# PreferredAI/cornac

Hardware: AMD Instinct MI355X
Metric: bpr_triplets_per_sec (higher is better)
Workload: dtype f32

## Files before the change

### cornac_amd/_lib.py

```python
import ctypes as C
import os
import subprocess

import numpy as np

_HERE = os.path.dirname(os.path.abspath(__file__))
PROFILE = os.environ.get("CORNAC_HIP_PROFILE", "") == "1"
LIB_PATH = os.path.join(_HERE, "lib", "libcornac_hip_profile.so" if PROFILE else "libcornac_hip.so")
CSRC = os.path.join(_HERE, "csrc")

MODE_DETERMINISTIC = 0
MODE_HOGWILD = 1
VEBPR_NO_OWNERSHIP = 0x100
HOG_FORM_MASK, HOG_FORM_SHIFT = 0xF0000, 16
FORM_AUTO, FORM_FUSED, FORM_STRATA, FORM_LDSBIN = (f << HOG_FORM_SHIFT for f in range(4))
HOG_PLAIN_STORES, HOG_VEC4_LAYOUT, HOG_NO_OWNERSHIP, HOG_DENSE_BIAS, HOG_SHARE_NEG = 1, 2, 4, 8, 16
HOG_BINNED, HOG_FUSED_OPT_OUT = 64, 128
HOG_ABLATE_MASK, HOG_ABLATE_SHIFT = 0xFF00, 8
NEG_UNIFORM = 0
NEG_POPULARITY = 1

SYMBOLS = [
    "cornac_hip_last_error", "cornac_hip_version", "cornac_hip_device_count", "cornac_hip_device_info",
    "cornac_hip_device_probe",
    "cornac_hip_bpr_create", "cornac_hip_bpr_destroy", "cornac_hip_bpr_set_factors", "cornac_hip_bpr_get_factors",
    "cornac_hip_bpr_bind_device", "cornac_hip_bpr_rebind_items", "cornac_hip_bpr_conveyor_setup", "cornac_hip_bpr_conveyor_layout", "cornac_hip_bpr_conveyor_enqueue", "cornac_hip_bpr_set_negative_population", "cornac_hip_bpr_device_ptrs", "cornac_hip_bpr_set_stream",
    "cornac_hip_bpr_seed_mt19937", "cornac_hip_bpr_seed_hogwild", "cornac_hip_bpr_fit_epochs",
    "cornac_hip_bpr_set_factors_f64", "cornac_hip_bpr_get_factors_f64", "cornac_hip_bpr_fit_epochs_f64",
    "cornac_hip_bpr_hogwild_enqueue", "cornac_hip_bpr_sync", "cornac_hip_bpr_debug_draw",
    "cornac_hip_bpr_last_timing", "cornac_hip_bpr_kernel_timing", "cornac_hip_mf_kernel_timing",
    "cornac_hip_bpr_debug_ownership", "cornac_hip_bpr_set_views", "cornac_hip_bpr_seed_view_stream",
    "cornac_hip_vebpr_fit_epochs", "cornac_hip_vebpr_fit_epochs_f64", "cornac_hip_vebpr_hogwild_form",
    "cornac_hip_mmmf_fit_epochs", "cornac_hip_mmmf_fit_epochs_f64", "cornac_hip_mmmf_hogwild_enqueue",
    "cornac_hip_bpr_strata_config", "cornac_hip_bpr_chunk_records", "cornac_hip_bpr_strata_stats", "cornac_hip_bpr_debug_strata",
    "cornac_hip_bpr_ldsbin_config", "cornac_hip_bpr_ldsbin_pass_config", "cornac_hip_bpr_ldsbin_stats",
    "cornac_hip_bpr_ldsbin_deal_config", "cornac_hip_bpr_debug_ldsbin_deal",
    "cornac_hip_bpr_sample_triplets", "cornac_hip_bpr_apply_triplets", "cornac_hip_bpr_gather_rows",
    "cornac_hip_bpr_staged_slots", "cornac_hip_bpr_emit_triplets", "cornac_hip_bpr_apply_staged",
    "cornac_hip_bpr_shard_mark", "cornac_hip_bpr_shard_slots", "cornac_hip_bpr_shard_uniq",
    "cornac_hip_bpr_scatter_diff_rows", "cornac_hip_bpr_switch_stream",
    "cornac_hip_bpr_scatter_add_rows", "cornac_hip_bpr_table_delta_begin", "cornac_hip_bpr_table_delta_finish",
    "cornac_hip_bpr_table_delta_step", "cornac_hip_table_delta", "cornac_hip_bpr_table_delta",
    "cornac_hip_bpr_resident_exchange_bins", "cornac_hip_bpr_epoch_resident_enqueue", "cornac_hip_bpr_resident_flush",
    "cornac_hip_stream_wait_counter", "cornac_hip_stream_set_flag", "cornac_hip_stream_ring_standin",
    "cornac_hip_vbpr_create", "cornac_hip_vbpr_destroy", "cornac_hip_vbpr_set_params", "cornac_hip_vbpr_get_params",
    "cornac_hip_vbpr_fit_batches", "cornac_hip_vbpr_item_tables",
    "cornac_hip_wmf_create", "cornac_hip_wmf_destroy", "cornac_hip_wmf_set_factors", "cornac_hip_wmf_get_factors",
    "cornac_hip_wmf_fit_batches", "cornac_hip_wmf_kernel_timing", "cornac_hip_wmf_last_timing",
    "cornac_hip_mf_create", "cornac_hip_mf_destroy", "cornac_hip_mf_set_factors", "cornac_hip_mf_get_factors",
    "cornac_hip_mf_fit", "cornac_hip_mf_bind_items", "cornac_hip_mf_bind_users", "cornac_hip_mf_set_stream", "cornac_hip_mf_epoch_enqueue",
    "cornac_hip_mf_sync", "cornac_hip_mf_fit_sgd", "cornac_hip_mf_last_timing",
    "cornac_hip_mf_hogwild_form", "cornac_hip_mf_hogwild_stats", "cornac_hip_mf_debug_split", "cornac_hip_mf_debug_ownership",
    "cornac_hip_mf_fit_minibatch", "cornac_hip_mf_fit_minibatch_dropout", "cornac_hip_mf_reset_optimizer",
    "cornac_hip_mf_pmf_set_factors", "cornac_hip_mf_pmf_get_factors", "cornac_hip_mf_pmf_fit", "cornac_hip_mf_pmf_form",
    "cornac_hip_mf_nmf_set_factors", "cornac_hip_mf_nmf_get_factors", "cornac_hip_mf_nmf_fit", "cornac_hip_mf_nmf_form",
    "cornac_hip_mf_hpf_set_tables", "cornac_hip_mf_hpf_get_tables", "cornac_hip_mf_hpf_fit", "cornac_hip_mf_hpf_elog",
    "cornac_hip_mf_hpf_form",
    "cornac_hip_scorer_create", "cornac_hip_scorer_destroy", "cornac_hip_scorer_set", "cornac_hip_score_user",
    "cornac_hip_scorer_set_f64", "cornac_hip_score_user_f64",
    "cornac_hip_score_block", "cornac_hip_rank_topk", "cornac_hip_rank_topk_device", "cornac_hip_score_pairs",
    "cornac_hip_scorer_set_exclusions", "cornac_hip_rank_topk_resident", "cornac_hip_scorer_host_buffer",
    "cornac_hip_rank_positions",
]


class HipError(RuntimeError):

    def __init__(self, code, msg):
        super().__init__("libcornac_hip error %d: %s" % (code, msg))
        self.code = code


def build(force=False, verbose=False):
    cmd = ["make", "-C", CSRC, "-j", "4"] + (["-B"] if force else []) + (["PROFILE=1"] if PROFILE else [])
    out = subprocess.run(cmd, stdout=subprocess.PIPE, stderr=subprocess.STDOUT, text=True)
    if verbose or out.returncode != 0:
        print(out.stdout)
    if out.returncode != 0:
        raise RuntimeError("building libcornac_hip.so failed")
    return LIB_PATH


_lib = None

_f32 = np.ctypeslib.ndpointer(np.float32, flags="C_CONTIGUOUS")
_i32 = np.ctypeslib.ndpointer(np.int32, flags="C_CONTIGUOUS")
_i64 = np.ctypeslib.ndpointer(np.int64, flags="C_CONTIGUOUS")
_vp = C.c_void_p


def _preload_torch_hip_runtime():
    import importlib.util
    import sys

    if "torch" in sys.modules:
        return
    try:
        spec = importlib.util.find_spec("torch")
        libdir = os.path.join(list(spec.submodule_search_locations)[0], "lib")
    except Exception:
        return
    for name in ("libhsa-runtime64.so", "libamdhip64.so"):
        path = os.path.join(libdir, name)
        if os.path.exists(path):
            try:
                C.CDLL(path, mode=C.RTLD_GLOBAL)
            except OSError:
                return


def lib():
    global _lib
    if _lib is None:
        if not os.path.exists(LIB_PATH):
            raise RuntimeError(
                "libcornac_hip.so not found at %s. Build it with `python -c 'import __graft_entry__ as g; g.build()'` "
                "or `make -C cornac_amd/csrc`. cornac_amd has no CPU fallback." % LIB_PATH)
        _preload_torch_hip_runtime()
        L = C.CDLL(LIB_PATH)
        L.cornac_hip_last_error.restype = C.c_char_p
        L.cornac_hip_version.restype = C.c_char_p
        L.cornac_hip_device_count.argtypes = [C.POINTER(C.c_int)]
        L.cornac_hip_device_info.argtypes = [C.c_int, C.c_char_p, C.c_int, C.POINTER(C.c_int), C.POINTER(C.c_int64)]
        L.cornac_hip_device_probe.argtypes = [C.c_int, C.c_int64, C.POINTER(C.c_double)]
        L.cornac_hip_bpr_create.argtypes = [C.POINTER(_vp), C.c_int, C.c_int64, C.c_int64, C.c_int64, C.c_int64,
                                            C.c_int, _i32, _i32, C.c_int64]
        L.cornac_hip_bpr_destroy.argtypes = [_vp]
        L.cornac_hip_bpr_set_factors.argtypes = [_vp, _vp, _vp, _vp]
        L.cornac_hip_bpr_get_factors.argtypes = [_vp, _vp, _vp, _vp]
        L.cornac_hip_bpr_bind_device.argtypes = [_vp, _vp, _vp, _vp]
        L.cornac_hip_bpr_rebind_items.argtypes = [_vp, _vp, _vp]
        L.cornac_hip_bpr_conveyor_setup.argtypes = [_vp, C.c_int, _vp, C.c_uint64, C.c_int, C.POINTER(C.c_int), C.POINTER(C.c_int),
                                                    C.POINTER(C.c_int)]
        L.cornac_hip_bpr_conveyor_layout.argtypes = [_vp, C.c_uint32, _vp, _vp]
        L.cornac_hip_bpr_conveyor_enqueue.argtypes = [_vp, C.c_uint32, C.c_uint32, C.c_int, C.POINTER(C.c_int32), C.POINTER(_vp),
                                                      C.c_float, C.c_float, C.c_int, C.c_int, C.c_int]
        L.cornac_hip_bpr_set_negative_population.argtypes = [_vp, _vp, C.c_int64]
        L.cornac_hip_bpr_device_ptrs.argtypes = [_vp, C.POINTER(_vp), C.POINTER(_vp), C.POINTER(_vp)]
        L.cornac_hip_bpr_set_stream.argtypes = [_vp, _vp]
        L.cornac_hip_bpr_switch_stream.argtypes = [_vp, _vp]
        L.cornac_hip_bpr_seed_mt19937.argtypes = [_vp, C.c_uint32, C.c_uint32, C.c_int]
        L.cornac_hip_bpr_seed_hogwild.argtypes = [_vp, C.c_uint64]
        L.cornac_hip_bpr_fit_epochs.argtypes = [_vp, C.c_int, C.c_float, C.c_float, C.c_int, C.c_int, C.c_int,
                                                C.c_int, C.POINTER(C.c_int64), C.POINTER(C.c_int64)]
        L.cornac_hip_bpr_set_factors_f64.argtypes = [_vp, _vp, _vp, _vp]
        L.cornac_hip_bpr_get_factors_f64.argtypes = [_vp, _vp, _vp, _vp]
        L.cornac_hip_bpr_fit_epochs_f64.argtypes = [_vp, C.c_int, C.c_double, C.c_double, C.c_int, C.c_int,
                                                    C.POINTER(C.c_int64), C.POINTER(C.c_int64)]
        L.cornac_hip_bpr_hogwild_enqueue.argtypes = [_vp, C.c_int64, C.c_float, C.c_float, C.c_int, C.c_int, C.c_int]
        L.cornac_hip_bpr_sync.argtypes = [_vp, C.POINTER(C.c_int64), C.POINTER(C.c_int64)]
        L.cornac_hip_bpr_debug_draw.argtypes = [_vp, C.c_int, C.c_uint64, C.c_int64, _i64]
        L.cornac_hip_bpr_last_timing.argtypes = [_vp, C.POINTER(C.c_double)]
        L.cornac_hip_bpr_set_views.argtypes = [_vp, _i32, _i32, C.c_int64]
        L.cornac_hip_bpr_seed_view_stream.argtypes = [_vp, C.c_uint32]
        L.cornac_hip_vebpr_hogwild_form.argtypes = [_vp, C.POINTER(C.c_int)]
        L.cornac_hip_vebpr_fit_epochs.argtypes = [_vp, C.c_int, C.c_float, C.c_float, C.c_float, C.c_int,
                                                  C.POINTER(C.c_int64), C.POINTER(C.c_int64)]
        L.cornac_hip_vebpr_fit_epochs_f64.argtypes = [_vp, C.c_int, C.c_double, C.c_double, C.c_double,
                                                      C.POINTER(C.c_int64), C.POINTER(C.c_int64)]
        L.cornac_hip_mmmf_fit_epochs.argtypes = [_vp, C.c_int, C.c_float, C.c_float, C.c_int, C.POINTER(C.c_int64),
                                                 C.POINTER(C.c_int64)]
        L.cornac_hip_mmmf_fit_epochs_f64.argtypes = [_vp, C.c_int, C.c_double, C.c_double, C.POINTER(C.c_int64),
                                                     C.POINTER(C.c_int64)]
        L.cornac_hip_mmmf_hogwild_enqueue.argtypes = [_vp, C.c_int64, C.c_float, C.c_float]
        L.cornac_hip_bpr_sample_triplets.argtypes = [_vp, C.c_int64, C.c_int, _vp, _vp, _vp]
        L.cornac_hip_bpr_apply_triplets.argtypes = [_vp, _vp, _vp, _vp, C.c_int64, _vp, _vp, C.c_int, C.c_float,
                                                    C.c_float, C.c_int]
        L.cornac_hip_bpr_gather_rows.argtypes = [_vp, _vp, _vp, C.c_int64, C.c_int, _vp]
        L.cornac_hip_bpr_staged_slots.argtypes = [_vp, C.c_int64, C.POINTER(C.c_int64)]
        L.cornac_hip_bpr_emit_triplets.argtypes = [_vp, C.c_int64, C.c_int, _vp, _vp, _vp, C.c_int64, C.POINTER(C.c_int64)]
        L.cornac_hip_bpr_apply_staged.argtypes = [_vp, _vp, _vp, _vp, C.c_int64, _vp, _vp, C.c_int, C.c_float, C.c_float,
                                                  C.c_int]
        L.cornac_hip_bpr_shard_mark.argtypes = [_vp, _vp, _vp, C.c_int64, C.c_int, C.c_int64, _vp]
        L.cornac_hip_bpr_shard_slots.argtypes = [_vp, _vp, _vp, C.c_int64, C.c_int, C.c_int64, _vp, _vp, _vp]
        L.cornac_hip_bpr_shard_uniq.argtypes = [_vp, _vp, _vp, C.c_int64, C.c_int64, _vp]
        L.cornac_hip_bpr_scatter_diff_rows.argtypes = [_vp, _vp, _vp, C.c_int64, C.c_int, _vp, _vp, _vp]
        L.cornac_hip_bpr_scatter_add_rows.argtypes = [_vp, _vp, _vp, C.c_int64, C.c_int, _vp]
        L.cornac_hip_bpr_table_delta_begin.argtypes = [_vp, _vp, _vp, C.c_int64, C.c_int, _vp, _vp]
        L.cornac_hip_bpr_table_delta_finish.argtypes = [_vp, _vp, _vp, _vp, _vp, C.c_int64, C.c_int]
        L.cornac_hip_bpr_table_delta_step.argtypes = [_vp, _vp, _vp, _vp, _vp, C.c_int64, C.c_int, _vp, _vp]
        L.cornac_hip_table_delta.argtypes = [C.c_int, C.c_int, _vp, _vp, _vp, _vp, _vp, C.c_int64, C.c_int, _vp, _vp]
        L.cornac_hip_bpr_table_delta.argtypes = [_vp, C.c_int, C.c_int, _vp, _vp, _vp, _vp, C.c_int64, C.c_int, _vp, _vp]
        L.cornac_hip_bpr_resident_exchange_bins.argtypes = [_vp, C.c_int, C.c_int, C.POINTER(C.c_int)]
        L.cornac_hip_bpr_epoch_resident_enqueue.argtypes = [_vp, C.c_float, C.c_float, C.c_int, C.c_int, C.c_int, C.c_int,
                                                            C.c_int, _vp, _vp, C.c_int64, _vp, C.c_int64, _vp, _vp, _vp,
                                                            C.POINTER(C.c_int)]
        L.cornac_hip_bpr_resident_flush.argtypes = [_vp, C.c_int, C.c_int, _vp, _vp, C.c_int64, _vp, C.c_int64, _vp, _vp]
        L.cornac_hip_stream_wait_counter.argtypes = [C.c_int, _vp, _vp, C.c_uint32, _vp, C.c_int]
        L.cornac_hip_stream_set_flag.argtypes = [C.c_int, _vp, _vp, C.c_uint32, _vp]
        L.cornac_hip_stream_ring_standin.argtypes = [C.c_int, _vp, _vp, C.c_int64, _vp, C.c_int64, C.c_int64, C.c_int]
        L.cornac_hip_bpr_debug_ownership.argtypes = [_vp, C.POINTER(C.c_int64), _vp, _vp, _vp]
        L.cornac_hip_bpr_strata_config.argtypes = [_vp, C.c_int, C.c_int, C.c_int]
        L.cornac_hip_bpr_chunk_records.argtypes = [_vp, C.c_int]
        L.cornac_hip_bpr_strata_stats.argtypes = [_vp, C.POINTER(C.c_int64)]
        L.cornac_hip_bpr_debug_strata.argtypes = [_vp, C.c_uint32, _vp, _vp, _vp, _vp, C.POINTER(C.c_uint32)]
        L.cornac_hip_bpr_ldsbin_config.argtypes = [_vp, C.c_int, C.c_int, C.c_int]
        L.cornac_hip_bpr_ldsbin_pass_config.argtypes = [_vp, C.c_int, C.c_int, C.c_int, C.c_int]
        L.cornac_hip_bpr_ldsbin_stats.argtypes = [_vp, C.POINTER(C.c_int64)]
        L.cornac_hip_bpr_ldsbin_deal_config.argtypes = [_vp, C.c_int, C.c_int]
        L.cornac_hip_bpr_debug_ldsbin_deal.argtypes = [_vp, C.c_uint64, C.c_uint32, _vp, _vp, _vp, _vp, _vp]
        L.cornac_hip_bpr_kernel_timing.argtypes = [_vp, C.c_int, C.POINTER(C.c_double), C.POINTER(C.c_int64)]
        L.cornac_hip_mf_kernel_timing.argtypes = [_vp, C.c_int, C.POINTER(C.c_double), C.POINTER(C.c_int64)]
        L.cornac_hip_vbpr_create.argtypes = [C.POINTER(_vp), C.c_int, C.c_int64, C.c_int64, C.c_int, C.c_int, C.c_int, _f32]
        L.cornac_hip_vbpr_destroy.argtypes = [_vp]
        L.cornac_hip_vbpr_set_params.argtypes = [_vp] + [_vp] * 6
        L.cornac_hip_vbpr_get_params.argtypes = [_vp] + [_vp] * 6
        L.cornac_hip_vbpr_fit_batches.argtypes = [_vp, _i32, _i32, _i32, C.c_int64, C.c_int, C.c_float, C.c_float,
                                                  C.c_float, C.c_float, C.POINTER(C.c_double)]
        L.cornac_hip_vbpr_item_tables.argtypes = [_vp, _f32, _f32]
        L.cornac_hip_mf_fit_minibatch.argtypes = [_vp, _i64, C.c_int64, C.c_int, C.c_int, C.c_float, C.c_float,
                                                  C.c_float, C.c_int, C.POINTER(C.c_double)]
        L.cornac_hip_mf_fit_minibatch_dropout.argtypes = [_vp, _i64, C.c_int64, C.c_int, C.c_int, C.c_float, C.c_float,
                                                          C.c_float, C.c_int, _vp, _vp, C.c_float, C.POINTER(C.c_double)]
        L.cornac_hip_mf_reset_optimizer.argtypes = [_vp]
        L.cornac_hip_mf_pmf_set_factors.argtypes = [_vp, _vp, _vp]
        L.cornac_hip_mf_pmf_get_factors.argtypes = [_vp, _vp, _vp]
        L.cornac_hip_mf_pmf_fit.argtypes = [_vp, C.c_int, C.c_float, C.c_float, C.c_float, C.c_int, _vp]
        L.cornac_hip_mf_pmf_form.argtypes = [_vp, C.POINTER(C.c_int), C.POINTER(C.c_int)]
        L.cornac_hip_mf_nmf_set_factors.argtypes = [_vp, _vp, _vp, _vp, _vp]
        L.cornac_hip_mf_nmf_get_factors.argtypes = [_vp, _vp, _vp, _vp, _vp]
        L.cornac_hip_mf_nmf_fit.argtypes = [_vp, C.c_int] + [C.c_float] * 6 + [C.c_int, C.c_int, _vp]
        L.cornac_hip_mf_nmf_form.argtypes = [_vp] + [C.POINTER(C.c_int)] * 3
        L.cornac_hip_mf_hpf_set_tables.argtypes = [_vp] * 5
        L.cornac_hip_mf_hpf_get_tables.argtypes = [_vp] * 7
        L.cornac_hip_mf_hpf_fit.argtypes = [_vp, C.c_int, C.c_int]
        L.cornac_hip_mf_hpf_elog.argtypes = [_vp, _vp, _vp]
        L.cornac_hip_mf_hpf_form.argtypes = [_vp] + [C.POINTER(C.c_int)] * 2
        L.cornac_hip_wmf_create.argtypes = [C.POINTER(_vp), C.c_int, C.c_int64, C.c_int64, C.c_int, _i64, _i32, _f32,
                                            C.c_int64]
        L.cornac_hip_wmf_destroy.argtypes = [_vp]
        L.cornac_hip_wmf_destroy.restype = None
        L.cornac_hip_wmf_set_factors.argtypes = [_vp, _f32, _f32]
        L.cornac_hip_wmf_get_factors.argtypes = [_vp, _f32, _f32]
        L.cornac_hip_wmf_fit_batches.argtypes = [_vp, _i32, _i64, C.c_int64, C.c_float, C.c_float, C.c_float,
                                                 C.c_float, C.c_float, _vp]
        L.cornac_hip_wmf_kernel_timing.argtypes = [_vp, C.c_int]
        L.cornac_hip_wmf_last_timing.argtypes = [_vp, C.POINTER(C.c_double)]
        L.cornac_hip_mf_create.argtypes = [C.POINTER(_vp), C.c_int, C.c_int64, C.c_int64, C.c_int, _i64, _i64, _f32,
                                           C.c_int64]
        L.cornac_hip_mf_destroy.argtypes = [_vp]
        L.cornac_hip_mf_set_factors.argtypes = [_vp, _vp, _vp, _vp, _vp]
        L.cornac_hip_mf_get_factors.argtypes = [_vp, _vp, _vp, _vp, _vp]
        L.cornac_hip_mf_bind_items.argtypes = [_vp, _vp, _vp]
        L.cornac_hip_mf_bind_users.argtypes = [_vp, _vp, _vp]
        L.cornac_hip_mf_set_stream.argtypes = [_vp, _vp]
        L.cornac_hip_mf_epoch_enqueue.argtypes = [_vp, C.c_int, C.c_int, C.c_float, C.c_float, C.c_float, C.c_int]
        L.cornac_hip_mf_sync.argtypes = [_vp, C.POINTER(C.c_double)]
        L.cornac_hip_mf_fit.argtypes = [_vp, C.c_int, C.c_float, C.c_float, C.c_float, C.c_int, C.c_int, C.c_int, _vp,
                                        C.POINTER(C.c_int)]
        L.cornac_hip_mf_fit_sgd.argtypes = [C.c_int, _i64, _i64, _f32, C.c_int64, _f32, _f32, _f32, _f32, C.c_int64,
                                            C.c_int64, C.c_int, C.c_float, C.c_float, C.c_float, C.c_int, C.c_int,
                                            C.c_int, C.c_int, _vp, C.POINTER(C.c_int)]
        L.cornac_hip_mf_last_timing.argtypes = [_vp, C.POINTER(C.c_double)]
        L.cornac_hip_mf_hogwild_form.argtypes = [_vp, C.c_int]
        L.cornac_hip_mf_hogwild_stats.argtypes = [_vp, C.POINTER(C.c_int64)]
        L.cornac_hip_mf_debug_split.argtypes = [_vp, C.POINTER(C.c_int64), C.POINTER(C.c_int64), _vp, _vp]
        L.cornac_hip_mf_debug_ownership.argtypes = [_vp, C.POINTER(C.c_int64), _vp, _vp, _vp]
        L.cornac_hip_scorer_create.argtypes = [C.POINTER(_vp), C.c_int, C.c_int64, C.c_int64, C.c_int]
        L.cornac_hip_scorer_destroy.argtypes = [_vp]
        L.cornac_hip_scorer_set.argtypes = [_vp, _f32, _f32, _vp, _vp]
        L.cornac_hip_score_user.argtypes = [_vp, C.c_int64, _f32]
        L.cornac_hip_scorer_set_f64.argtypes = [_vp, _vp, _vp, _vp, _vp]
        L.cornac_hip_score_user_f64.argtypes = [_vp, C.c_int64, _vp]
        L.cornac_hip_score_block.argtypes = [_vp, _i32, C.c_int64, _f32]
        L.cornac_hip_score_pairs.argtypes = [_vp, _i32, _i32, C.c_int64, C.c_int, C.c_float, C.c_float, _f32]
        L.cornac_hip_rank_topk.argtypes = [_vp, _i32, C.c_int64, C.c_int, _vp, _vp, _i32, _f32]
        L.cornac_hip_rank_positions.argtypes = [_vp, _i32, C.c_int64, _vp, _vp, _vp, _vp, _i32, _i32, _i32, _f32]
        L.cornac_hip_rank_topk_device.argtypes = [_vp, C.c_int64, C.c_int64, C.c_int, C.c_int, C.POINTER(C.c_double)]
        L.cornac_hip_scorer_set_exclusions.argtypes = [_vp, _vp, _vp]
        L.cornac_hip_scorer_host_buffer.argtypes = [_vp, C.c_size_t, C.POINTER(_vp)]
        L.cornac_hip_rank_topk_resident.argtypes = [_vp, _vp, C.c_int64, C.c_int64, C.c_int, _vp, _vp, _vp]
        _lib = L
    return _lib


def check(rc):
    if rc != 0:
        raise HipError(rc, lib().cornac_hip_last_error().decode("utf-8", "replace"))


def stream_wait_counter(device, stream, d_counter, target, d_error, timeout_ms=5000):
    check(lib().cornac_hip_stream_wait_counter(int(device), stream, d_counter, int(target), d_error, int(timeout_ms)))


def stream_ring_standin(device, stream, d_src, src_floats, d_dst, dst_floats, n_floats, n_workgroups=16):
    check(lib().cornac_hip_stream_ring_standin(int(device), stream, d_src, int(src_floats), d_dst, int(dst_floats),
                                               int(n_floats), int(n_workgroups)))


def stream_set_flag(device, stream, d_flag, value=1, d_unless=None):
    check(lib().cornac_hip_stream_set_flag(int(device), stream, d_flag, int(value), d_unless))


def device_count():
    n = C.c_int(0)
    check(lib().cornac_hip_device_count(C.byref(n)))
    return n.value


def device_probe(device=0, nbytes=6 << 30):
    o = (C.c_double * 3)()
    check(lib().cornac_hip_device_probe(device, int(nbytes), o))
    return {"d2d_copy_GBps": o[0], "stream_read_GBps": o[1], "row_gather_512B_GBps": o[2], "buffer_bytes": int(nbytes)}


def device_info(device=0):
    name = C.create_string_buffer(256)
    cus = C.c_int()
    mem = C.c_int64()
    check(lib().cornac_hip_device_info(device, name, 256, C.byref(cus), C.byref(mem)))
    return {"name": name.value.decode(), "compute_units": cus.value, "hbm_bytes": mem.value}


def _ptr(a):
    return None if a is None else a.ctypes.data


def _f32c(a):
    return None if a is None else np.ascontiguousarray(a, dtype=np.float32)


class BprTrainer:

    def __init__(self, indptr, indices, n_users, n_items, total_users, total_items, k, device=0):
        self.indptr = np.ascontiguousarray(indptr, np.int32)
        self.indices = np.ascontiguousarray(indices, np.int32)
        self.shape = (int(total_users), int(total_items), int(k))
        self.nnz = len(self.indices)
        self.n_items = int(n_items)
        self.device, self._stream = int(device), None
        self.h = _vp()
        check(lib().cornac_hip_bpr_create(C.byref(self.h), device, n_users, n_items, total_users, total_items, k,
                                          self.indptr, self.indices, self.nnz))

    def close(self):
        if getattr(self, "h", None) is not None and self.h and lib is not None:
            lib().cornac_hip_bpr_destroy(self.h)
            self.h = None

    __del__ = close

    def set_factors(self, U=None, V=None, B=None):
        U, V, B = _f32c(U), _f32c(V), _f32c(B)
        tu, ti, k = self.shape
        assert U is None or U.shape == (tu, k)
        assert V is None or V.shape == (ti, k)
        assert B is None or B.shape == (ti,)
        check(lib().cornac_hip_bpr_set_factors(self.h, _ptr(U), _ptr(V), _ptr(B)))

    def get_factors(self):
        tu, ti, k = self.shape
        U, V, B = np.empty((tu, k), np.float32), np.empty((ti, k), np.float32), np.empty(ti, np.float32)
        check(lib().cornac_hip_bpr_get_factors(self.h, U.ctypes.data, V.ctypes.data, B.ctypes.data))
        return U, V, B

    def set_factors_f64(self, U, V, B):
        tu, ti, k = self.shape
        U, V, B = (np.ascontiguousarray(a, np.float64) for a in (U, V, B))
        assert U.shape == (tu, k) and V.shape == (ti, k) and B.shape == (ti,)
        check(lib().cornac_hip_bpr_set_factors_f64(self.h, U.ctypes.data, V.ctypes.data, B.ctypes.data))

    def get_factors_f64(self):
        tu, ti, k = self.shape
        U, V, B = np.empty((tu, k), np.float64), np.empty((ti, k), np.float64), np.empty(ti, np.float64)
        check(lib().cornac_hip_bpr_get_factors_f64(self.h, U.ctypes.data, V.ctypes.data, B.ctypes.data))
        return U, V, B

    def fit_epochs_f64(self, n_epochs, lr, reg, use_bias=True, neg_population=NEG_UNIFORM):
        c, s = C.c_int64(), C.c_int64()
        check(lib().cornac_hip_bpr_fit_epochs_f64(self.h, n_epochs, float(lr), float(reg), int(use_bias), neg_population,
                                                  C.byref(c), C.byref(s)))
        return c.value, s.value

    def get_user_factors(self):
        tu, _, k = self.shape
        U = np.empty((tu, k), np.float32)
        check(lib().cornac_hip_bpr_get_factors(self.h, U.ctypes.data, None, None))
        return U

    def get_item_factors(self):
        _, ti, k = self.shape
        V, B = np.empty((ti, k), np.float32), np.empty(ti, np.float32)
        check(lib().cornac_hip_bpr_get_factors(self.h, None, V.ctypes.data, B.ctypes.data))
        return V, B

    def seed_mt19937(self, seed_pos, seed_neg, shared_stream=False):
        check(lib().cornac_hip_bpr_seed_mt19937(self.h, seed_pos, seed_neg, int(shared_stream)))

    def seed_hogwild(self, seed):
        check(lib().cornac_hip_bpr_seed_hogwild(self.h, int(seed) & 0xFFFFFFFFFFFFFFFF))

    def fit_epochs(self, n_epochs, lr, reg, use_bias=True, neg_population=NEG_UNIFORM, mode=MODE_HOGWILD, flags=0):
        c, s = C.c_int64(), C.c_int64()
        check(lib().cornac_hip_bpr_fit_epochs(self.h, n_epochs, lr, reg, int(use_bias), neg_population, mode, flags,
                                              C.byref(c), C.byref(s)))
        return c.value, s.value

    def hogwild_enqueue(self, n_samples, lr, reg, use_bias=True, neg_population=NEG_UNIFORM, flags=0):
        check(lib().cornac_hip_bpr_hogwild_enqueue(self.h, n_samples, lr, reg, int(use_bias), neg_population, flags))

    def sync(self):
        c, s = C.c_int64(), C.c_int64()
        check(lib().cornac_hip_bpr_sync(self.h, C.byref(c), C.byref(s)))
        return c.value, s.value

    def bind_device(self, dU=None, dV=None, dB=None):
        check(lib().cornac_hip_bpr_bind_device(self.h, dU, dV, dB))

    def set_negative_population(self, items):
        items = np.ascontiguousarray(items if items is not None else [], np.int32)
        check(lib().cornac_hip_bpr_set_negative_population(self.h, items.ctypes.data if len(items) else None, len(items)))

    def rebind_items(self, dV, dB):
        check(lib().cornac_hip_bpr_rebind_items(self.h, dV, dB))

    def conveyor_setup(self, n_blocks, rank_item=None, deal_seed=0, release_item_tables=True):
        order = None if rank_item is None else np.ascontiguousarray(rank_item, np.int32)
        nb, bpb, cap = C.c_int(), C.c_int(), C.c_int()
        check(lib().cornac_hip_bpr_conveyor_setup(self.h, int(n_blocks), None if order is None else order.ctypes.data,
                                                  int(deal_seed) & 0xFFFFFFFFFFFFFFFF, int(bool(release_item_tables)),
                                                  C.byref(nb), C.byref(bpb), C.byref(cap)))
        return nb.value, bpb.value, cap.value

    def conveyor_layout(self, layout_epoch, d_slot_item, d_item_slot):
        check(lib().cornac_hip_bpr_conveyor_layout(self.h, int(layout_epoch), d_slot_item, d_item_slot))

    def conveyor_enqueue(self, epoch, layout_epoch, first_blocks, d_rows, lr, reg, use_bias=True, neg_population=NEG_UNIFORM,
                         flags=0):
        n = len(first_blocks)
        fb = (C.c_int32 * n)(*[int(b) for b in first_blocks])
        rows = (_vp * n)(*[int(p) for p in d_rows])
        check(lib().cornac_hip_bpr_conveyor_enqueue(self.h, int(epoch), int(layout_epoch), n, fb, rows, lr, reg, int(use_bias),
                                                    neg_population, int(flags)))

    def device_ptrs(self):
        u, v, b = _vp(), _vp(), _vp()
        check(lib().cornac_hip_bpr_device_ptrs(self.h, C.byref(u), C.byref(v), C.byref(b)))
        return u.value, v.value, b.value

    def set_stream(self, stream_ptr):
        check(lib().cornac_hip_bpr_set_stream(self.h, stream_ptr))
        self._stream = stream_ptr

    def switch_stream(self, stream_ptr):
        check(lib().cornac_hip_bpr_switch_stream(self.h, stream_ptr))
        self._stream = stream_ptr

    def sample_triplets(self, n_draws, d_u, d_i, d_j, neg_population=NEG_UNIFORM):
        check(lib().cornac_hip_bpr_sample_triplets(self.h, int(n_draws), neg_population, d_u, d_i, d_j))

    def apply_triplets(self, d_u, d_slot_i, d_slot_j, n, d_rows, d_bias, bias_stride, lr, reg, use_bias=True):
        check(lib().cornac_hip_bpr_apply_triplets(self.h, d_u, d_slot_i, d_slot_j, int(n), d_rows, d_bias,
                                                  int(bias_stride), lr, reg, int(use_bias)))

    def staged_slots(self, n_draws):
        n = C.c_int64()
        check(lib().cornac_hip_bpr_staged_slots(self.h, int(n_draws), C.byref(n)))
        return n.value

    def emit_triplets(self, n_draws, d_u, d_i, d_j, slots_cap, neg_population=NEG_UNIFORM):
        n = C.c_int64()
        check(lib().cornac_hip_bpr_emit_triplets(self.h, int(n_draws), neg_population, d_u, d_i, d_j, int(slots_cap),
                                                 C.byref(n)))
        return n.value

    def apply_staged(self, d_u, d_slot_i, d_slot_j, n_slots, d_rows, d_bias, bias_stride, lr, reg, use_bias=True):
        check(lib().cornac_hip_bpr_apply_staged(self.h, d_u, d_slot_i, d_slot_j, int(n_slots), d_rows, d_bias,
                                                int(bias_stride), lr, reg, int(use_bias)))

    def shard_mark(self, d_i, d_j, n, world, rows_per_rank, d_mark):
        check(lib().cornac_hip_bpr_shard_mark(self.h, d_i, d_j, int(n), int(world), int(rows_per_rank), d_mark))

    def shard_slots(self, d_i, d_j, n, world, rows_per_rank, d_scan, d_slot_i, d_slot_j):
        check(lib().cornac_hip_bpr_shard_slots(self.h, d_i, d_j, int(n), int(world), int(rows_per_rank), d_scan, d_slot_i,
                                               d_slot_j))

    def shard_uniq(self, d_mark, d_scan, n_rows, rows_per_rank, d_uniq_local):
        check(lib().cornac_hip_bpr_shard_uniq(self.h, d_mark, d_scan, int(n_rows), int(rows_per_rank), d_uniq_local))

    def scatter_diff_rows(self, d_table, d_ids, n, width, d_now, d_before, d_scale=None):
        check(lib().cornac_hip_bpr_scatter_diff_rows(self.h, d_table, d_ids, int(n), int(width), d_now, d_before, d_scale))

    def _delta(self, op, rule, *args):
        check(lib().cornac_hip_bpr_table_delta(self.h, op, int(rule), *args))

    def table_delta_begin(self, d_flat, d_base, n_items, k, d_bucket, d_local, rule=0):
        if rule:
            return self._delta(0, rule, d_flat, d_base, None, None, int(n_items), int(k), d_bucket, d_local)
        check(lib().cornac_hip_bpr_table_delta_begin(self.h, d_flat, d_base, int(n_items), int(k), d_bucket, d_local))

    def table_delta_finish(self, d_flat, d_base, d_bucket, d_local, n_items, k, rule=0):
        if rule:
            return self._delta(1, rule, d_flat, d_base, d_bucket, d_local, int(n_items), int(k), None, None)
        check(lib().cornac_hip_bpr_table_delta_finish(self.h, d_flat, d_base, d_bucket, d_local, int(n_items), int(k)))

    def table_delta_step(self, d_flat, d_base, d_bucket_prev, d_local_prev, n_items, k, d_bucket, d_local, rule=0):
        if rule:
            return self._delta(2, rule, d_flat, d_base, d_bucket_prev, d_local_prev, int(n_items), int(k), d_bucket, d_local)
        check(lib().cornac_hip_bpr_table_delta_step(self.h, d_flat, d_base, d_bucket_prev, d_local_prev, int(n_items),
                                                    int(k), d_bucket, d_local))

    def resident_exchange_bins(self, neg_population=NEG_UNIFORM, flags=0):
        n = C.c_int()
        check(lib().cornac_hip_bpr_resident_exchange_bins(self.h, neg_population, flags, C.byref(n)))
        return n.value

    def epoch_resident_enqueue(self, lr, reg, use_bias, neg_population, flags, n_exchanges, rule, d_base, d_buckets,
                               bucket_stride, d_keeps, keep_stride, d_arrive, d_landed, d_applied):
        n = C.c_int()
        check(lib().cornac_hip_bpr_epoch_resident_enqueue(self.h, lr, reg, int(use_bias), neg_population, flags,
                                                          int(n_exchanges), int(rule), d_base, d_buckets, int(bucket_stride),
                                                          d_keeps, int(keep_stride), d_arrive, d_landed, d_applied, C.byref(n)))
        return n.value

    def resident_flush(self, n_exchanges, rule, d_base, d_buckets, bucket_stride, d_keeps, keep_stride, d_applied, d_landed=None):
        check(lib().cornac_hip_bpr_resident_flush(self.h, int(n_exchanges), int(rule), d_base, d_buckets, int(bucket_stride),
                                                  d_keeps, int(keep_stride), d_applied, d_landed))

    def gather_rows(self, d_table, d_ids, n, width, d_out):
        check(lib().cornac_hip_bpr_gather_rows(self.h, d_table, d_ids, int(n), int(width), d_out))

    def scatter_add_rows(self, d_table, d_ids, n, width, d_delta):
        check(lib().cornac_hip_bpr_scatter_add_rows(self.h, d_table, d_ids, int(n), int(width), d_delta))

    def debug_draw(self, stream, hi, n):
        out = np.empty(n, np.int64)
        check(lib().cornac_hip_bpr_debug_draw(self.h, stream, hi, n, out))
        return out

    def set_views(self, view_indptr, view_indices):
        self.v_indptr = np.ascontiguousarray(view_indptr, np.int32)
        self.v_indices = np.ascontiguousarray(view_indices, np.int32)
        if len(self.v_indices) == 0:
            self.v_indices = np.zeros(1, np.int32)
        check(lib().cornac_hip_bpr_set_views(self.h, self.v_indptr, self.v_indices, int(self.v_indptr[-1])))

    def seed_view_stream(self, seed_view):
        check(lib().cornac_hip_bpr_seed_view_stream(self.h, seed_view))

    def fit_epochs_vebpr(self, n_epochs, lr, reg, alpha, mode=MODE_HOGWILD, ownership=True):
        c, s = C.c_int64(), C.c_int64()
        check(lib().cornac_hip_vebpr_fit_epochs(self.h, n_epochs, lr, reg, alpha, mode | (0 if ownership else VEBPR_NO_OWNERSHIP),
                                                C.byref(c), C.byref(s)))
        return c.value, s.value

    def fit_epochs_vebpr_f64(self, n_epochs, lr, reg, alpha):
        c, s = C.c_int64(), C.c_int64()
        check(lib().cornac_hip_vebpr_fit_epochs_f64(self.h, n_epochs, float(lr), float(reg), float(alpha), C.byref(c),
                                                    C.byref(s)))
        return c.value, s.value

    def vebpr_hogwild_owned(self):
        o = C.c_int()
        check(lib().cornac_hip_vebpr_hogwild_form(self.h, C.byref(o)))
        return bool(o.value)

    def mmmf_fit_epochs(self, n_epochs, lr, reg, mode=MODE_HOGWILD):
        c, s = C.c_int64(), C.c_int64()
        check(lib().cornac_hip_mmmf_fit_epochs(self.h, n_epochs, lr, reg, mode, C.byref(c), C.byref(s)))
        return c.value, s.value

    def mmmf_fit_epochs_f64(self, n_epochs, lr, reg):
        c, s = C.c_int64(), C.c_int64()
        check(lib().cornac_hip_mmmf_fit_epochs_f64(self.h, n_epochs, float(lr), float(reg), C.byref(c), C.byref(s)))
        return c.value, s.value

    def mmmf_hogwild_enqueue(self, n_samples, lr, reg):
        check(lib().cornac_hip_mmmf_hogwild_enqueue(self.h, n_samples, lr, reg))

    def debug_ownership(self):
        w = C.c_int64()
        check(lib().cornac_hip_bpr_debug_ownership(self.h, C.byref(w), None, None, None))
        if w.value == 0:
            return None
        wp = np.empty(w.value + 1, np.int64)
        ou, oi = np.empty(self.nnz, np.int32), np.empty(self.nnz, np.int32)
        check(lib().cornac_hip_bpr_debug_ownership(self.h, C.byref(w), wp.ctypes.data, ou.ctypes.data,
                                                   oi.ctypes.data))
        return wp, ou, oi

    def ldsbin_config(self, hot_x1000=75, min_candidates=48, max_rounds=4):
        check(lib().cornac_hip_bpr_ldsbin_config(self.h, int(hot_x1000), int(min_candidates), int(max_rounds)))

    def ldsbin_deal_config(self, strata_groups=16, hot_cost_x16=32):
        check(lib().cornac_hip_bpr_ldsbin_deal_config(self.h, int(strata_groups), int(hot_cost_x16)))

    def debug_ldsbin_deal(self, seed, epoch):
        st = self.ldsbin_stats()
        bins, nh = st["bins"], st["hot_interactions"]
        bin_of = np.empty(self.n_items, np.int32)
        cold, off = np.empty(bins, np.uint32), np.empty(bins + 1, np.uint32)
        hu, hi = np.empty(max(nh, 1), np.int32), np.empty(max(nh, 1), np.int32)
        check(lib().cornac_hip_bpr_debug_ldsbin_deal(self.h, int(seed), int(epoch), bin_of.ctypes.data, cold.ctypes.data,
                                                     off.ctypes.data, hu.ctypes.data, hi.ctypes.data))
        return bin_of, cold, off, hu[:nh], hi[:nh]

    def ldsbin_pass_config(self, enable=True, waves=8, lds_kb=64, min_draws_x100=200):
        check(lib().cornac_hip_bpr_ldsbin_pass_config(self.h, int(bool(enable)), int(waves), int(lds_kb), int(min_draws_x100)))

    def ldsbin_stats(self):
        o = (C.c_int64 * 8)()
        check(lib().cornac_hip_bpr_ldsbin_stats(self.h, o))
        return {"bins": o[0], "rows_per_bin": o[1], "n_hot": o[2], "hot_interactions": o[3], "bitmap_words": o[4],
                "lds_bytes": o[5], "lock_timeouts": o[6], "block_threads": o[7]}

    def strata_config(self, hot_permille=120, hot_min_mult_x100=200, rehash_period=1):
        check(lib().cornac_hip_bpr_strata_config(self.h, int(hot_permille), int(hot_min_mult_x100), int(rehash_period)))

    def chunk_records(self, enable=True):
        check(lib().cornac_hip_bpr_chunk_records(self.h, int(bool(enable))))

    def strata_stats(self):
        o = (C.c_int64 * 4)()
        check(lib().cornac_hip_bpr_strata_stats(self.h, o))
        return {"n_hot": o[0], "misplaced_workgroups": o[1], "bucket_builds": o[2], "waves": o[3]}

    def debug_strata(self, epoch):
        wp = self.debug_ownership()[0]
        W = len(wp) - 1
        sptr = np.empty(8 * W + 1, np.int64)
        ru, ri = np.empty(self.nnz, np.int32), np.empty(self.nnz, np.int32)
        rank_item = np.empty(self.n_items, np.int32)
        key = C.c_uint32()
        check(lib().cornac_hip_bpr_debug_strata(self.h, int(epoch), sptr.ctypes.data, ru.ctypes.data, ri.ctypes.data,
                                                rank_item.ctypes.data, C.byref(key)))
        return sptr, ru, ri, rank_item, key.value

    def kernel_timing(self, enable=True):
        ms, n = C.c_double(), C.c_int64()
        check(lib().cornac_hip_bpr_kernel_timing(self.h, int(enable), C.byref(ms), C.byref(n)))
        return ms.value, n.value

    def last_timing(self):
        t = (C.c_double * 4)()
        check(lib().cornac_hip_bpr_last_timing(self.h, t))
        return {"sampler_ms": t[0], "schedule_ms": t[1], "sgd_ms": t[2], "total_ms": t[3]}


class MfTrainer:
    def __init__(self, rid, cid, val, n_users, n_items, k, device=0):
        self.rid = np.ascontiguousarray(rid, np.int64)
        self.cid = np.ascontiguousarray(cid, np.int64)
        self.val = np.ascontiguousarray(val, np.float32)
        self.shape = (int(n_users), int(n_items), int(k))
        self.h = _vp()
        check(lib().cornac_hip_mf_create(C.byref(self.h), device, n_users, n_items, k, self.rid, self.cid, self.val,
                                         len(self.val)))
        self.device, self._stream = int(device), None

    def close(self):
        if getattr(self, "h", None) is not None and self.h and lib is not None:
            lib().cornac_hip_mf_destroy(self.h)
            self.h = None

    __del__ = close

    def set_factors(self, U=None, V=None, Bu=None, Bi=None):
        U, V, Bu, Bi = _f32c(U), _f32c(V), _f32c(Bu), _f32c(Bi)
        check(lib().cornac_hip_mf_set_factors(self.h, _ptr(U), _ptr(V), _ptr(Bu), _ptr(Bi)))

    def get_factors(self):
        nu, ni, k = self.shape
        U, V = np.empty((nu, k), np.float32), np.empty((ni, k), np.float32)
        Bu, Bi = np.empty(nu, np.float32), np.empty(ni, np.float32)
        check(lib().cornac_hip_mf_get_factors(self.h, U.ctypes.data, V.ctypes.data, Bu.ctypes.data, Bi.ctypes.data))
        return U, V, Bu, Bi

    def fit(self, max_iter, lr, reg, mu, use_bias=True, early_stop=False, mode=MODE_HOGWILD):
        loss = np.zeros(max(max_iter, 1), np.float32)
        n = C.c_int()
        check(lib().cornac_hip_mf_fit(self.h, max_iter, lr, reg, mu, int(use_bias), int(early_stop), mode,
                                      loss.ctypes.data, C.byref(n)))
        return loss[:n.value], n.value

    def bind_items(self, d_V, d_Bi):
        check(lib().cornac_hip_mf_bind_items(self.h, d_V, d_Bi))

    def bind_users(self, d_U, d_Bu):
        check(lib().cornac_hip_mf_bind_users(self.h, d_U, d_Bu))

    def set_stream(self, hip_stream):
        check(lib().cornac_hip_mf_set_stream(self.h, hip_stream))
        self._stream = hip_stream

    def epoch_enqueue(self, part, n_parts, lr, reg, mu, use_bias=True):
        check(lib().cornac_hip_mf_epoch_enqueue(self.h, int(part), int(n_parts), lr, reg, mu, int(use_bias)))

    def sync(self):
        l = C.c_double()
        check(lib().cornac_hip_mf_sync(self.h, C.byref(l)))
        return l.value

    def table_delta_begin(self, d_flat, d_base, n_items, k, d_bucket, d_local, rule=0):
        check(lib().cornac_hip_table_delta(0 | (int(rule) << 4), self.device, self._stream, d_flat, d_base, None, None,
                                           int(n_items), int(k), d_bucket, d_local))

    def table_delta_finish(self, d_flat, d_base, d_bucket, d_local, n_items, k, rule=0):
        check(lib().cornac_hip_table_delta(1 | (int(rule) << 4), self.device, self._stream, d_flat, d_base, d_bucket, d_local,
                                           int(n_items), int(k), None, None))

    def table_delta_step(self, d_flat, d_base, d_bucket_prev, d_local_prev, n_items, k, d_bucket, d_local, rule=0):
        check(lib().cornac_hip_table_delta(2 | (int(rule) << 4), self.device, self._stream, d_flat, d_base, d_bucket_prev,
                                           d_local_prev, int(n_items), int(k), d_bucket, d_local))

    OPTIMIZERS = {"sgd": 0, "adam": 1, "rmsprop": 2, "adagrad": 3}

    def fit_minibatch(self, order, batch_size, optimizer, lr, reg, mu, use_bias=True, keep_u=None, keep_i=None,
                      keep_scale=1.0):
        order = np.ascontiguousarray(order, np.int64)
        loss = C.c_double()
        if keep_u is not None:
            keep_u, keep_i = np.ascontiguousarray(keep_u, np.uint8), np.ascontiguousarray(keep_i, np.uint8)
            if keep_u.shape != (len(order), self.shape[2]) or keep_i.shape != keep_u.shape:
                raise ValueError("keep masks must be [len(order), k] = %r, got %r / %r"
                                 % ((len(order), self.shape[2]), keep_u.shape, keep_i.shape))
            check(lib().cornac_hip_mf_fit_minibatch_dropout(self.h, order, len(order), int(batch_size),
                                                            self.OPTIMIZERS[optimizer], lr, reg, mu, int(use_bias),
                                                            keep_u.ctypes.data, keep_i.ctypes.data, float(keep_scale),
                                                            C.byref(loss)))
            return loss.value
        check(lib().cornac_hip_mf_fit_minibatch(self.h, order, len(order), int(batch_size), self.OPTIMIZERS[optimizer],
                                                lr, reg, mu, int(use_bias), C.byref(loss)))
        return loss.value

    def reset_optimizer(self):
        check(lib().cornac_hip_mf_reset_optimizer(self.h))

    PMF_VARIANTS = {"linear": 0, "non_linear": 1}

    def pmf_set_factors(self, U, V):
        nu, ni, k = self.shape
        U, V = np.ascontiguousarray(U, np.float64), np.ascontiguousarray(V, np.float64)
        if U.shape != (nu, k) or V.shape != (ni, k):
            raise ValueError("PMF tables must be %r and %r, got %r and %r" % ((nu, k), (ni, k), U.shape, V.shape))
        check(lib().cornac_hip_mf_pmf_set_factors(self.h, U.ctypes.data, V.ctypes.data))

    def pmf_get_factors(self):
        nu, ni, k = self.shape
        U, V = np.empty((nu, k), np.float64), np.empty((ni, k), np.float64)
        check(lib().cornac_hip_mf_pmf_get_factors(self.h, U.ctypes.data, V.ctypes.data))
        return U, V

    def pmf_fit(self, n_epochs, lr, reg, gamma, variant):
        loss = np.zeros(max(int(n_epochs), 1), np.float64)
        check(lib().cornac_hip_mf_pmf_fit(self.h, int(n_epochs), lr, reg, gamma, self.PMF_VARIANTS.get(variant, variant),
                                          loss.ctypes.data))
        return loss[:max(int(n_epochs), 0)]

    def pmf_form(self):
        form, group = C.c_int(), C.c_int()
        check(lib().cornac_hip_mf_pmf_form(self.h, C.byref(form), C.byref(group)))
        return form.value, group.value

    def nmf_set_factors(self, U, V, Bu=None, Bi=None):
        nu, ni, k = self.shape
        U, V, Bu, Bi = _f32c(U), _f32c(V), _f32c(Bu), _f32c(Bi)
        if U.shape != (nu, k) or V.shape != (ni, k):
            raise ValueError("NMF tables must be %r and %r, got %r and %r" % ((nu, k), (ni, k), U.shape, V.shape))
        if (Bu is not None and Bu.shape != (nu,)) or (Bi is not None and Bi.shape != (ni,)):
            raise ValueError("NMF biases must be (%d,) and (%d,)" % (nu, ni))
        check(lib().cornac_hip_mf_nmf_set_factors(self.h, _ptr(U), _ptr(V), _ptr(Bu), _ptr(Bi)))

    def nmf_get_factors(self):
        nu, ni, k = self.shape
        U, V = np.empty((nu, k), np.float32), np.empty((ni, k), np.float32)
        Bu, Bi = np.empty(nu, np.float32), np.empty(ni, np.float32)
        check(lib().cornac_hip_mf_nmf_get_factors(self.h, U.ctypes.data, V.ctypes.data, Bu.ctypes.data, Bi.ctypes.data))
        return U, V, Bu, Bi

    def nmf_fit(self, n_epochs, lr, lambda_u, lambda_v, lambda_bu, lambda_bi, mu, use_bias=False, mode=MODE_HOGWILD):
        loss = np.zeros(max(int(n_epochs), 1), np.float64)
        check(lib().cornac_hip_mf_nmf_fit(self.h, int(n_epochs), lr, lambda_u, lambda_v, lambda_bu, lambda_bi, mu,
                                          int(bool(use_bias)), int(mode), loss.ctypes.data))
        return loss[:max(int(n_epochs), 0)]

    def nmf_form(self):
        o = [C.c_int(), C.c_int(), C.c_int()]
        check(lib().cornac_hip_mf_nmf_form(self.h, *[C.byref(x) for x in o]))
        return tuple(x.value for x in o)

    HPF_MAX_K = 256

    def hpf_set_tables(self, G_s, G_r, L_s, L_r):
        nu, ni, k = self.shape
        if k > self.HPF_MAX_K:
            raise ValueError("HPF keeps a row's sums in registers: k = %d is above its limit of %d" % (k, self.HPF_MAX_K))
        tables = [np.ascontiguousarray(a, np.float64) for a in (G_s, G_r, L_s, L_r)]
        for a, name, shape in zip(tables, ("G_s", "G_r", "L_s", "L_r"), ((nu, k), (nu, k), (ni, k), (ni, k))):
            if a.shape != shape:
                raise ValueError("HPF table %s must be %r, got %r" % (name, shape, a.shape))
            if not (np.isfinite(a).all() and (a > 0).all()):
                raise ValueError("HPF table %s must be strictly positive and finite" % name)
        check(lib().cornac_hip_mf_hpf_set_tables(self.h, *[a.ctypes.data for a in tables]))

    def hpf_get_tables(self):
        nu, ni, k = self.shape
        out = [np.empty(s, np.float64) for s in ((nu, k), (nu, k), (ni, k), (ni, k), (nu,), (ni,))]
        check(lib().cornac_hip_mf_hpf_get_tables(self.h, *[a.ctypes.data for a in out]))
        return tuple(out)

    def hpf_fit(self, n_iters, hierarchical=True):
        check(lib().cornac_hip_mf_hpf_fit(self.h, int(n_iters), int(bool(hierarchical))))

    def hpf_elog(self):
        nu, ni, k = self.shape
        Lt, Lb = np.empty((nu, k), np.float64), np.empty((ni, k), np.float64)
        check(lib().cornac_hip_mf_hpf_elog(self.h, Lt.ctypes.data, Lb.ctypes.data))
        return Lt, Lb

    def hpf_form(self):
        o = [C.c_int(), C.c_int()]
        check(lib().cornac_hip_mf_hpf_form(self.h, *[C.byref(x) for x in o]))
        return tuple(x.value for x in o)

    def kernel_timing(self, enable=True):
        ms, n = C.c_double(), C.c_int64()
        check(lib().cornac_hip_mf_kernel_timing(self.h, int(enable), C.byref(ms), C.byref(n)))
        return ms.value, n.value

    def hogwild_form(self, form):
        check(lib().cornac_hip_mf_hogwild_form(self.h, int(form)))

    def hogwild_stats(self):
        o = (C.c_int64 * 4)()
        check(lib().cornac_hip_mf_hogwild_stats(self.h, o))
        return {"form_used": o[0], "tiles": o[1], "rows_per_bin": o[2], "gave_up": bool(o[3])}

    def debug_split(self):
        ns, nv = C.c_int64(), C.c_int64()
        check(lib().cornac_hip_mf_debug_split(self.h, C.byref(ns), C.byref(nv), None, None))
        items, ptr = np.empty(ns.value, np.int32), np.zeros(ns.value + 1, np.int32)
        if ns.value:
            check(lib().cornac_hip_mf_debug_split(self.h, C.byref(ns), C.byref(nv), items.ctypes.data, ptr.ctypes.data))
        return items, ptr

    def debug_ownership(self):
        w = C.c_int64()
        check(lib().cornac_hip_mf_debug_ownership(self.h, C.byref(w), None, None, None))
        if w.value == 0:
            return None
        wp = np.empty(w.value + 1, np.int64)
        ou, oi = np.empty(len(self.val), np.int32), np.empty(len(self.val), np.int32)
        check(lib().cornac_hip_mf_debug_ownership(self.h, C.byref(w), wp.ctypes.data, ou.ctypes.data, oi.ctypes.data))
        return wp, ou, oi

    def last_timing(self):
        t = (C.c_double * 4)()
        check(lib().cornac_hip_mf_last_timing(self.h, t))
        return {"schedule_ms": t[1], "sgd_ms": t[2], "total_ms": t[3]}


def mf_fit_sgd(rid, cid, val, U, V, Bu, Bi, lr, reg, mu, max_iter, use_bias, early_stop, mode, device=0):
    loss = np.zeros(max(max_iter, 1), np.float32)
    n = C.c_int()
    check(lib().cornac_hip_mf_fit_sgd(device, np.ascontiguousarray(rid, np.int64), np.ascontiguousarray(cid, np.int64),
                                      np.ascontiguousarray(val, np.float32), len(val), U, V, Bu, Bi, U.shape[0],
                                      V.shape[0], U.shape[1], lr, reg, mu, max_iter, int(use_bias), int(early_stop),
                                      mode, loss.ctypes.data, C.byref(n)))
    return loss[:n.value]


class Scorer:
    def __init__(self, U, V, item_base=None, user_base=None, device=0):
        U, V = _f32c(U), _f32c(V)
        self.n_users, self.k = U.shape
        self.n_items = V.shape[0]
        self.h = _vp()
        check(lib().cornac_hip_scorer_create(C.byref(self.h), device, self.n_users, self.n_items, self.k))
        self.set(U, V, item_base, user_base)

    def set(self, U, V, item_base=None, user_base=None):
        ib, ub = _f32c(item_base), _f32c(user_base)
        check(lib().cornac_hip_scorer_set(self.h, _f32c(U), _f32c(V), _ptr(ib), _ptr(ub)))

    def close(self):
        if getattr(self, "h", None) is not None and self.h and lib is not None:
            lib().cornac_hip_scorer_destroy(self.h)
            self.h = None

    __del__ = close

    def score_user(self, user):
        out = np.empty(self.n_items, np.float32)
        check(lib().cornac_hip_score_user(self.h, int(user), out))
        return out

    def set_f64(self, U, V, item_base=None, user_base=None):
        U, V = np.ascontiguousarray(U, np.float64), np.ascontiguousarray(V, np.float64)
        assert U.shape == (self.n_users, self.k) and V.shape == (self.n_items, self.k)
        ib = None if item_base is None else np.ascontiguousarray(item_base, np.float64)
        ub = None if user_base is None else np.ascontiguousarray(user_base, np.float64)
        check(lib().cornac_hip_scorer_set_f64(self.h, U.ctypes.data, V.ctypes.data, _ptr(ib), _ptr(ub)))

    def score_user_f64(self, user):
        out = np.empty(self.n_items, np.float64)
        check(lib().cornac_hip_score_user_f64(self.h, int(user), out.ctypes.data))
        return out

    def score_block(self, users):
        users = np.ascontiguousarray(users, np.int32)
        out = np.empty((len(users), self.n_items), np.float32)
        check(lib().cornac_hip_score_block(self.h, users, len(users), out))
        return out

    def score_pairs(self, users, items, clip=None):
        users = np.ascontiguousarray(users, np.int32)
        items = np.ascontiguousarray(items, np.int32)
        out = np.empty(len(users), np.float32)
        lo, hi = (0.0, 0.0) if clip is None else (float(clip[0]), float(clip[1]))
        check(lib().cornac_hip_score_pairs(self.h, users, items, len(users), int(clip is not None), lo, hi, out))
        return out

    def rank_topk(self, users, topk, exclude=None):
        users = np.ascontiguousarray(users, np.int32)
        items = np.empty((len(users), topk), np.int32)
        scores = np.empty((len(users), topk), np.float32)
        ip = ix = None
        if exclude is not None:
            ip = np.ascontiguousarray(exclude[0], np.int64)
            ix = np.ascontiguousarray(exclude[1], np.int32)
        check(lib().cornac_hip_rank_topk(self.h, users, len(users), topk, _ptr(ip), _ptr(ix), items, scores))
        return items, scores

    def rank_positions(self, users, targets, exclude=None):
        users = np.ascontiguousarray(users, np.int32)
        tp = np.ascontiguousarray(targets[0], np.int64)
        tx = np.ascontiguousarray(targets[1], np.int32)
        nt = int(tp[-1])
        greater, pos, ge = (np.empty(nt, np.int32) for _ in range(3))
        scores = np.empty(nt, np.float32)
        ip = ix = None
        if exclude is not None:
            ip = np.ascontiguousarray(exclude[0], np.int64)
            ix = np.ascontiguousarray(exclude[1], np.int32)
        check(lib().cornac_hip_rank_positions(self.h, users, len(users), _ptr(ip), _ptr(ix), _ptr(tp), _ptr(tx), greater,
                                              pos, ge, scores))
        return greater, pos, ge, scores

    def set_exclusions(self, indptr=None, indices=None):
        if indptr is None:
            check(lib().cornac_hip_scorer_set_exclusions(self.h, None, None))
            return
        ip = np.ascontiguousarray(indptr, np.int64)
        ix = np.ascontiguousarray(indices, np.int32)
        assert len(ip) == self.n_users + 1
        check(lib().cornac_hip_scorer_set_exclusions(self.h, ip.ctypes.data, _ptr(ix) if len(ix) else None))

    def rank_topk_resident(self, users, topk, fetch=True, timed=False, pinned=False):
        if isinstance(users, tuple):
            up, u0, n = None, int(users[0]), int(users[1])
        else:
            ua = np.ascontiguousarray(users, np.int32)
            up, u0, n = ua.ctypes.data, 0, len(ua)
        if fetch and pinned:
            want_scores = fetch != "items"
            nbytes = n * topk * 4 * (2 if want_scores else 1)
            buf = _vp()
            check(lib().cornac_hip_scorer_host_buffer(self.h, nbytes, C.byref(buf)))
            raw = (C.c_char * nbytes).from_address(buf.value)
            items = np.frombuffer(raw, np.int32, n * topk).reshape(n, topk)
            scores = np.frombuffer(raw, np.float32, n * topk, offset=n * topk * 4).reshape(n, topk) if want_scores else None
        else:
            items = np.empty((n, topk), np.int32) if fetch else None
            scores = np.empty((n, topk), np.float32) if fetch and fetch != "items" else None
        ms = C.c_double()
        check(lib().cornac_hip_rank_topk_resident(self.h, up, u0, n, topk, _ptr(items), _ptr(scores),
                                                  C.cast(C.byref(ms), _vp) if timed else None))
        return (items, scores, ms.value) if timed else (items, scores)

    def rank_topk_device_ms(self, u0, n, topk, repeats=1):
        ms = C.c_double()
        check(lib().cornac_hip_rank_topk_device(self.h, u0, n, topk, repeats, C.byref(ms)))
        return ms.value


class VbprTrainer:
    NAMES = ("Bi", "Gu", "Gi", "Tu", "E", "Bp")

    def __init__(self, features, n_users, n_items, k, k2, device=0):
        self.F = np.ascontiguousarray(features, np.float32)
        assert self.F.shape[0] == n_items
        self.dims = dict(n_users=int(n_users), n_items=int(n_items), k=int(k), k2=int(k2), n_feat=self.F.shape[1])
        self.h = _vp()
        check(lib().cornac_hip_vbpr_create(C.byref(self.h), device, n_users, n_items, k, k2, self.F.shape[1], self.F))

    def close(self):
        if getattr(self, "h", None) is not None and self.h and lib is not None:
            lib().cornac_hip_vbpr_destroy(self.h)
            self.h = None

    __del__ = close

    def _shapes(self):
        d = self.dims
        return {"Bi": (d["n_items"],), "Gu": (d["n_users"], d["k"]), "Gi": (d["n_items"], d["k"]),
                "Tu": (d["n_users"], d["k2"]), "E": (d["n_feat"], d["k2"]), "Bp": (d["n_feat"],)}

    def set_params(self, **params):
        arrs = []
        for n in self.NAMES:
            a = params.get(n)
            if a is not None:
                a = np.ascontiguousarray(np.asarray(a, np.float32).reshape(self._shapes()[n]))
            arrs.append(a)
        check(lib().cornac_hip_vbpr_set_params(self.h, *[_ptr(a) for a in arrs]))

    def get_params(self):
        out = {n: np.empty(s, np.float32) for n, s in self._shapes().items()}
        check(lib().cornac_hip_vbpr_get_params(self.h, *[out[n].ctypes.data for n in self.NAMES]))
        return out

    def fit_batches(self, u, i, j, batch_size, lr, lambda_w, lambda_b, lambda_e):
        u, i, j = (np.ascontiguousarray(x, np.int32) for x in (u, i, j))
        nll = C.c_double()
        check(lib().cornac_hip_vbpr_fit_batches(self.h, u, i, j, len(u), batch_size, lr, lambda_w, lambda_b, lambda_e,
                                                C.byref(nll)))
        return nll.value

    def item_tables(self):
        d = self.dims
        th, vb = np.empty((d["n_items"], d["k2"]), np.float32), np.empty(d["n_items"], np.float32)
        check(lib().cornac_hip_vbpr_item_tables(self.h, th, vb))
        return th, vb


class WmfTrainer:

    def __init__(self, csc, k, device=0):
        csc = csc.tocsc()
        self.n_users, self.n_items = (int(x) for x in csc.shape)
        self.k = int(k)
        self._indptr = np.ascontiguousarray(csc.indptr, np.int64)
        self._rows = np.ascontiguousarray(csc.indices, np.int32)
        self._vals = np.ascontiguousarray(csc.data, np.float32)
        self.h = _vp()
        check(lib().cornac_hip_wmf_create(C.byref(self.h), device, self.n_users, self.n_items, self.k, self._indptr,
                                          self._rows if len(self._rows) else np.zeros(1, np.int32),
                                          self._vals if len(self._vals) else np.zeros(1, np.float32), len(self._vals)))

    def close(self):
        if getattr(self, "h", None) is not None and self.h and lib is not None:
            lib().cornac_hip_wmf_destroy(self.h)
            self.h = None

    __del__ = close

    def set_factors(self, U, V):
        U = np.ascontiguousarray(np.asarray(U, np.float32).reshape(self.n_users, self.k))
        V = np.ascontiguousarray(np.asarray(V, np.float32).reshape(self.n_items, self.k))
        check(lib().cornac_hip_wmf_set_factors(self.h, U, V))

    def get_factors(self):
        U, V = np.empty((self.n_users, self.k), np.float32), np.empty((self.n_items, self.k), np.float32)
        check(lib().cornac_hip_wmf_get_factors(self.h, U, V))
        return U, V

    def fit_batches(self, batches, lambda_u, lambda_v, a, b, lr):
        batches = [np.asarray(x, np.int32).ravel() for x in batches]
        if not batches:
            return np.zeros(0)
        ptr = np.zeros(len(batches) + 1, np.int64)
        np.cumsum([len(x) for x in batches], out=ptr[1:])
        ids = np.ascontiguousarray(np.concatenate(batches), np.int32)
        loss = np.zeros(len(batches), np.float64)
        check(lib().cornac_hip_wmf_fit_batches(self.h, ids, ptr, len(batches), lambda_u, lambda_v, a, b, lr,
                                               loss.ctypes.data))
        return loss

    def kernel_timing(self, enabled=True):
        check(lib().cornac_hip_wmf_kernel_timing(self.h, int(enabled)))

    def last_device_ms(self):
        ms = C.c_double()
        check(lib().cornac_hip_wmf_last_timing(self.h, C.byref(ms)))
        return ms.value
```

### cornac_amd/csrc/score.hip

```cpp
#include <algorithm>
#include <cmath>
#include <cstdlib>

#include "common.h"

namespace chip {

constexpr int kBlk = 256;
typedef float f32x16 __attribute__((ext_vector_type(16)));
typedef float v4f32 __attribute__((ext_vector_type(4)));

__device__ __forceinline__ uint32_t order_key(float s) {
    const uint32_t b = __float_as_uint(s);
    const uint32_t k = (b & 0x80000000u) ? ~b : (b | 0x80000000u);
    return k ? k : 1u;
}
__device__ __forceinline__ float key_to_float(uint32_t k) {
    const uint32_t b = (k & 0x80000000u) ? (k & 0x7fffffffu) : ~k;
    return __uint_as_float(b);
}

__global__ __launch_bounds__(kBlk) void score_valu_kernel(const float *__restrict__ U, const float *__restrict__ V,
                                                          const float *__restrict__ item_base,
                                                          const float *__restrict__ user_base,
                                                          const int32_t *__restrict__ users, int64_t u0,
                                                          int64_t n_items, int k, int ld, float *__restrict__ out) {
    extern __shared__ float urow[];
    const int64_t b = blockIdx.y;
    const int64_t u = users ? (int64_t)users[b] : u0 + b;
    for (int f = threadIdx.x; f < k; f += kBlk) urow[f] = U[u * ld + f];
    __syncthreads();
    const int64_t i = (int64_t)blockIdx.x * kBlk + threadIdx.x;
    if (i >= n_items) return;
    const float *row = V + i * ld;
    float acc = 0.f;
    for (int f = 0; f < k; ++f) acc = fmaf(urow[f], row[f], acc);
    const float ub = user_base ? user_base[u] : 0.f;
    const float ib = item_base ? item_base[i] : 0.f;
    out[b * n_items + i] = (ib + ub) + acc;
}

__global__ __launch_bounds__(kBlk) void score_pairs_kernel(const float *__restrict__ U, const float *__restrict__ V,
                                                           const float *__restrict__ item_base,
                                                           const float *__restrict__ user_base,
                                                           const int32_t *__restrict__ users,
                                                           const int32_t *__restrict__ items, int64_t n, int k, int ld,
                                                           int do_clip, float lo, float hi, float *__restrict__ out) {
    const int64_t p = (int64_t)blockIdx.x * kBlk + threadIdx.x;
    if (p >= n) return;
    const int64_t u = users[p], i = items[p];
    const float *pu = U + u * ld, *pv = V + i * ld;
    float acc = 0.f;
    for (int f = 0; f < k; ++f) acc = fmaf(pu[f], pv[f], acc);
    float s = ((item_base ? item_base[i] : 0.f) + (user_base ? user_base[u] : 0.f)) + acc;
    if (do_clip) s = fminf(fmaxf(s, lo), hi);
    out[p] = s;
}

template <int KT, int MT>
__global__ __launch_bounds__(kBlk) void score_gemm_mfma_kernel(const float *__restrict__ U,
                                                               const float *__restrict__ V,
                                                               const float *__restrict__ item_base,
                                                               const float *__restrict__ user_base,
                                                               const int32_t *__restrict__ users, int64_t u0,
                                                               int64_t n_rows, int64_t n_items, int k,
                                                               int tiles_per_strip, float *__restrict__ out) {
    const int wave = threadIdx.x >> 6, lane = threadIdx.x & 63;
    const int col = lane & 31, half = lane >> 5;
    const int64_t row_tile0 = ((int64_t)blockIdx.y * (kBlk / 64) + wave) * MT;
    if (row_tile0 * 32 >= n_rows) return;
    float a[MT][KT];
    float ubias[MT];
    int64_t urow[MT];
#pragma unroll
    for (int m = 0; m < MT; ++m) {
        const int64_t r = (row_tile0 + m) * 32 + col;
        const bool ok = r < n_rows;
        const int64_t u = ok ? (users ? (int64_t)users[r] : u0 + r) : 0;
        urow[m] = u;
        const float *p = U + u * (2 * KT) + half;
#pragma unroll
        for (int t = 0; t < KT; ++t) a[m][t] = p[2 * t];
        ubias[m] = 0.f;
    }
    const int64_t n_item_tiles = (n_items + 31) / 32;
    const int64_t t_begin = (int64_t)blockIdx.x * tiles_per_strip;
    const int64_t t_end = min(n_item_tiles, t_begin + tiles_per_strip);
    for (int64_t it = t_begin; it < t_end; ++it) {
        const int64_t item = it * 32 + col;
        const bool iok = item < n_items;
        const float *q = V + (iok ? item : 0) * (2 * KT) + half;
        float bfrag[KT];
#pragma unroll
        for (int t = 0; t < KT; ++t) bfrag[t] = q[2 * t];
        const float ib = (iok && item_base) ? item_base[item] : 0.f;
#pragma unroll
        for (int m = 0; m < MT; ++m) {
            f32x16 acc = {0.f, 0.f, 0.f, 0.f, 0.f, 0.f, 0.f, 0.f, 0.f, 0.f, 0.f, 0.f, 0.f, 0.f, 0.f, 0.f};
#pragma unroll
            for (int t = 0; t < KT; ++t) acc = __builtin_amdgcn_mfma_f32_32x32x2f32(a[m][t], bfrag[t], acc, 0, 0, 0);
            if (iok) {
#pragma unroll
                for (int r = 0; r < 16; ++r) {
                    const int64_t row = (row_tile0 + m) * 32 + (r & 3) + 8 * (r >> 2) + 4 * half;
                    if (row < n_rows) {
                        float ub = 0.f;
                        if (user_base) ub = user_base[users ? (int64_t)users[row] : u0 + row];
                        out[row * n_items + item] = (ib + ub) + acc[r];
                    }
                }
            }
        }
    }
    (void)ubias;
    (void)urow;
}

template <typename T>
__device__ __forceinline__ uint32_t lds_offset(T *p) {
    return (uint32_t)(uintptr_t)(__attribute__((address_space(3))) T *)p;
}

template <int KT, int CAP, bool UB>
__global__ __launch_bounds__(kBlk, ((KT <= 32 || CAP <= 42) ? 2 : 1)) void rank_fused_kernel(const float *__restrict__ U, const float *__restrict__ V,
                                                          const float *__restrict__ item_base,
                                                          const float *__restrict__ user_base,
                                                          const int32_t *__restrict__ users, int64_t u0,
                                                          int64_t n_rows, int64_t n_items, int64_t work_per_wg,
                                                          int topk, const int64_t *__restrict__ excl_indptr,
                                                          const int32_t *__restrict__ excl_indices, int64_t excl_row0,
                                                          const uint32_t *__restrict__ excl_bits,
                                                          const int32_t *__restrict__ perm, float *tau_pub,
                                                          unsigned long long *__restrict__ part, int ablate) {
    constexpr int KP = 2 * KT;
    __shared__ unsigned long long keys[kBlk / 64][32][CAP];
    __shared__ int32_t ipos[3][32];
    __shared__ int cnt[kBlk / 64][32];
    __shared__ float tau[kBlk / 64][32];
    __shared__ float btile[2][32][KP + 1];
    __shared__ uint32_t meta_dump[1];
    __shared__ uint32_t wmask[3][kBlk / 64][32];
    __shared__ float ibase[3][32];
    const int wave = threadIdx.x >> 6, lane = threadIdx.x & 63;
    const int col = lane & 31, half = lane >> 5;
    const int64_t n_item_tiles = (n_items + 31) / 32;
    const int64_t n_row_blocks = (n_rows + 127) / 128;
    const int64_t work_total = n_row_blocks * n_item_tiles;
    int64_t pos = (int64_t)blockIdx.x * work_per_wg;
    const int64_t work_end = min(work_total, pos + work_per_wg);
    int64_t cur_rb = 0;
    float bcur[KT];
    constexpr int STG = (32 * KP / 4 + kBlk - 1) / kBlk;
    v4f32 stg[STG];
    uint32_t voff[STG];
#pragma unroll
    for (int q = 0; q < STG; ++q) {
        const int idx = threadIdx.x + q * kBlk;
        voff[q] = idx < 32 * KP / 4 ? (uint32_t)(((idx / (KP / 4)) * KP + 4 * (idx % (KP / 4))) * 4) : 0u;
    }
    uint32_t stg_a = 0;
    int32_t stg_id = 0;
    const uint32_t *pa = reinterpret_cast<const uint32_t *>(item_base);
    int64_t pa_stride = 0;
    const bool wave0 = __builtin_amdgcn_readfirstlane((int)(threadIdx.x >> 6)) == 0;
    const int32_t *pb = perm;
    auto stage_seek = [&](int64_t it) {
        if (threadIdx.x < 32) {
            pa = reinterpret_cast<const uint32_t *>(item_base) + it * 32 + threadIdx.x;
            pa_stride = 32;
        } else if (excl_bits && threadIdx.x < 32 + 32 * (kBlk / 64) && !(ablate & 32)) {
            const int w = (threadIdx.x - 32) >> 5, rl = (threadIdx.x - 32) & 31;
            pa = excl_bits + ((cur_rb * (kBlk / 64) + w) * 32 + rl) * n_item_tiles + it;
            pa_stride = 1;
        } else {
            pa = reinterpret_cast<const uint32_t *>(item_base);
            pa_stride = 0;
        }
        pb = perm + it * 32 + (threadIdx.x & 31);
    };
    auto stage_load = [&](int64_t it) {
        const char *vb = reinterpret_cast<const char *>(V) + it * (int64_t)(32 * KP * 4);
#pragma unroll
        for (int q = 0; q < STG; ++q) stg[q] = *reinterpret_cast<const v4f32 *>(vb + voff[q]);
        stg_a = *pa;
        pa += pa_stride;
        if (wave0) {
            stg_id = *pb;
            pb += 32;
        }
    };
    uint32_t meta_addr0 = lds_offset(&meta_dump[0]), meta_stride = 0;
    if (threadIdx.x < 32) {
        meta_addr0 = lds_offset(&ibase[0][threadIdx.x]);
        meta_stride = 32 * sizeof(float);
    } else if (excl_bits && threadIdx.x < 32 + 32 * (kBlk / 64)) {
        meta_addr0 = lds_offset(&wmask[0][(threadIdx.x - 32) >> 5][(threadIdx.x - 32) & 31]);
        meta_stride = (kBlk / 64) * 32 * sizeof(uint32_t);
    }
    auto stage_store = [&](int buf, int wbuf) {
#pragma unroll
        for (int q = 0; q < STG; ++q) {
            const int idx = threadIdx.x + q * kBlk;
            if ((q + 1) * kBlk <= 32 * KP / 4 || idx < 32 * KP / 4) {
                float *dst = &btile[buf][idx / (KP / 4)][4 * (idx % (KP / 4))];
                dst[0] = stg[q].x; dst[1] = stg[q].y; dst[2] = stg[q].z; dst[3] = stg[q].w;
            }
        }
        *reinterpret_cast<__attribute__((address_space(3))) uint32_t *>(meta_addr0 + (uint32_t)wbuf * meta_stride) = stg_a;
        if (wave0) ipos[wbuf][threadIdx.x & 31] = stg_id;
    };
    constexpr int FG = KT < 8 ? KT : 8;
    auto load_frags = [&](int buf, int g) {
#pragma unroll
        for (int t = g * FG; t < (g + 1) * FG; ++t) bcur[t] = btile[buf][col][2 * t + half];
    };
    const f32x16 zero16 = {0.f, 0.f, 0.f, 0.f, 0.f, 0.f, 0.f, 0.f, 0.f, 0.f, 0.f, 0.f, 0.f, 0.f, 0.f, 0.f};

    int64_t pos_hi = work_end;
    while (pos_hi > pos) {
        const int64_t rb = (pos_hi - 1) / n_item_tiles;
        cur_rb = rb;
        const int64_t seg_lo = max(pos, rb * n_item_tiles);
        const int64_t t_begin = seg_lo - rb * n_item_tiles;
        const int64_t t_end = pos_hi - rb * n_item_tiles;
        const int64_t seg = (int64_t)blockIdx.x - (rb * n_item_tiles) / work_per_wg;
        pos_hi = seg_lo;
        const int64_t row_tile = rb * (kBlk / 64) + wave;
        if (lane < 32) {
            cnt[wave][lane] = 0;
            const int64_t row = row_tile * 32 + lane;
            float t0 = -INFINITY;
            if (row >= n_rows) t0 = INFINITY;
            else if (t_begin > 0) t0 = __hip_atomic_load(tau_pub + row, __ATOMIC_RELAXED, __HIP_MEMORY_SCOPE_AGENT);
            tau[wave][lane] = t0;
        }
        float a[KT];
        {
            const int64_t r = row_tile * 32 + col;
            const bool ok = r < n_rows;
            const int64_t u = ok ? (users ? (int64_t)users[r] : u0 + r) : 0;
            const float *p = U + u * (2 * KT) + half;
#pragma unroll
            for (int t = 0; t < KT; ++t) a[t] = p[2 * t];
        }
        float ubias[16], thr[16];
        int cnt_r[16];
#pragma unroll
        for (int r = 0; r < 16; ++r) {
            const int rl = (r & 3) + 8 * (r >> 2) + 4 * half;
            const int64_t row = row_tile * 32 + rl;
            const bool row_ok = row < n_rows;
            ubias[r] = 0.f;
            if (user_base && row_ok) ubias[r] = user_base[users ? (int64_t)users[row] : u0 + row];
            thr[r] = row_ok ? -INFINITY : INFINITY;
            cnt_r[r] = 0;
        }
        if (t_begin > 0) {
            __builtin_amdgcn_fence(__ATOMIC_ACQ_REL, "wavefront");
            __builtin_amdgcn_wave_barrier();
#pragma unroll
            for (int r = 0; r < 16; ++r) thr[r] = tau[wave][(r & 3) + 8 * (r >> 2) + 4 * half];
        }
        auto compact = [&](unsigned need_l) __attribute__((always_inline)) {
            unsigned need = __builtin_amdgcn_readlane(need_l, 0) | __builtin_amdgcn_readlane(need_l, 32);
            if (col == 0) {
#pragma unroll
                for (int r = 0; r < 16; ++r) cnt[wave][(r & 3) + 8 * (r >> 2) + 4 * half] = cnt_r[r];
            }
            __builtin_amdgcn_fence(__ATOMIC_ACQ_REL, "wavefront");
            __builtin_amdgcn_wave_barrier();
            while (need) {
                const int rl = __builtin_ctz(need);
                need &= need - 1u;
                const int c = cnt[wave][rl];
                unsigned long long *krow = keys[wave][rl];
                unsigned long long mine = lane < c ? krow[lane] : 0ull;
                if (excl_indptr && !excl_bits) {
                    bool dropped = false;
                    if (mine != 0ull) {
                        const int32_t item = (int32_t)(uint32_t)mine;
                        const int64_t grow = excl_row0 + row_tile * 32 + rl;
                        int64_t lo = excl_indptr[grow], hi = excl_indptr[grow + 1];
                        const int64_t end = hi;
                        while (lo < hi) {
                            const int64_t mid = lo + ((hi - lo) >> 1);
                            if (excl_indices[mid] < item) lo = mid + 1; else hi = mid;
                        }
                        dropped = lo < end && excl_indices[lo] == item;
                    }
                    if (dropped) {
                        mine = 0ull;
                        krow[lane] = 0ull;
                    }
                    __builtin_amdgcn_fence(__ATOMIC_ACQ_REL, "wavefront");
                    __builtin_amdgcn_wave_barrier();
                }
                int rank = 0;
                for (int j0 = 0; j0 < c; j0 += 8) {
                    unsigned long long kj[8];
#pragma unroll
                    for (int q = 0; q < 8; ++q) kj[q] = krow[min(j0 + q, CAP - 1)];
#pragma unroll
                    for (int q = 0; q < 8; ++q) rank += (j0 + q < c && kj[q] > mine) ? 1 : 0;
                }
                const bool live = mine != 0ull;
                const int n_keep = min(__popcll(__ballot(live)), topk);
                const unsigned long long kth_mask = __ballot(live && rank == topk - 1);
                if (lane < CAP) krow[lane] = 0ull;
                if (live && rank < topk) krow[rank] = mine;
                if (kth_mask != 0ull) {
                    const int src = __builtin_ctzll(kth_mask);
                    const unsigned hi = __builtin_amdgcn_readlane((unsigned)(mine >> 32), src);
                    if (lane == 0 && row_tile * 32 + rl < n_rows) tau[wave][rl] = key_to_float(hi);
                }
                if (lane == 0) cnt[wave][rl] = n_keep;
            }
            __builtin_amdgcn_fence(__ATOMIC_ACQ_REL, "wavefront");
            __builtin_amdgcn_wave_barrier();
#pragma unroll
            for (int r = 0; r < 16; ++r) {
                const int rl = (r & 3) + 8 * (r >> 2) + 4 * half;
                thr[r] = tau[wave][rl];
                cnt_r[r] = cnt[wave][rl];
            }
        };
        f32x16 acc_a = zero16, acc_b = zero16;
        int wb = 0;
        float ib_a = 0.f, ib_b = 0.f;
        int32_t id_a = 0, id_b = 0;
        stage_seek(t_begin);
        stage_load(t_begin);
        stage_store(0, 0);
        __syncthreads();
        if (t_begin + 1 < t_end) stage_load(t_begin + 1);
        {
#pragma unroll
            for (int t = 0; t < KT; ++t) bcur[t] = btile[0][col][2 * t + half];
            ib_a = ibase[0][col];
            id_a = ipos[0][col];
#pragma unroll
            for (int t = 0; t < KT; ++t) acc_a = __builtin_amdgcn_mfma_f32_32x32x2f32(a[t], bcur[t], acc_a, 0, 0, 0);
        }
        if (t_begin + 1 < t_end) stage_store(1, 1);
        __syncthreads();
        auto step = [&](int64_t it, f32x16 &acc_cur, f32x16 &acc_nxt, float &ib_cur, float &ib_nxt, int32_t &id_cur,
                        int32_t &id_nxt) __attribute__((always_inline)) {
            const int buf_next = (int)((it + 1 - t_begin) & 1);
            load_frags(buf_next, 0);
            __builtin_amdgcn_sched_barrier(0);
            if (it + 2 < t_end && !(ablate & 2)) stage_load(it + 2);
            const int wb1 = wb == 2 ? 0 : wb + 1, wb2 = wb1 == 2 ? 0 : wb1 + 1;
            ib_nxt = ibase[wb1][col];
            id_nxt = ipos[wb1][col];
            const int32_t item = id_cur;
            unsigned long long hm[16];
            float sc[16];
#pragma unroll
            for (int g = 0; g < KT / FG; ++g) {
                if (g + 1 < KT / FG) load_frags(buf_next, g + 1);
                __builtin_amdgcn_sched_barrier(0);
#pragma unroll
                for (int t = g * FG; t < (g + 1) * FG; ++t) {
                    if (t == 0) acc_nxt = __builtin_amdgcn_mfma_f32_32x32x2f32(a[t], bcur[t], zero16, 0, 0, 0);
                    else acc_nxt = __builtin_amdgcn_mfma_f32_32x32x2f32(a[t], bcur[t], acc_nxt, 0, 0, 0);
                    if (t < 16) {
                        const int r = t;
                        sc[r] = UB ? (ib_cur + ubias[r]) + acc_cur[r] : ib_cur + acc_cur[r];
                        hm[r] = __ballot(sc[r] >= thr[r]);
                    }
                }
                __builtin_amdgcn_sched_barrier(0);
            }
            if (KT < 16) {
#pragma unroll
                for (int r = KT; r < 16; ++r) {
                    sc[r] = UB ? (ib_cur + ubias[r]) + acc_cur[r] : ib_cur + acc_cur[r];
                    hm[r] = __ballot(sc[r] >= thr[r]);
                }
            }
            unsigned long long any = 0ull;
#pragma unroll
            for (int r = 0; r < 16; ++r) any |= hm[r];
            if (ablate & 1) any = 0ull;
            auto drop_excluded = [&]() __attribute__((always_inline)) {
                const uint32_t wv = wmask[wb][wave][col];
                unsigned long long left = 0ull;
#pragma unroll
                for (int r = 0; r < 16; ++r) {
                    if (hm[r] != 0ull) {
                        const int rl = (r & 3) + 8 * (r >> 2);
                        const unsigned long long m = (unsigned long long)(uint32_t)__builtin_amdgcn_readlane(wv, rl) |
                                                     ((unsigned long long)(uint32_t)__builtin_amdgcn_readlane(wv, rl + 4) << 32);
                        hm[r] &= ~m;
                        left |= hm[r];
                    }
                }
                return left;
            };
            if (any != 0ull && excl_bits) any = drop_excluded();
            if (any != 0ull) {
                unsigned over_l = 0;
#pragma unroll
                for (int r = 0; r < 16; ++r) {
                    if (hm[r] != 0ull) {
                        const unsigned mine = half ? (unsigned)(hm[r] >> 32) : (unsigned)hm[r];
                        if (cnt_r[r] + __popc(mine) > CAP) over_l |= 1u << ((r & 3) + 8 * (r >> 2) + 4 * half);
                    }
                }
                if ((__builtin_amdgcn_readlane(over_l, 0) | __builtin_amdgcn_readlane(over_l, 32)) != 0u) {
                    compact(over_l);
#pragma unroll
                    for (int r = 0; r < 16; ++r) hm[r] = __ballot(sc[r] >= thr[r]);
                    if (excl_bits) (void)drop_excluded();
                }
#pragma unroll
                for (int r = 0; r < 16; ++r) {
                    const unsigned long long m = hm[r];
                    if (m != 0ull) {
                        const unsigned mine = half ? (unsigned)(m >> 32) : (unsigned)m;
                        if ((mine >> col) & 1u) {
                            const int rl = (r & 3) + 8 * (r >> 2) + 4 * half;
                            const int slot = cnt_r[r] + __popc(mine & ((1u << col) - 1u));
                            keys[wave][rl][slot] =
                                ((unsigned long long)order_key(sc[r]) << 32) | (unsigned long long)(uint32_t)item;
                        }
                        cnt_r[r] += __popc(mine);
                    }
                }
            }
            if (it + 2 < t_end && !(ablate & 8)) stage_store((int)((it + 2 - t_begin) & 1), wb2);
            if (!(ablate & 4)) __syncthreads();
            wb = wb1;
        };
        for (int64_t it = t_begin; it < t_end; it += 2) {
            step(it, acc_a, acc_b, ib_a, ib_b, id_a, id_b);
            if (it + 1 < t_end) step(it + 1, acc_b, acc_a, ib_b, ib_a, id_b, id_a);
        }
        compact(0xffffffffu);
        for (int rl = 0; rl < 32; ++rl) {
            const int64_t row = row_tile * 32 + rl;
            if (row >= n_rows) break;
            if (lane < topk) part[(seg * n_rows + row) * topk + lane] = keys[wave][rl][lane];
        }
        if (t_begin == 0 && t_end < n_item_tiles && lane < 32 && row_tile * 32 + lane < n_rows)
            __hip_atomic_store(tau_pub + row_tile * 32 + lane, tau[wave][lane], __ATOMIC_RELAXED, __HIP_MEMORY_SCOPE_AGENT);
        __builtin_amdgcn_fence(__ATOMIC_ACQ_REL, "wavefront");
        __builtin_amdgcn_wave_barrier();
    }
}

constexpr int kBitmapChunk = 1024;
constexpr int kBitmapRows = 1;
__global__ __launch_bounds__(kBlk) void excl_bitmap_kernel(const int64_t *__restrict__ indptr,
                                                          const int32_t *__restrict__ indices,
                                                          const int32_t *__restrict__ users, int64_t u0, int by_user,
                                                          const int32_t *__restrict__ inv_perm, int64_t n_rows,
                                                          int64_t n_rows_padded, int64_t n_item_tiles,
                                                          uint32_t *__restrict__ bits) {
    constexpr int NR = kBitmapRows;
    __shared__ uint32_t bm_all[kBlk / 64][NR][kBitmapChunk];
    const int wave = threadIdx.x >> 6, lane = threadIdx.x & 63;
    const int64_t row0 = ((int64_t)blockIdx.x * (kBlk / 64) + wave) * NR;
    if (row0 >= n_rows_padded) return;
    int64_t lo[NR], cnt[NR];
    int64_t cnt_max = 0;
#pragma unroll
    for (int q = 0; q < NR; ++q) {
        lo[q] = 0;
        cnt[q] = 0;
        const int64_t row = row0 + q;
        if (row < n_rows) {
            const int64_t key = by_user ? (users ? (int64_t)users[row] : u0 + row) : row;
            lo[q] = indptr[key];
            cnt[q] = indptr[key + 1] - lo[q];
        }
        cnt_max = max(cnt_max, cnt[q]);
    }
    for (int64_t c0 = 0; c0 < n_item_tiles; c0 += kBitmapChunk) {
        const int nt = (int)min((int64_t)kBitmapChunk, n_item_tiles - c0);
#pragma unroll
        for (int q = 0; q < NR; ++q)
            for (int i = lane; i < nt; i += 64) bm_all[wave][q][i] = 0u;
        __builtin_amdgcn_fence(__ATOMIC_ACQ_REL, "wavefront");
        __builtin_amdgcn_wave_barrier();
        for (int64_t p = lane; p < cnt_max; p += 64) {
            int32_t e[NR], pos[NR];
#pragma unroll
            for (int q = 0; q < NR; ++q) e[q] = p < cnt[q] ? indices[lo[q] + p] : 0;
#pragma unroll
            for (int q = 0; q < NR; ++q) pos[q] = inv_perm[e[q]];
#pragma unroll
            for (int q = 0; q < NR; ++q) {
                const int t = (pos[q] >> 5) - (int)c0;
                if (p < cnt[q] && t >= 0 && t < nt) atomicOr(&bm_all[wave][q][t], 1u << (pos[q] & 31));
            }
        }
        __builtin_amdgcn_fence(__ATOMIC_ACQ_REL, "wavefront");
        __builtin_amdgcn_wave_barrier();
#pragma unroll
        for (int q = 0; q < NR; ++q) {
            if (row0 + q < n_rows_padded)
                for (int i = lane; i < nt; i += 64)
                    __builtin_nontemporal_store(bm_all[wave][q][i], &bits[(row0 + q) * n_item_tiles + c0 + i]);
        }
        __builtin_amdgcn_fence(__ATOMIC_ACQ_REL, "wavefront");
        __builtin_amdgcn_wave_barrier();
    }
}

__global__ __launch_bounds__(64) void rank_merge_kernel(const unsigned long long *__restrict__ part, int n_strips,
                                                        int64_t n_rows, int topk, int pad,
                                                        int32_t *__restrict__ items_out,
                                                        float *__restrict__ scores_out) {
    extern __shared__ unsigned long long mlist[];
    const int64_t row = blockIdx.x;
    const int tid = threadIdx.x;
    const int n = n_strips * topk;
    for (int i = tid; i < pad; i += 64) {
        unsigned long long key = 0ull;
        if (i < n) key = part[((int64_t)(i / topk) * n_rows + row) * topk + (i % topk)];
        mlist[i] = key;
    }
    __syncthreads();
    for (int kk = 2; kk <= pad; kk <<= 1) {
        for (int j = kk >> 1; j > 0; j >>= 1) {
            for (int i = tid; i < pad; i += 64) {
                const int ixj = i ^ j;
                if (ixj > i) {
                    const unsigned long long x = mlist[i], y = mlist[ixj];
                    const bool desc = (i & kk) == 0;
                    if (desc ? (x < y) : (x > y)) {
                        mlist[i] = y;
                        mlist[ixj] = x;
                    }
                }
            }
            __syncthreads();
        }
    }
    for (int i = tid; i < topk; i += 64) {
        const unsigned long long key = mlist[i];
        items_out[row * topk + i] = key ? (int32_t)(uint32_t)key : -1;
        scores_out[row * topk + i] = key ? key_to_float((uint32_t)(key >> 32)) : -INFINITY;
    }
}

__global__ __launch_bounds__(kBlk) void mark_excluded_kernel(const int64_t *__restrict__ excl_indptr,
                                                             const int32_t *__restrict__ excl_indices, int64_t row0,
                                                             int64_t n_items, uint8_t *__restrict__ excl_mask) {
    const int64_t row = blockIdx.x;
    const int64_t lo = excl_indptr[row0 + row], hi = excl_indptr[row0 + row + 1];
    for (int64_t p = lo + threadIdx.x; p < hi; p += kBlk) {
        const int32_t it = excl_indices[p];
        if (it >= 0 && it < n_items) excl_mask[row * n_items + it] = 1;
    }
}

__device__ __forceinline__ unsigned long long composite_key(const float *__restrict__ scores,
                                                            const uint8_t *__restrict__ excl, int64_t i) {
    if (excl && excl[i]) return 0ull;
    return ((unsigned long long)order_key(scores[i]) << 32) | (unsigned long long)(uint32_t)i;
}

constexpr int TOPK_MAX = 2048;

__global__ __launch_bounds__(kBlk) void topk_select_kernel(const float *__restrict__ scores,
                                                           const uint8_t *__restrict__ excl_mask, int64_t n_items,
                                                           int topk, int topk_pad, int32_t *__restrict__ items_out,
                                                           float *__restrict__ scores_out) {
    __shared__ unsigned int hist[256];
    __shared__ unsigned long long sh_prefix;
    __shared__ unsigned int sh_remaining, sh_count;
    extern __shared__ unsigned long long list[];
    const int64_t row = blockIdx.x;
    const float *srow = scores + row * n_items;
    const uint8_t *erow = excl_mask ? excl_mask + row * n_items : nullptr;
    const int tid = threadIdx.x;
    if (tid == 0) {
        sh_prefix = 0ull;
        sh_remaining = (unsigned)topk;
        sh_count = 0;
    }
    __syncthreads();
    for (int pass = 0; pass < 8; ++pass) {
        const int shift = 56 - 8 * pass;
        hist[tid] = 0;
        __syncthreads();
        const unsigned long long prefix = sh_prefix;
        for (int64_t i = tid; i < n_items; i += kBlk) {
            const unsigned long long key = composite_key(srow, erow, i);
            const bool match = pass == 0 ? true : ((key >> (shift + 8)) == prefix);
            if (match) atomicAdd(&hist[(unsigned)(key >> shift) & 255u], 1u);
        }
        __syncthreads();
        if (tid == 0) {
            unsigned int rem = sh_remaining, acc = 0;
            int b = 255;
            for (; b > 0; --b) {
                if (acc + hist[b] >= rem) break;
                acc += hist[b];
            }
            sh_remaining = rem - acc;
            sh_prefix = (prefix << 8) | (unsigned long long)b;
        }
        __syncthreads();
    }
    const unsigned long long thresh = sh_prefix;
    for (int i = tid; i < topk_pad; i += kBlk) list[i] = 0ull;
    __syncthreads();
    for (int64_t i = tid; i < n_items; i += kBlk) {
        const unsigned long long key = composite_key(srow, erow, i);
        if (key >= thresh && key != 0ull) {
            const unsigned int pos = atomicAdd(&sh_count, 1u);
            if (pos < (unsigned)topk_pad) list[pos] = key;
        }
    }
    __syncthreads();
    for (int kk = 2; kk <= topk_pad; kk <<= 1) {
        for (int j = kk >> 1; j > 0; j >>= 1) {
            for (int i = tid; i < topk_pad; i += kBlk) {
                const int ixj = i ^ j;
                if (ixj > i) {
                    const unsigned long long x = list[i], y = list[ixj];
                    const bool desc = (i & kk) == 0;
                    if (desc ? (x < y) : (x > y)) {
                        list[i] = y;
                        list[ixj] = x;
                    }
                }
            }
            __syncthreads();
        }
    }
    for (int i = tid; i < topk; i += kBlk) {
        const unsigned long long key = list[i];
        items_out[row * topk + i] = key ? (int32_t)(uint32_t)key : -1;
        scores_out[row * topk + i] = key ? key_to_float((uint32_t)(key >> 32)) : -INFINITY;
    }
}

constexpr int kSortBlk = 1024;
constexpr int kSortChunk = 8192;
__global__ __launch_bounds__(kSortBlk) void full_sort_kernel(const float *__restrict__ scores,
                                                             const uint8_t *__restrict__ excl_mask, int64_t n_items,
                                                             int64_t n_pad, unsigned long long *__restrict__ scratch,
                                                             int topk, int32_t *__restrict__ items_out,
                                                             float *__restrict__ scores_out) {
    __shared__ unsigned long long lk[kSortChunk];
    const int64_t row = blockIdx.x;
    const float *srow = scores + row * n_items;
    const uint8_t *erow = excl_mask ? excl_mask + row * n_items : nullptr;
    unsigned long long *keys = scratch + row * n_pad;
    const int tid = threadIdx.x;
    const int64_t ch = n_pad < kSortChunk ? n_pad : kSortChunk;
    auto lds_stages = [&](int64_t c0, int64_t kk, int64_t j_hi) {
        for (int64_t j = j_hi; j > 0; j >>= 1) {
            for (int64_t p = tid; p < (ch >> 1); p += kSortBlk) {
                const int64_t i = ((p & ~(j - 1)) << 1) | (p & (j - 1)), ixj = i | j;
                const unsigned long long x = lk[i], y = lk[ixj];
                const bool desc = ((c0 + i) & kk) == 0;
                if (desc ? (x < y) : (x > y)) {
                    lk[i] = y;
                    lk[ixj] = x;
                }
            }
            __syncthreads();
        }
    };
    for (int64_t c0 = 0; c0 < n_pad; c0 += ch) {
        for (int64_t i = tid; i < ch; i += kSortBlk) {
            const int64_t g = c0 + i;
            lk[i] = g < n_items ? composite_key(srow, erow, g) : 0ull;
        }
        __syncthreads();
        for (int64_t kk = 2; kk <= ch; kk <<= 1) lds_stages(c0, kk, kk >> 1);
        for (int64_t i = tid; i < ch; i += kSortBlk) keys[c0 + i] = lk[i];
        __syncthreads();
    }
    for (int64_t kk = ch << 1; kk <= n_pad; kk <<= 1) {
        for (int64_t j = kk >> 1; j >= ch; j >>= 1) {
            for (int64_t p = tid; p < (n_pad >> 1); p += kSortBlk) {
                const int64_t i = ((p & ~(j - 1)) << 1) | (p & (j - 1)), ixj = i | j;
                const unsigned long long x = keys[i], y = keys[ixj];
                const bool desc = (i & kk) == 0;
                if (desc ? (x < y) : (x > y)) {
                    keys[i] = y;
                    keys[ixj] = x;
                }
            }
            __syncthreads();
        }
        for (int64_t c0 = 0; c0 < n_pad; c0 += ch) {
            for (int64_t i = tid; i < ch; i += kSortBlk) lk[i] = keys[c0 + i];
            __syncthreads();
            lds_stages(c0, kk, ch >> 1);
            for (int64_t i = tid; i < ch; i += kSortBlk) keys[c0 + i] = lk[i];
            __syncthreads();
        }
    }
    for (int64_t i = tid; i < topk; i += kSortBlk) {
        const unsigned long long key = keys[i];
        items_out[row * topk + i] = key ? (int32_t)(uint32_t)key : -1;
        scores_out[row * topk + i] = key ? key_to_float((uint32_t)(key >> 32)) : -INFINITY;
    }
}


constexpr int kPosT = 8;
__global__ __launch_bounds__(kBlk) void rank_positions_kernel(const float *__restrict__ scores,
                                                              const uint8_t *__restrict__ excl_mask, int64_t n_items,
                                                              const int64_t *__restrict__ tgt_indptr,
                                                              const int32_t *__restrict__ tgt_indices, int64_t row0,
                                                              int32_t *__restrict__ greater_out,
                                                              int32_t *__restrict__ pos_out,
                                                              int32_t *__restrict__ ge_out,
                                                              float *__restrict__ score_out) {
    const int64_t row = blockIdx.x;
    const float *srow = scores + row * n_items;
    const uint8_t *erow = excl_mask ? excl_mask + row * n_items : nullptr;
    const int64_t lo = tgt_indptr[row0 + row], hi = tgt_indptr[row0 + row + 1];
    __shared__ int cnt[kPosT * 3];
    const int64_t mis = (int64_t)((reinterpret_cast<uintptr_t>(srow) >> 2) & 3);
    const int64_t head = min(n_items, (4 - mis) & 3);
    const int64_t body_end = head + ((n_items - head) & ~int64_t(3));
    const bool vec_mask = !erow || ((reinterpret_cast<uintptr_t>(erow) + head) & 3) == 0;
    for (int64_t t0 = lo; t0 < hi; t0 += kPosT) {
        uint32_t ts[kPosT];
        bool ok[kPosT];
        int32_t titem[kPosT];
#pragma unroll
        for (int q = 0; q < kPosT; ++q) {
            const int64_t t = t0 + q;
            const int32_t item = t < hi ? tgt_indices[t] : -1;
            ok[q] = item >= 0 && item < n_items && !(erow && erow[item]);
            ts[q] = ok[q] ? order_key(srow[item]) : 0xFFFFFFFFu;
            titem[q] = item;
        }
        int g[kPosT], eq[kPosT], tie[kPosT];
#pragma unroll
        for (int q = 0; q < kPosT; ++q) g[q] = eq[q] = tie[q] = 0;
        auto visit = [&](const bool *live, const float *sc, int64_t i, int n) __attribute__((always_inline)) {
            uint32_t oc[4];
            unsigned long long any_eq = 0;
#pragma unroll
            for (int c = 0; c < n; ++c) {
                oc[c] = live[c] ? order_key(sc[c]) : 0u;
#pragma unroll
                for (int q = 0; q < kPosT; ++q) {
                    g[q] += oc[c] > ts[q];
                    any_eq |= __ballot(oc[c] == ts[q]);
                }
            }
            if (any_eq) {
#pragma unroll
                for (int c = 0; c < n; ++c) {
                    asm volatile("" : "+v"(oc[c]));
#pragma unroll
                    for (int q = 0; q < kPosT; ++q) {
                        const bool same = live[c] && oc[c] == ts[q];
                        eq[q] += same;
                        tie[q] += same && (uint32_t)(i + c) > (uint32_t)titem[q];
                    }
                }
            }
        };
        for (int64_t i = threadIdx.x; i < head; i += kBlk) {
            const bool lv = !(erow && erow[i]);
            const float sc = srow[i];
            visit(&lv, &sc, i, 1);
        }
        auto fetch = [&](int64_t i0, v4f32 &sv, uint32_t &em) __attribute__((always_inline)) {
            const bool in = i0 < body_end;
            sv = in ? *reinterpret_cast<const v4f32 *>(srow + i0) : v4f32{0.f, 0.f, 0.f, 0.f};
            em = 0u;
            if (erow && in) {
                if (vec_mask) em = *reinterpret_cast<const uint32_t *>(erow + i0);
                else em = (uint32_t)erow[i0] | ((uint32_t)erow[i0 + 1] << 8) | ((uint32_t)erow[i0 + 2] << 16) | ((uint32_t)erow[i0 + 3] << 24);
            }
        };
        const int64_t i_first = head + 4 * (int64_t)threadIdx.x, i_stop = body_end + 4 * (int64_t)(kBlk - 1);
        v4f32 sv_n = {0.f, 0.f, 0.f, 0.f};
        uint32_t em_n = 0u;
        if (i_first < i_stop) fetch(i_first, sv_n, em_n);
        for (int64_t i0 = i_first; i0 < i_stop; i0 += 4 * kBlk) {
            const v4f32 sv = sv_n;
            const uint32_t em = em_n;
            if (i0 + 4 * kBlk < i_stop) fetch(i0 + 4 * kBlk, sv_n, em_n);
            const bool in = i0 < body_end;
            const bool lv[4] = {in && !(em & 0xffu), in && !(em & 0xff00u), in && !(em & 0xff0000u), in && !(em & 0xff000000u)};
            const float sc[4] = {sv.x, sv.y, sv.z, sv.w};
            visit(lv, sc, i0, 4);
        }
        for (int64_t i = body_end + threadIdx.x; i < n_items; i += kBlk) {
            const bool lv = !(erow && erow[i]);
            const float sc = srow[i];
            visit(&lv, &sc, i, 1);
        }
#pragma unroll
        for (int q = 0; q < kPosT; ++q)
            for (int o = 32; o > 0; o >>= 1) {
                g[q] += __shfl_xor(g[q], o, 64);
                eq[q] += __shfl_xor(eq[q], o, 64);
                tie[q] += __shfl_xor(tie[q], o, 64);
            }
        if (threadIdx.x < kPosT * 3) cnt[threadIdx.x] = 0;
        __syncthreads();
        if ((threadIdx.x & 63) == 0) {
#pragma unroll
            for (int q = 0; q < kPosT; ++q) {
                atomicAdd(&cnt[q * 3 + 0], g[q]);
                atomicAdd(&cnt[q * 3 + 1], g[q] + tie[q]);
                atomicAdd(&cnt[q * 3 + 2], g[q] + eq[q]);
            }
        }
        __syncthreads();
#pragma unroll
        for (int q = 0; q < kPosT; ++q) {
            const int64_t t = t0 + q;
            if (threadIdx.x == q && t < hi) {
                greater_out[t] = ok[q] ? cnt[q * 3 + 0] : -1;
                pos_out[t] = ok[q] ? cnt[q * 3 + 1] : -1;
                ge_out[t] = ok[q] ? cnt[q * 3 + 2] : -1;
                score_out[t] = ok[q] ? srow[titem[q]] : -INFINITY;
            }
        }
        __syncthreads();
    }
}

}

using namespace chip;

struct cornac_hip_scorer {
    int device = 0;
    int64_t n_users = 0, n_items = 0;
    int k = 0;
    int ld = 0;
    hipStream_t stream = nullptr;
    DevBuf<float> U, V, item_base, user_base;
    DevBuf<float> Vr, ibr;
    DevBuf<int32_t> perm, inv_perm;
    DevBuf<uint32_t> excl_bits;
    void *pinned_out = nullptr;
    size_t pinned_bytes = 0;
    std::vector<void *> pinned_retired;
    DevBuf<int64_t> res_excl_indptr;
    DevBuf<int32_t> res_excl_indices;
    bool has_res_excl = false;
    DevBuf<float> tau_pub;
    bool has_user_base = false, is_set = false;
    DevBuf<float> scores;
    DevBuf<uint8_t> excl;
    DevBuf<int32_t> d_users, d_items_out, d_excl_indices;
    DevBuf<int64_t> d_excl_indptr;
    DevBuf<float> d_scores_out;
    DevBuf<int64_t> d_tgt_indptr;
    DevBuf<int32_t> d_tgt_indices, d_tgt_counts;
    DevBuf<float> d_tgt_scores;
    DevBuf<unsigned long long> sort_scratch, part;
    DevBuf<double> U64, V64, ib64, ub64, scores64;
    bool f64_set = false, f64_user_base = false;
};

static __global__ __launch_bounds__(256) void permute_rows_kernel(const float *__restrict__ V, const float *__restrict__ ib,
                                                                  const int32_t *__restrict__ perm, int64_t n, int ld,
                                                                  float *__restrict__ Vr, float *__restrict__ ibr) {
    const int gl = threadIdx.x & 15;
    for (int64_t p = ((int64_t)blockIdx.x * 256 + threadIdx.x) >> 4; p < n; p += ((int64_t)gridDim.x * 256) >> 4) {
        const int64_t src = perm[p];
        for (int f = gl * 4; f < ld; f += 64)
            *reinterpret_cast<v4f32 *>(Vr + p * ld + f) = *reinterpret_cast<const v4f32 *>(V + src * ld + f);
        if (gl == 0) ibr[p] = ib[src];
    }
}

static void build_rank_order(cornac_hip_scorer_t h, const float *U, const float *V, const float *item_base) {
    const int64_t ni = h->n_items, nu = h->n_users;
    const int k = h->k;
    const int64_t sample = std::min<int64_t>(nu, 16384), stride = std::max<int64_t>(1, nu / sample);
    const bool full_cov = (double)ni * k * k <= 4e9;
    std::vector<double> mean((size_t)k, 0.0), cov(full_cov ? (size_t)k * k : 0, 0.0);
    double ss = 0;
    int64_t cnt = 0;
    for (int64_t u = 0; u < nu; u += stride, ++cnt) {
        const float *ur = U + u * k;
        for (int f = 0; f < k; ++f) {
            mean[(size_t)f] += ur[f];
            ss += (double)ur[f] * ur[f];
        }
        if (full_cov)
            for (int f = 0; f < k; ++f)
                for (int g = f; g < k; ++g) cov[(size_t)f * k + g] += (double)ur[f] * ur[g];
    }
    const double inv = 1.0 / (double)std::max<int64_t>(cnt, 1);
    for (int f = 0; f < k; ++f) mean[(size_t)f] *= inv;
    if (full_cov)
        for (int f = 0; f < k; ++f)
            for (int g = f; g < k; ++g) {
                const double c = cov[(size_t)f * k + g] * inv - mean[(size_t)f] * mean[(size_t)g];
                cov[(size_t)f * k + g] = cov[(size_t)g * k + f] = c;
            }
    const double iso = std::max(0.0, ss * inv - [&] { double m2 = 0; for (int f = 0; f < k; ++f) m2 += mean[(size_t)f] * mean[(size_t)f]; return m2; }()) / (double)k;
    std::vector<float> pri((size_t)ni);
    std::vector<double> tmp((size_t)k);
    for (int64_t i = 0; i < ni; ++i) {
        const float *vr = V + i * k;
        double m = 0, var = 0;
        for (int f = 0; f < k; ++f) m += mean[(size_t)f] * vr[f];
        if (full_cov) {
            for (int f = 0; f < k; ++f) {
                double t = 0;
                for (int g = 0; g < k; ++g) t += cov[(size_t)f * k + g] * vr[g];
                var += t * vr[f];
            }
        } else {
            for (int f = 0; f < k; ++f) var += (double)vr[f] * vr[f];
            var *= iso;
        }
        pri[(size_t)i] = (float)((item_base ? (double)item_base[i] : 0.0) + m + 2.0 * std::sqrt(std::max(var, 0.0)));
    }
    std::vector<int32_t> order((size_t)ni);
    for (int64_t i = 0; i < ni; ++i) order[(size_t)i] = (int32_t)i;
    std::stable_sort(order.begin(), order.end(), [&](int32_t a, int32_t b) {
        const float pa = pri[(size_t)a], pb = pri[(size_t)b];
        return (pa > pb) || (pa != pa && pb == pb);
    });
    const int64_t ni_pad = (ni + 31) / 32 * 32;
    h->perm.ensure((size_t)ni_pad);
    h->Vr.ensure((size_t)ni_pad * h->ld);
    h->ibr.ensure((size_t)ni_pad);
    HIP_CHECK(hipMemsetAsync(h->perm.p, 0, (size_t)ni_pad * sizeof(int32_t), h->stream));
    HIP_CHECK(hipMemsetAsync(h->Vr.p, 0, (size_t)ni_pad * h->ld * sizeof(float), h->stream));
    HIP_CHECK(hipMemsetD32Async((hipDeviceptr_t)h->ibr.p, 0x7fc00000u , (size_t)ni_pad, h->stream));
    h->perm.upload(order.data(), (size_t)ni, h->stream);
    std::vector<int32_t> inv_order((size_t)ni);
    for (int64_t p = 0; p < ni; ++p) inv_order[(size_t)order[(size_t)p]] = (int32_t)p;
    h->inv_perm.ensure((size_t)ni);
    h->inv_perm.upload(inv_order.data(), (size_t)ni, h->stream);
    const unsigned grid = (unsigned)std::max<int64_t>(1, std::min<int64_t>((ni * 16 + 255) / 256, 8192));
    hipLaunchKernelGGL(permute_rows_kernel, dim3(grid), dim3(256), 0, h->stream, h->V.p, h->item_base.p, h->perm.p, ni, h->ld,
                       h->Vr.p, h->ibr.p);
    HIP_CHECK(hipGetLastError());
    HIP_CHECK(hipStreamSynchronize(h->stream));
}

static void validate_csr(const int64_t *indptr, const int32_t *indices, int64_t n, int64_t n_items, const char *what) {
    REQUIRE(indptr[0] == 0, "%s_indptr must start at 0", what);
    for (int64_t r = 0; r < n; ++r)
        REQUIRE(indptr[r + 1] >= indptr[r], "%s_indptr decreases at row %lld", what, (long long)r);
    const int64_t ne = indptr[n];
    int32_t lo = 0, hi = 0;
    for (int64_t p = 0; p < ne; ++p) {
        lo = std::min(lo, indices[p]);
        hi = std::max(hi, indices[p]);
    }
    REQUIRE(lo >= 0 && hi < n_items, "%s_indices out of range [0, %lld)", what, (long long)n_items);
}

static void sc_check(cornac_hip_scorer_t h, bool need_set = true) {
    REQUIRE(h != nullptr, "scorer handle is NULL");
    HIP_CHECK(hipSetDevice(h->device));
    if (need_set) REQUIRE(h->is_set, "cornac_hip_scorer_set has not been called");
}

static int64_t rows_per_batch(cornac_hip_scorer_t h) {
    const int64_t cap = (int64_t(2) << 30) / (h->n_items * (int64_t)sizeof(float));
    return std::max<int64_t>(32, std::min<int64_t>(cap / 32 * 32, 16384));
}

static void launch_scores(cornac_hip_scorer_t h, const int32_t *d_users, int64_t u0, int64_t n, bool use_mfma) {
    const float *ub = h->has_user_base ? h->user_base.p : nullptr;
    const int k = h->k;
    if (use_mfma && k <= 128) {
        const int64_t n_item_tiles = (h->n_items + 31) / 32;
        const DeviceInfo &di = device_info(h->device);
        auto go = [&](auto kernel, int MT) {
            const int64_t row_tiles = (n + 31) / 32;
            const int64_t wg_rows = (row_tiles + (int64_t)MT * 4 - 1) / ((int64_t)MT * 4);
            int64_t strips = std::max<int64_t>(1, ((int64_t)di.cus * 8 + wg_rows - 1) / wg_rows);
            strips = std::min(strips, n_item_tiles);
            const int tiles_per_strip = (int)((n_item_tiles + strips - 1) / strips);
            const int64_t gx = (n_item_tiles + tiles_per_strip - 1) / tiles_per_strip;
            hipLaunchKernelGGL(kernel, dim3((unsigned)gx, (unsigned)wg_rows), dim3(kBlk), 0, h->stream, h->U.p, h->V.p,
                               h->item_base.p, ub, d_users, u0, n, h->n_items, k, tiles_per_strip, h->scores.p);
        };
        if (h->ld == 16) go(score_gemm_mfma_kernel<8, 2>, 2);
        else if (h->ld == 32) go(score_gemm_mfma_kernel<16, 2>, 2);
        else if (h->ld == 64) go(score_gemm_mfma_kernel<32, 2>, 2);
        else go(score_gemm_mfma_kernel<64, 1>, 1);
    } else {
        dim3 grid((unsigned)((h->n_items + kBlk - 1) / kBlk), (unsigned)n);
        hipLaunchKernelGGL(score_valu_kernel, grid, dim3(kBlk), (size_t)k * sizeof(float), h->stream, h->U.p, h->V.p,
                           h->item_base.p, ub, d_users, u0, h->n_items, k, h->ld, h->scores.p);
    }
    HIP_CHECK(hipGetLastError());
}

static void launch_rank(cornac_hip_scorer_t h, int64_t n, int topk, bool have_excl, int32_t *items_out,
                        float *scores_out) {
    const uint8_t *excl = have_excl ? h->excl.p : nullptr;
    if (topk <= TOPK_MAX) {
        int pad = 1;
        while (pad < topk) pad <<= 1;
        hipLaunchKernelGGL(topk_select_kernel, dim3((unsigned)n), dim3(kBlk), (size_t)pad * 8, h->stream, h->scores.p,
                           excl, h->n_items, topk, pad, items_out, scores_out);
    } else {
        int64_t pad = 1;
        while (pad < h->n_items) pad <<= 1;
        h->sort_scratch.ensure((size_t)(n * pad));
        hipLaunchKernelGGL(full_sort_kernel, dim3((unsigned)n), dim3(kSortBlk), 0, h->stream, h->scores.p, excl,
                           h->n_items, pad, h->sort_scratch.p, topk, items_out, scores_out);
    }
    HIP_CHECK(hipGetLastError());
}

constexpr int kFusedMaxTopk = 32;

static bool can_fuse(cornac_hip_scorer_t h, int topk) { return topk <= kFusedMaxTopk && h->k <= 128; }

constexpr int64_t kMaxBitmapTiles = 8192;

static void launch_rank_fused_rows(cornac_hip_scorer_t h, const int32_t *d_users, int64_t u0, int64_t n, int topk,
                                   const int64_t *d_excl_indptr, const int32_t *d_excl_indices, int64_t excl_row0,
                                   int32_t *items_out, float *scores_out, bool excl_by_user) {
    const float *ub = h->has_user_base ? h->user_base.p : nullptr;
    const DeviceInfo &di = device_info(h->device);
    const int ablate = prof_env_int("CORNAC_HIP_RANK_ABLATE", 0);
    const int64_t n_item_tiles = (h->n_items + 31) / 32;
    const int64_t wg_rows = (n + 127) / 128;
    const int wgs_per_cu = (h->ld <= 64 || topk <= 10) ? 2 : 1;
    const int64_t work_total = wg_rows * n_item_tiles;
    int64_t work_per_wg = std::max<int64_t>((work_total + (int64_t)di.cus * wgs_per_cu - 1) / ((int64_t)di.cus * wgs_per_cu),
                                            std::min<int64_t>(16, n_item_tiles));
    const int64_t n_wgs = (work_total + work_per_wg - 1) / work_per_wg;
    const int64_t max_segs = (n_item_tiles + work_per_wg - 1) / work_per_wg + 1;
    h->part.ensure((size_t)(max_segs * n * topk));
    HIP_CHECK(hipMemsetAsync(h->part.p, 0, (size_t)(max_segs * n * topk) * sizeof(unsigned long long), h->stream));
    h->tau_pub.ensure((size_t)n);
    HIP_CHECK(hipMemsetD32Async((hipDeviceptr_t)h->tau_pub.p, 0xff800000u , (size_t)n, h->stream));
    const uint32_t *d_bits = nullptr;
    const bool no_bitmap = prof_env_set("CORNAC_HIP_RANK_NO_BITMAP");
    if (d_excl_indptr && n_item_tiles <= kMaxBitmapTiles && !no_bitmap) {
        const int64_t rows_padded = wg_rows * 128;
        h->excl_bits.ensure((size_t)(rows_padded * n_item_tiles));
        hipLaunchKernelGGL(excl_bitmap_kernel, dim3((unsigned)((rows_padded + kBitmapRows * (kBlk / 64) - 1) / (kBitmapRows * (kBlk / 64)))), dim3(kBlk), 0,
                           h->stream, d_excl_indptr + (excl_by_user ? 0 : excl_row0), d_excl_indices, d_users, u0,
                           excl_by_user ? 1 : 0, h->inv_perm.p, n, rows_padded, n_item_tiles, h->excl_bits.p);
        d_bits = h->excl_bits.p;
    } else if (d_excl_indptr) {
        REQUIRE(!excl_by_user, "resident exclusion lists need the bitmap path (catalogue too large)");
    }
    dim3 grid((unsigned)n_wgs), block(kBlk);
#define FUSED(KT_, CAP_) do {                                                                                    \
    if (prof_env_set("CORNAC_HIP_RANK_ABLATE")) {                                                                 \
        int occ = 0;                                                                                              \
        (void)hipOccupancyMaxActiveBlocksPerMultiprocessor(&occ, rank_fused_kernel<KT_, CAP_, true>, kBlk, 0);     \
        fprintf(stderr, "[rank_fused<%d,%d>] %u workgroups x %lld block-tiles, <= %lld segments/row, %d workgroups/CU\n", \
                KT_, CAP_, grid.x, (long long)work_per_wg, (long long)max_segs, occ);                              \
    }                                                                                                             \
    if (ub)                                                                                                       \
        hipLaunchKernelGGL((rank_fused_kernel<KT_, CAP_, true>), grid, block, 0, h->stream, h->U.p, h->Vr.p,       \
                           h->ibr.p, ub, d_users, u0, n, h->n_items, work_per_wg, topk, d_bits ? nullptr : d_excl_indptr, \
                           d_excl_indices, excl_row0, d_bits, h->perm.p, h->tau_pub.p, h->part.p, ablate);       \
    else                                                                                                          \
        hipLaunchKernelGGL((rank_fused_kernel<KT_, CAP_, false>), grid, block, 0, h->stream, h->U.p, h->Vr.p,      \
                           h->ibr.p, ub, d_users, u0, n, h->n_items, work_per_wg, topk, d_bits ? nullptr : d_excl_indptr, \
                           d_excl_indices, excl_row0, d_bits, h->perm.p, h->tau_pub.p, h->part.p, ablate); } while (0)
    if (topk <= 10 && h->ld == 128) {
        FUSED(64, 42);
    } else if (topk <= 24) {
        if (h->ld == 16) FUSED(8, 56);
        else if (h->ld == 32) FUSED(16, 56);
        else if (h->ld == 64) FUSED(32, 56);
        else FUSED(64, 56);
    } else {
        if (h->ld == 16) FUSED(8, 64);
        else if (h->ld == 32) FUSED(16, 64);
        else if (h->ld == 64) FUSED(32, 64);
        else FUSED(64, 64);
    }
#undef FUSED
    int pad = 1;
    while (pad < (int)max_segs * topk) pad <<= 1;
    hipLaunchKernelGGL(rank_merge_kernel, dim3((unsigned)n), dim3(64), (size_t)pad * 8, h->stream, h->part.p,
                       (int)max_segs, n, topk, pad, items_out, scores_out);
    HIP_CHECK(hipGetLastError());
}

constexpr int64_t kExclBitmapBudget = int64_t(512) << 20;
static void launch_rank_fused(cornac_hip_scorer_t h, const int32_t *d_users, int64_t u0, int64_t n, int topk,
                              const int64_t *d_excl_indptr, const int32_t *d_excl_indices, int64_t excl_row0,
                              int32_t *items_out, float *scores_out, bool excl_by_user = false) {
    const int64_t n_item_tiles = (h->n_items + 31) / 32;
    int64_t rows = n;
    if (d_excl_indptr && n_item_tiles <= kMaxBitmapTiles)
        rows = std::max<int64_t>(128, (kExclBitmapBudget / (n_item_tiles * 4)) / 128 * 128);
    for (int64_t r0 = 0; r0 < n; r0 += rows) {
        const int64_t m = std::min(rows, n - r0);
        launch_rank_fused_rows(h, d_users ? d_users + r0 : nullptr, u0 + r0, m, topk, d_excl_indptr, d_excl_indices,
                               excl_row0 + r0, items_out + r0 * topk, scores_out ? scores_out + r0 * topk : nullptr,
                               excl_by_user);
    }
}

extern "C" {

int cornac_hip_scorer_create(cornac_hip_scorer_t *out, int device, int64_t n_users, int64_t n_items, int k) {
    return guarded([&] {
        REQUIRE(out != nullptr, "out handle pointer is NULL");
        *out = nullptr;
        REQUIRE(n_users > 0 && n_items > 0 && k > 0, "n_users, n_items and k must be positive");
        REQUIRE(n_items < (int64_t(1) << 31), "n_items exceeds int32");
        use_device(device);
        std::unique_ptr<cornac_hip_scorer> h(new cornac_hip_scorer());
        h->device = device; h->n_users = n_users; h->n_items = n_items; h->k = k;
        h->ld = k <= 16 ? 16 : k <= 32 ? 32 : k <= 64 ? 64 : k <= 128 ? 128 : k;
        HIP_CHECK(hipStreamCreateWithFlags(&h->stream, hipStreamNonBlocking));
        h->U.alloc((size_t)n_users * h->ld);
        h->V.alloc((size_t)n_items * h->ld);
        HIP_CHECK(hipMemsetAsync(h->U.p, 0, h->U.n * sizeof(float), h->stream));
        HIP_CHECK(hipMemsetAsync(h->V.p, 0, h->V.n * sizeof(float), h->stream));
        HIP_CHECK(hipStreamSynchronize(h->stream));
        h->item_base.alloc((size_t)n_items);
        h->user_base.alloc((size_t)n_users);
        *out = h.release();
    });
}

int cornac_hip_scorer_destroy(cornac_hip_scorer_t h) {
    return guarded([&] {
        if (!h) return;
        (void)hipSetDevice(h->device);
        if (h->stream) {
            (void)hipStreamSynchronize(h->stream);
            (void)hipStreamDestroy(h->stream);
        }
        if (h->pinned_out) (void)hipHostFree(h->pinned_out);
        for (void *q : h->pinned_retired) (void)hipHostFree(q);
        delete h;
    });
}

int cornac_hip_scorer_set(cornac_hip_scorer_t h, const float *U, const float *V, const float *item_base,
                          const float *user_base) {
    return guarded([&] {
        sc_check(h, false);
        REQUIRE(U && V, "U and V are required");
        HIP_CHECK(hipMemcpy2DAsync(h->U.p, (size_t)h->ld * 4, U, (size_t)h->k * 4, (size_t)h->k * 4, (size_t)h->n_users,
                                   hipMemcpyHostToDevice, h->stream));
        HIP_CHECK(hipMemcpy2DAsync(h->V.p, (size_t)h->ld * 4, V, (size_t)h->k * 4, (size_t)h->k * 4, (size_t)h->n_items,
                                   hipMemcpyHostToDevice, h->stream));
        if (item_base) h->item_base.upload(item_base, (size_t)h->n_items, h->stream);
        else HIP_CHECK(hipMemsetAsync(h->item_base.p, 0, (size_t)h->n_items * 4, h->stream));
        h->has_user_base = user_base != nullptr;
        if (user_base) h->user_base.upload(user_base, (size_t)h->n_users, h->stream);
        build_rank_order(h, U, V, item_base);
        HIP_CHECK(hipStreamSynchronize(h->stream));
        h->is_set = true;
    });
}

int cornac_hip_score_user(cornac_hip_scorer_t h, int64_t user, float *out) {
    return guarded([&] {
        sc_check(h);
        REQUIRE(user >= 0 && user < h->n_users, "user %lld out of range", (long long)user);
        REQUIRE(out != nullptr, "out is NULL");
        h->scores.ensure((size_t)h->n_items);
        launch_scores(h, nullptr, user, 1, false);
        h->scores.download(out, (size_t)h->n_items, h->stream);
        HIP_CHECK(hipStreamSynchronize(h->stream));
    });
}

namespace chip {
__global__ __launch_bounds__(256) void score_user_f64_kernel(const double *__restrict__ u, const double *__restrict__ V,
                                                             const double *__restrict__ item_base, double user_base,
                                                             int64_t n_items, int k, double *__restrict__ out) {
    const int64_t i = (int64_t)blockIdx.x * 256 + threadIdx.x;
    if (i >= n_items) return;
    double acc = 0.0;
    const double *v = V + i * k;
    for (int f = 0; f < k; ++f) acc = acc + u[f] * v[f];
    out[i] = (item_base ? item_base[i] : 0.0) + user_base + acc;
}
}

int cornac_hip_scorer_set_f64(cornac_hip_scorer_t h, const double *U, const double *V, const double *item_base,
                              const double *user_base) {
    return guarded([&] {
        sc_check(h, false);
        REQUIRE(U && V, "U and V are required");
        h->U64.ensure((size_t)h->n_users * h->k);
        h->V64.ensure((size_t)h->n_items * h->k);
        h->U64.upload(U, (size_t)h->n_users * h->k, h->stream);
        h->V64.upload(V, (size_t)h->n_items * h->k, h->stream);
        h->ib64.ensure((size_t)h->n_items);
        if (item_base) h->ib64.upload(item_base, (size_t)h->n_items, h->stream);
        else HIP_CHECK(hipMemsetAsync(h->ib64.p, 0, (size_t)h->n_items * sizeof(double), h->stream));
        h->f64_user_base = user_base != nullptr;
        if (user_base) {
            h->ub64.ensure((size_t)h->n_users);
            h->ub64.upload(user_base, (size_t)h->n_users, h->stream);
        }
        h->scores64.ensure((size_t)h->n_items);
        HIP_CHECK(hipStreamSynchronize(h->stream));
        h->f64_set = true;
    });
}

int cornac_hip_score_user_f64(cornac_hip_scorer_t h, int64_t user, double *out) {
    return guarded([&] {
        sc_check(h, false);
        REQUIRE(h->f64_set, "no float64 tables (cornac_hip_scorer_set_f64)");
        REQUIRE(user >= 0 && user < h->n_users, "user %lld out of range", (long long)user);
        REQUIRE(out != nullptr, "out is NULL");
        double ub = 0.0;
        if (h->f64_user_base) HIP_CHECK(hipMemcpyAsync(&ub, h->ub64.p + user, sizeof ub, hipMemcpyDeviceToHost, h->stream));
        if (h->f64_user_base) HIP_CHECK(hipStreamSynchronize(h->stream));
        hipLaunchKernelGGL(score_user_f64_kernel, dim3((unsigned)((h->n_items + 255) / 256)), dim3(256), 0, h->stream,
                           h->U64.p + (size_t)user * h->k, h->V64.p, h->ib64.p, ub, h->n_items, h->k, h->scores64.p);
        HIP_CHECK(hipGetLastError());
        h->scores64.download(out, (size_t)h->n_items, h->stream);
        HIP_CHECK(hipStreamSynchronize(h->stream));
    });
}

int cornac_hip_score_block(cornac_hip_scorer_t h, const int32_t *users, int64_t n, float *out) {
    return guarded([&] {
        sc_check(h);
        REQUIRE(users && out && n > 0, "bad arguments");
        for (int64_t b = 0; b < n; ++b)
            REQUIRE(users[b] >= 0 && users[b] < h->n_users, "user %d out of range", users[b]);
        const int64_t cap = rows_per_batch(h);
        h->scores.ensure((size_t)(std::min(cap, n) * h->n_items));
        h->d_users.ensure((size_t)std::min(cap, n));
        for (int64_t b0 = 0; b0 < n; b0 += cap) {
            const int64_t nb = std::min(cap, n - b0);
            h->d_users.upload(users + b0, (size_t)nb, h->stream);
            launch_scores(h, h->d_users.p, 0, nb, true);
            h->scores.download(out + b0 * h->n_items, (size_t)(nb * h->n_items), h->stream);
            HIP_CHECK(hipStreamSynchronize(h->stream));
        }
    });
}

int cornac_hip_rank_topk(cornac_hip_scorer_t h, const int32_t *users, int64_t n, int topk, const int64_t *excl_indptr,
                         const int32_t *excl_indices, int32_t *items_out, float *scores_out) {
    return guarded([&] {
        sc_check(h);
        REQUIRE(users && items_out && scores_out && n > 0, "bad arguments");
        REQUIRE(topk >= 1 && topk <= h->n_items, "topk must be in [1, n_items]");
        for (int64_t b = 0; b < n; ++b)
            REQUIRE(users[b] >= 0 && users[b] < h->n_users, "user %d out of range", users[b]);
        const bool have_excl = excl_indptr != nullptr && excl_indices != nullptr;
        if (have_excl) {
            validate_csr(excl_indptr, excl_indices, n, h->n_items, "excl");
            h->d_excl_indptr.ensure((size_t)n + 1);
            h->d_excl_indptr.upload(excl_indptr, (size_t)n + 1, h->stream);
            const int64_t ne = excl_indptr[n];
            h->d_excl_indices.ensure((size_t)std::max<int64_t>(ne, 1));
            if (ne > 0) h->d_excl_indices.upload(excl_indices, (size_t)ne, h->stream);
        }
        if (can_fuse(h, topk)) {
            if (have_excl && (h->n_items + 31) / 32 > kMaxBitmapTiles)
                for (int64_t b = 0; b < n; ++b)
                    for (int64_t p = excl_indptr[b] + 1; p < excl_indptr[b + 1]; ++p)
                        REQUIRE(excl_indices[p] > excl_indices[p - 1], "exclusion row %lld is not strictly sorted",
                                (long long)b);
            h->d_users.ensure((size_t)n);
            h->d_items_out.ensure((size_t)(n * topk));
            h->d_scores_out.ensure((size_t)(n * topk));
            h->d_users.upload(users, (size_t)n, h->stream);
            launch_rank_fused(h, h->d_users.p, 0, n, topk, have_excl ? h->d_excl_indptr.p : nullptr,
                              have_excl ? h->d_excl_indices.p : nullptr, 0, h->d_items_out.p, h->d_scores_out.p);
            h->d_items_out.download(items_out, (size_t)(n * topk), h->stream);
            h->d_scores_out.download(scores_out, (size_t)(n * topk), h->stream);
            HIP_CHECK(hipStreamSynchronize(h->stream));
            return;
        }
        int64_t cap = rows_per_batch(h);
        if (topk > TOPK_MAX) cap = std::min<int64_t>(cap, 1024);
        const int64_t nb_max = std::min(cap, n);
        h->scores.ensure((size_t)(nb_max * h->n_items));
        h->d_users.ensure((size_t)nb_max);
        h->d_items_out.ensure((size_t)(nb_max * topk));
        h->d_scores_out.ensure((size_t)(nb_max * topk));
        if (have_excl) h->excl.ensure((size_t)(nb_max * h->n_items));
        for (int64_t b0 = 0; b0 < n; b0 += cap) {
            const int64_t nb = std::min(cap, n - b0);
            h->d_users.upload(users + b0, (size_t)nb, h->stream);
            launch_scores(h, h->d_users.p, 0, nb, true);
            if (have_excl) {
                HIP_CHECK(hipMemsetAsync(h->excl.p, 0, (size_t)(nb * h->n_items), h->stream));
                hipLaunchKernelGGL(mark_excluded_kernel, dim3((unsigned)nb), dim3(kBlk), 0, h->stream,
                                   h->d_excl_indptr.p, h->d_excl_indices.p, b0, h->n_items, h->excl.p);
            }
            launch_rank(h, nb, topk, have_excl, h->d_items_out.p, h->d_scores_out.p);
            h->d_items_out.download(items_out + b0 * topk, (size_t)(nb * topk), h->stream);
            h->d_scores_out.download(scores_out + b0 * topk, (size_t)(nb * topk), h->stream);
            HIP_CHECK(hipStreamSynchronize(h->stream));
        }
    });
}

int cornac_hip_rank_positions(cornac_hip_scorer_t h, const int32_t *users, int64_t n, const int64_t *excl_indptr,
                              const int32_t *excl_indices, const int64_t *tgt_indptr, const int32_t *tgt_indices,
                              int32_t *greater_out, int32_t *pos_out, int32_t *ge_out, float *tgt_scores_out) {
    return guarded([&] {
        sc_check(h);
        REQUIRE(users && tgt_indptr && n > 0, "bad arguments");
        REQUIRE(tgt_indptr[0] == 0, "tgt_indptr must start at 0");
        for (int64_t b = 0; b < n; ++b) {
            REQUIRE(users[b] >= 0 && users[b] < h->n_users, "user %d out of range", users[b]);
            REQUIRE(tgt_indptr[b + 1] >= tgt_indptr[b], "tgt_indptr must not decrease");
        }
        const int64_t nt = tgt_indptr[n];
        if (nt == 0) return;
        REQUIRE(tgt_indices && greater_out && pos_out && ge_out && tgt_scores_out, "bad arguments");
        const bool have_excl = excl_indptr != nullptr && excl_indices != nullptr;
        if (have_excl) {
            validate_csr(excl_indptr, excl_indices, n, h->n_items, "excl");
            h->d_excl_indptr.ensure((size_t)n + 1);
            h->d_excl_indptr.upload(excl_indptr, (size_t)n + 1, h->stream);
            const int64_t ne = excl_indptr[n];
            h->d_excl_indices.ensure((size_t)std::max<int64_t>(ne, 1));
            if (ne > 0) h->d_excl_indices.upload(excl_indices, (size_t)ne, h->stream);
        }
        h->d_tgt_indptr.ensure((size_t)n + 1);
        h->d_tgt_indptr.upload(tgt_indptr, (size_t)n + 1, h->stream);
        h->d_tgt_indices.ensure((size_t)nt);
        h->d_tgt_indices.upload(tgt_indices, (size_t)nt, h->stream);
        h->d_tgt_counts.ensure((size_t)(3 * nt));
        h->d_tgt_scores.ensure((size_t)nt);
        const int64_t cap = rows_per_batch(h);
        const int64_t nb_max = std::min(cap, n);
        h->scores.ensure((size_t)(nb_max * h->n_items));
        h->d_users.ensure((size_t)nb_max);
        if (have_excl) h->excl.ensure((size_t)(nb_max * h->n_items));
        for (int64_t b0 = 0; b0 < n; b0 += cap) {
            const int64_t nb = std::min(cap, n - b0);
            h->d_users.upload(users + b0, (size_t)nb, h->stream);
            launch_scores(h, h->d_users.p, 0, nb, true);
            if (have_excl) {
                HIP_CHECK(hipMemsetAsync(h->excl.p, 0, (size_t)(nb * h->n_items), h->stream));
                hipLaunchKernelGGL(mark_excluded_kernel, dim3((unsigned)nb), dim3(kBlk), 0, h->stream,
                                   h->d_excl_indptr.p, h->d_excl_indices.p, b0, h->n_items, h->excl.p);
            }
            hipLaunchKernelGGL(rank_positions_kernel, dim3((unsigned)nb), dim3(kBlk), 0, h->stream, h->scores.p,
                               have_excl ? h->excl.p : nullptr, h->n_items, h->d_tgt_indptr.p, h->d_tgt_indices.p, b0,
                               h->d_tgt_counts.p, h->d_tgt_counts.p + nt, h->d_tgt_counts.p + 2 * nt,
                               h->d_tgt_scores.p);
            HIP_CHECK(hipGetLastError());
            HIP_CHECK(hipStreamSynchronize(h->stream));
        }
        HIP_CHECK(hipMemcpyAsync(greater_out, h->d_tgt_counts.p, (size_t)nt * 4, hipMemcpyDeviceToHost, h->stream));
        HIP_CHECK(hipMemcpyAsync(pos_out, h->d_tgt_counts.p + nt, (size_t)nt * 4, hipMemcpyDeviceToHost, h->stream));
        HIP_CHECK(hipMemcpyAsync(ge_out, h->d_tgt_counts.p + 2 * nt, (size_t)nt * 4, hipMemcpyDeviceToHost, h->stream));
        h->d_tgt_scores.download(tgt_scores_out, (size_t)nt, h->stream);
        HIP_CHECK(hipStreamSynchronize(h->stream));
    });
}

int cornac_hip_score_pairs(cornac_hip_scorer_t h, const int32_t *users, const int32_t *items, int64_t n, int clip,
                           float lo, float hi, float *out) {
    return guarded([&] {
        sc_check(h);
        REQUIRE(users && items && out && n > 0, "bad arguments");
        for (int64_t p = 0; p < n; ++p)
            REQUIRE(users[p] >= 0 && users[p] < h->n_users && items[p] >= 0 && items[p] < h->n_items,
                    "pair %lld is out of range", (long long)p);
        DevBuf<int32_t> du, di;
        DevBuf<float> dout;
        du.alloc((size_t)n);
        di.alloc((size_t)n);
        dout.alloc((size_t)n);
        du.upload(users, (size_t)n, h->stream);
        di.upload(items, (size_t)n, h->stream);
        hipLaunchKernelGGL(score_pairs_kernel, dim3((unsigned)((n + kBlk - 1) / kBlk)), dim3(kBlk), 0, h->stream,
                           h->U.p, h->V.p, h->item_base.p, h->has_user_base ? h->user_base.p : nullptr, du.p, di.p, n,
                           h->k, h->ld, clip, lo, hi, dout.p);
        HIP_CHECK(hipGetLastError());
        dout.download(out, (size_t)n, h->stream);
        HIP_CHECK(hipStreamSynchronize(h->stream));
    });
}

int cornac_hip_scorer_set_exclusions(cornac_hip_scorer_t h, const int64_t *indptr, const int32_t *indices) {
    return guarded([&] {
        sc_check(h, false);
        if (!indptr) {
            h->has_res_excl = false;
            return;
        }
        REQUIRE(indices != nullptr || indptr[h->n_users] == 0, "indices is NULL");
        validate_csr(indptr, indices, h->n_users, h->n_items, "excl");
        const int64_t ne = indptr[h->n_users];
        h->res_excl_indptr.ensure((size_t)h->n_users + 1);
        h->res_excl_indices.ensure((size_t)std::max<int64_t>(ne, 1));
        h->res_excl_indptr.upload(indptr, (size_t)h->n_users + 1, h->stream);
        if (ne > 0) h->res_excl_indices.upload(indices, (size_t)ne, h->stream);
        HIP_CHECK(hipStreamSynchronize(h->stream));
        h->has_res_excl = true;
    });
}

int cornac_hip_rank_topk_resident(cornac_hip_scorer_t h, const int32_t *users, int64_t u0, int64_t n, int topk,
                                  int32_t *items_out, float *scores_out, double *device_ms) {
    return guarded([&] {
        sc_check(h);
        REQUIRE(h->has_res_excl, "cornac_hip_scorer_set_exclusions has not been called");
        REQUIRE(n > 0 && topk >= 1 && topk <= h->n_items, "bad arguments");
        REQUIRE(can_fuse(h, topk) && (h->n_items + 31) / 32 <= kMaxBitmapTiles,
                "resident exclusion lists serve the fused top-k path (topk <= 32, k <= 128, <= 262144 items)");
        if (users) {
            for (int64_t b = 0; b < n; ++b) REQUIRE(users[b] >= 0 && users[b] < h->n_users, "user %d out of range", users[b]);
            h->d_users.ensure((size_t)n);
            h->d_users.upload(users, (size_t)n, h->stream);
        } else {
            REQUIRE(u0 >= 0 && u0 + n <= h->n_users, "user range out of bounds");
        }
        h->d_items_out.ensure((size_t)(n * topk));
        h->d_scores_out.ensure((size_t)(n * topk));
        hipEvent_t e0 = nullptr, e1 = nullptr;
        if (device_ms) {
            HIP_CHECK(hipEventCreate(&e0));
            HIP_CHECK(hipEventCreate(&e1));
            HIP_CHECK(hipEventRecord(e0, h->stream));
        }
        launch_rank_fused(h, users ? h->d_users.p : nullptr, u0, n, topk, h->res_excl_indptr.p, h->res_excl_indices.p, 0,
                          h->d_items_out.p, h->d_scores_out.p, true);
        if (device_ms) HIP_CHECK(hipEventRecord(e1, h->stream));
        if (items_out) h->d_items_out.download(items_out, (size_t)(n * topk), h->stream);
        if (scores_out) h->d_scores_out.download(scores_out, (size_t)(n * topk), h->stream);
        HIP_CHECK(hipStreamSynchronize(h->stream));
        if (device_ms) {
            float t = 0.f;
            HIP_CHECK(hipEventElapsedTime(&t, e0, e1));
            (void)hipEventDestroy(e0);
            (void)hipEventDestroy(e1);
            *device_ms = (double)t;
        }
    });
}

int cornac_hip_scorer_host_buffer(cornac_hip_scorer_t h, size_t bytes, void **out) {
    return guarded([&] {
        sc_check(h);
        REQUIRE(out != nullptr, "out is NULL");
        if (bytes > h->pinned_bytes) {
            if (h->pinned_out) h->pinned_retired.push_back(h->pinned_out);
            h->pinned_out = nullptr;
            const size_t want = std::max(bytes, 2 * h->pinned_bytes);
            h->pinned_bytes = 0;
            HIP_CHECK(hipHostMalloc(&h->pinned_out, want, hipHostMallocDefault));
            h->pinned_bytes = want;
        }
        *out = h->pinned_out;
    });
}

int cornac_hip_rank_topk_device(cornac_hip_scorer_t h, int64_t u0, int64_t n, int topk, int repeats, double *ms) {
    return guarded([&] {
        sc_check(h);
        REQUIRE(u0 >= 0 && n > 0 && u0 + n <= h->n_users, "user range out of bounds");
        REQUIRE(topk >= 1 && topk <= h->n_items, "topk out of range");
        REQUIRE(repeats >= 1 && ms, "bad arguments");
        const bool fused = can_fuse(h, topk);
        const int64_t cap = fused ? n : rows_per_batch(h);
        const int64_t nb_max = std::min(cap, n);
        if (!fused) h->scores.ensure((size_t)(nb_max * h->n_items));
        if (!fused && topk > TOPK_MAX) {
            int64_t pad = 1;
            while (pad < h->n_items) pad <<= 1;
            h->sort_scratch.ensure((size_t)(nb_max * pad));
        }
        h->d_items_out.ensure((size_t)(nb_max * topk));
        h->d_scores_out.ensure((size_t)(nb_max * topk));
        hipEvent_t e0, e1;
        HIP_CHECK(hipEventCreate(&e0));
        HIP_CHECK(hipEventCreate(&e1));
        HIP_CHECK(hipEventRecord(e0, h->stream));
        for (int r = 0; r < repeats; ++r) {
            for (int64_t b0 = 0; b0 < n; b0 += cap) {
                const int64_t nb = std::min(cap, n - b0);
                if (fused) {
                    launch_rank_fused(h, nullptr, u0 + b0, nb, topk, nullptr, nullptr, 0, h->d_items_out.p,
                                      h->d_scores_out.p);
                } else {
                    launch_scores(h, nullptr, u0 + b0, nb, true);
                    launch_rank(h, nb, topk, false, h->d_items_out.p, h->d_scores_out.p);
                }
            }
        }
        HIP_CHECK(hipEventRecord(e1, h->stream));
        HIP_CHECK(hipEventSynchronize(e1));
        float t = 0.f;
        HIP_CHECK(hipEventElapsedTime(&t, e0, e1));
        (void)hipEventDestroy(e0);
        (void)hipEventDestroy(e1);
        *ms = (double)t;
    });
}
}
```

### include/cornac_hip.h

```cpp
#ifndef CORNAC_HIP_H_
#define CORNAC_HIP_H_

#include <stdint.h>

#ifdef __cplusplus
extern "C" {
#endif

#define CORNAC_HIP_OK 0
#define CORNAC_HIP_ERR_INVALID 1
#define CORNAC_HIP_ERR_HIP 2
#define CORNAC_HIP_ERR_NO_DEVICE 3
#define CORNAC_HIP_ERR_UNSUPPORTED 4

#define CORNAC_HIP_MODE_DETERMINISTIC 0
#define CORNAC_HIP_MODE_HOGWILD 1

#define CORNAC_HIP_NEG_UNIFORM 0
#define CORNAC_HIP_NEG_POPULARITY 1

const char *cornac_hip_last_error(void);
const char *cornac_hip_version(void);
int cornac_hip_device_count(int *count);
int cornac_hip_device_info(int device, char *name, int name_len, int *compute_units, int64_t *hbm_bytes);
int cornac_hip_device_probe(int device, int64_t bytes, double *out3);

typedef struct cornac_hip_bpr *cornac_hip_bpr_t;

int cornac_hip_bpr_create(cornac_hip_bpr_t *out, int device, int64_t n_users, int64_t n_items,
                          int64_t total_users, int64_t total_items, int k, const int32_t *indptr,
                          const int32_t *indices, int64_t nnz);
int cornac_hip_bpr_destroy(cornac_hip_bpr_t h);

int cornac_hip_bpr_set_factors(cornac_hip_bpr_t h, const float *U, const float *V, const float *B);
int cornac_hip_bpr_get_factors(cornac_hip_bpr_t h, float *U, float *V, float *B);

int cornac_hip_bpr_set_factors_f64(cornac_hip_bpr_t h, const double *U, const double *V, const double *B);
int cornac_hip_bpr_get_factors_f64(cornac_hip_bpr_t h, double *U, double *V, double *B);
int cornac_hip_bpr_fit_epochs_f64(cornac_hip_bpr_t h, int n_epochs, double lr, double reg, int use_bias, int neg_population,
                                  int64_t *correct, int64_t *skipped);

int cornac_hip_bpr_bind_device(cornac_hip_bpr_t h, float *dU, float *dV, float *dB);
int cornac_hip_bpr_device_ptrs(cornac_hip_bpr_t h, float **dU, float **dV, float **dB);
int cornac_hip_bpr_rebind_items(cornac_hip_bpr_t h, float *dV, float *dB);
int cornac_hip_bpr_set_stream(cornac_hip_bpr_t h, void *hip_stream);
int cornac_hip_bpr_switch_stream(cornac_hip_bpr_t h, void *hip_stream);

int cornac_hip_bpr_seed_mt19937(cornac_hip_bpr_t h, uint32_t mt_seed_pos, uint32_t mt_seed_neg, int shared_stream);
int cornac_hip_bpr_seed_hogwild(cornac_hip_bpr_t h, uint64_t seed);

int cornac_hip_bpr_set_negative_population(cornac_hip_bpr_t h, const int32_t *items, int64_t n);

#define CORNAC_HIP_HOG_PLAIN_STORES 1
#define CORNAC_HIP_HOG_VEC4_LAYOUT 2
#define CORNAC_HIP_HOG_NO_OWNERSHIP 4
#define CORNAC_HIP_HOG_DENSE_BIAS 8
#define CORNAC_HIP_HOG_SHARE_NEG 16
#define CORNAC_HIP_HOG_BINNED 64
#define CORNAC_HIP_HOG_FUSED_OPT_OUT 128
#define CORNAC_HIP_HOG_ABLATE_MASK 0xff00
#define CORNAC_HIP_HOG_ABLATE_SHIFT 8
#define CORNAC_HIP_HOG_FORM_MASK 0xf0000
#define CORNAC_HIP_HOG_FORM_SHIFT 16
#define CORNAC_HIP_FORM_AUTO (0 << CORNAC_HIP_HOG_FORM_SHIFT)
#define CORNAC_HIP_FORM_FUSED (1 << CORNAC_HIP_HOG_FORM_SHIFT)
#define CORNAC_HIP_FORM_STRATA (2 << CORNAC_HIP_HOG_FORM_SHIFT)
#define CORNAC_HIP_FORM_LDSBIN (3 << CORNAC_HIP_HOG_FORM_SHIFT)

int cornac_hip_bpr_fit_epochs(cornac_hip_bpr_t h, int n_epochs, float lr, float reg, int use_bias, int neg_population,
                              int mode, int hogwild_flags, int64_t *correct, int64_t *skipped);
int cornac_hip_bpr_hogwild_enqueue(cornac_hip_bpr_t h, int64_t n_samples, float lr, float reg, int use_bias,
                                   int neg_population, int hogwild_flags);
int cornac_hip_bpr_sync(cornac_hip_bpr_t h, int64_t *correct, int64_t *skipped);

int cornac_hip_bpr_debug_draw(cornac_hip_bpr_t h, int stream, uint64_t hi, int64_t n, int64_t *out);
int cornac_hip_bpr_debug_ownership(cornac_hip_bpr_t h, int64_t *n_waves, int64_t *wave_ptr, int32_t *own_u,
                                   int32_t *own_i);
int cornac_hip_bpr_strata_config(cornac_hip_bpr_t h, int hot_permille, int hot_min_mult_x100, int rehash_period);
int cornac_hip_bpr_chunk_records(cornac_hip_bpr_t h, int enable);
int cornac_hip_bpr_strata_stats(cornac_hip_bpr_t h, int64_t *out4);
int cornac_hip_bpr_debug_strata(cornac_hip_bpr_t h, uint32_t epoch, int64_t *sptr, int32_t *rec_u, int32_t *rec_i,
                                int32_t *rank_item, uint32_t *key);
int cornac_hip_bpr_ldsbin_config(cornac_hip_bpr_t h, int hot_x1000, int min_candidates, int max_rounds);
int cornac_hip_bpr_ldsbin_pass_config(cornac_hip_bpr_t h, int enable, int waves, int lds_kb, int min_draws_x100);
int cornac_hip_bpr_ldsbin_stats(cornac_hip_bpr_t h, int64_t *out8);
int cornac_hip_bpr_ldsbin_deal_config(cornac_hip_bpr_t h, int strata_groups, int hot_cost_x16);
int cornac_hip_bpr_debug_ldsbin_deal(cornac_hip_bpr_t h, uint64_t seed, uint32_t epoch, int32_t *bin_of_item,
                                     uint32_t *cold_mass, uint32_t *hot_off, int32_t *hot_u, int32_t *hot_i);
int cornac_hip_bpr_kernel_timing(cornac_hip_bpr_t h, int enable, double *total_ms, int64_t *launches);
int cornac_hip_bpr_last_timing(cornac_hip_bpr_t h, double *ms4);

int cornac_hip_bpr_sample_triplets(cornac_hip_bpr_t h, int64_t n_draws, int neg_population, int32_t *d_u,
                                   int32_t *d_i, int32_t *d_j);
int cornac_hip_bpr_apply_triplets(cornac_hip_bpr_t h, const int32_t *d_u, const int32_t *d_slot_i,
                                  const int32_t *d_slot_j, int64_t n, float *d_rows, float *d_bias, int bias_stride,
                                  float lr, float reg, int use_bias);
int cornac_hip_bpr_staged_slots(cornac_hip_bpr_t h, int64_t n_draws, int64_t *n_slots);
int cornac_hip_bpr_emit_triplets(cornac_hip_bpr_t h, int64_t n_draws, int neg_population, int32_t *d_u, int32_t *d_i,
                                 int32_t *d_j, int64_t slots_cap, int64_t *n_slots);
int cornac_hip_bpr_apply_staged(cornac_hip_bpr_t h, const int32_t *d_u, const int32_t *d_slot_i, const int32_t *d_slot_j,
                                int64_t n_slots, float *d_rows, float *d_bias, int bias_stride, float lr, float reg,
                                int use_bias);
int cornac_hip_bpr_shard_mark(cornac_hip_bpr_t h, const int32_t *d_i, const int32_t *d_j, int64_t n, int world,
                              int64_t rows_per_rank, int32_t *d_mark);
int cornac_hip_bpr_shard_slots(cornac_hip_bpr_t h, const int32_t *d_i, const int32_t *d_j, int64_t n, int world,
                               int64_t rows_per_rank, const int32_t *d_scan, int32_t *d_slot_i, int32_t *d_slot_j);
int cornac_hip_bpr_shard_uniq(cornac_hip_bpr_t h, const int32_t *d_mark, const int32_t *d_scan, int64_t n_rows,
                              int64_t rows_per_rank, int32_t *d_uniq_local);
int cornac_hip_bpr_scatter_diff_rows(cornac_hip_bpr_t h, float *d_table, const int32_t *d_ids, int64_t n, int width,
                                     const float *d_now, const float *d_before, const float *d_scale);
int cornac_hip_bpr_gather_rows(cornac_hip_bpr_t h, const float *d_table, const int32_t *d_ids, int64_t n, int width,
                               float *d_out);
int cornac_hip_bpr_scatter_add_rows(cornac_hip_bpr_t h, float *d_table, const int32_t *d_ids, int64_t n, int width,
                                    const float *d_delta);
int cornac_hip_bpr_table_delta_begin(cornac_hip_bpr_t h, const float *d_flat, const float *d_base, int64_t n_items,
                                     int k, float *d_bucket, float *d_local);
int cornac_hip_bpr_table_delta_finish(cornac_hip_bpr_t h, float *d_flat, float *d_base, const float *d_bucket,
                                      const float *d_local, int64_t n_items, int k);
int cornac_hip_bpr_table_delta_step(cornac_hip_bpr_t h, float *d_flat, float *d_base, const float *d_bucket_prev,
                                    const float *d_local_prev, int64_t n_items, int k, float *d_bucket, float *d_local);
int cornac_hip_bpr_table_delta(cornac_hip_bpr_t h, int op, int rule, float *d_flat, float *d_base, const float *d_bucket_prev,
                               const float *d_local_prev, int64_t n_items, int k, float *d_bucket, float *d_local);
int cornac_hip_table_delta(int op, int device, void *hip_stream, float *d_flat, float *d_base, const float *d_bucket_prev,
                           const float *d_local_prev, int64_t n_items, int k, float *d_bucket, float *d_local);
int cornac_hip_bpr_resident_exchange_bins(cornac_hip_bpr_t h, int neg_population, int hogwild_flags, int *n_bins);
int cornac_hip_bpr_epoch_resident_enqueue(cornac_hip_bpr_t h, float lr, float reg, int use_bias, int neg_population,
                                          int hogwild_flags, int n_exchanges, int rule, float *d_base, float *d_buckets,
                                          int64_t bucket_stride, float *d_keeps, int64_t keep_stride, uint32_t *d_arrive,
                                          const uint32_t *d_landed, uint32_t *d_applied, int *n_arrivals);
int cornac_hip_bpr_resident_flush(cornac_hip_bpr_t h, int n_exchanges, int rule, float *d_base, const float *d_buckets,
                                  int64_t bucket_stride, const float *d_keeps, int64_t keep_stride,
                                  const uint32_t *d_applied, const uint32_t *d_landed);
int cornac_hip_bpr_conveyor_setup(cornac_hip_bpr_t h, int n_blocks, const int32_t *rank_item, uint64_t deal_seed,
                                  int release_item_tables, int *n_bins, int *bins_per_block, int *cap);
int cornac_hip_bpr_conveyor_layout(cornac_hip_bpr_t h, uint32_t layout_epoch, int32_t *d_slot_item, int32_t *d_item_slot);
int cornac_hip_bpr_conveyor_enqueue(cornac_hip_bpr_t h, uint32_t epoch, uint32_t layout_epoch, int n_ranges,
                                    const int32_t *first_block, float *const *d_rows, float lr, float reg, int use_bias,
                                    int neg_population, int hogwild_flags);
int cornac_hip_stream_wait_counter(int device, void *hip_stream, const uint32_t *d_counter, uint32_t target,
                                   uint32_t *d_error, int timeout_ms);
int cornac_hip_stream_set_flag(int device, void *hip_stream, uint32_t *d_flag, uint32_t value, const uint32_t *d_unless);
int cornac_hip_stream_ring_standin(int device, void *hip_stream, const float *d_src, int64_t src_floats, float *d_dst,
                                   int64_t dst_floats, int64_t n_floats, int n_workgroups);

int cornac_hip_bpr_set_views(cornac_hip_bpr_t h, const int32_t *view_indptr, const int32_t *view_indices,
                             int64_t nnz_view);
int cornac_hip_bpr_seed_view_stream(cornac_hip_bpr_t h, uint32_t mt_seed_view);
int cornac_hip_vebpr_fit_epochs(cornac_hip_bpr_t h, int n_epochs, float lr, float reg, float alpha, int mode,
                                int64_t *correct, int64_t *skipped);
int cornac_hip_vebpr_fit_epochs_f64(cornac_hip_bpr_t h, int n_epochs, double lr, double reg, double alpha, int64_t *correct,
                                    int64_t *skipped);
#define CORNAC_HIP_VEBPR_NO_OWNERSHIP 0x100
int cornac_hip_vebpr_hogwild_form(cornac_hip_bpr_t h, int *owned);

int cornac_hip_mmmf_fit_epochs(cornac_hip_bpr_t h, int n_epochs, float lr, float reg, int mode, int64_t *correct,
                               int64_t *skipped);
int cornac_hip_mmmf_fit_epochs_f64(cornac_hip_bpr_t h, int n_epochs, double lr, double reg, int64_t *correct,
                                   int64_t *skipped);
int cornac_hip_mmmf_hogwild_enqueue(cornac_hip_bpr_t h, int64_t n_samples, float lr, float reg);

typedef struct cornac_hip_mf *cornac_hip_mf_t;

int cornac_hip_mf_create(cornac_hip_mf_t *out, int device, int64_t n_users, int64_t n_items, int k,
                         const int64_t *rid, const int64_t *cid, const float *val, int64_t nnz);
int cornac_hip_mf_destroy(cornac_hip_mf_t h);
int cornac_hip_mf_set_factors(cornac_hip_mf_t h, const float *U, const float *V, const float *Bu, const float *Bi);
int cornac_hip_mf_get_factors(cornac_hip_mf_t h, float *U, float *V, float *Bu, float *Bi);
int cornac_hip_mf_fit(cornac_hip_mf_t h, int max_iter, float lr, float reg, float mu, int use_bias, int early_stop,
                      int mode, float *loss_per_epoch, int *epochs_run);
int cornac_hip_mf_hogwild_form(cornac_hip_mf_t h, int form);
int cornac_hip_mf_hogwild_stats(cornac_hip_mf_t h, int64_t *out4);
int cornac_hip_mf_debug_split(cornac_hip_mf_t h, int64_t *n_split, int64_t *n_virtual, int32_t *split_item, int32_t *split_ptr);
int cornac_hip_mf_debug_ownership(cornac_hip_mf_t h, int64_t *n_waves, int64_t *wave_ptr, int32_t *own_u, int32_t *own_i);
int cornac_hip_mf_fit_sgd(int device, const int64_t *rid, const int64_t *cid, const float *val, int64_t nnz, float *U,
                          float *V, float *Bu, float *Bi, int64_t n_users, int64_t n_items, int k, float lr, float reg,
                          float mu, int max_iter, int use_bias, int early_stop, int mode, float *loss_per_epoch,
                          int *epochs_run);
int cornac_hip_mf_bind_items(cornac_hip_mf_t h, float *dV, float *dBi);
int cornac_hip_mf_bind_users(cornac_hip_mf_t h, float *dU, float *dBu);
int cornac_hip_mf_set_stream(cornac_hip_mf_t h, void *hip_stream);
int cornac_hip_mf_epoch_enqueue(cornac_hip_mf_t h, int part, int n_parts, float lr, float reg, float mu, int use_bias);
int cornac_hip_mf_sync(cornac_hip_mf_t h, double *sq_err_sum);
int cornac_hip_mf_kernel_timing(cornac_hip_mf_t h, int enable, double *total_ms, int64_t *launches);
int cornac_hip_mf_last_timing(cornac_hip_mf_t h, double *ms4);

#define CORNAC_HIP_PMF_LINEAR 0
#define CORNAC_HIP_PMF_NON_LINEAR 1
int cornac_hip_mf_pmf_set_factors(cornac_hip_mf_t h, const double *U, const double *V);
int cornac_hip_mf_pmf_get_factors(cornac_hip_mf_t h, double *U, double *V);
int cornac_hip_mf_pmf_fit(cornac_hip_mf_t h, int n_epochs, float lr, float reg, float gamma, int variant, double *loss_per_epoch);
int cornac_hip_mf_pmf_form(cornac_hip_mf_t h, int *form, int *group);

int cornac_hip_mf_nmf_set_factors(cornac_hip_mf_t h, const float *U, const float *V, const float *Bu, const float *Bi);
int cornac_hip_mf_nmf_get_factors(cornac_hip_mf_t h, float *U, float *V, float *Bu, float *Bi);
int cornac_hip_mf_nmf_fit(cornac_hip_mf_t h, int n_epochs, float lr, float lambda_u, float lambda_v, float lambda_bu,
                          float lambda_bi, float mu, int use_bias, int mode, double *loss_per_epoch);
int cornac_hip_mf_nmf_form(cornac_hip_mf_t h, int *sum_form, int *bias_form, int *rows_split);

int cornac_hip_mf_hpf_set_tables(cornac_hip_mf_t h, const double *G_s, const double *G_r, const double *L_s, const double *L_r);
int cornac_hip_mf_hpf_get_tables(cornac_hip_mf_t h, double *G_s, double *G_r, double *L_s, double *L_r, double *K_r, double *T_r);
int cornac_hip_mf_hpf_fit(cornac_hip_mf_t h, int n_iters, int hierarchical);
int cornac_hip_mf_hpf_elog(cornac_hip_mf_t h, double *Lt, double *Lb);
int cornac_hip_mf_hpf_form(cornac_hip_mf_t h, int *group, int *rows_split);

#define CORNAC_HIP_OPT_SGD 0
#define CORNAC_HIP_OPT_ADAM 1
#define CORNAC_HIP_OPT_RMSPROP 2
#define CORNAC_HIP_OPT_ADAGRAD 3
int cornac_hip_mf_fit_minibatch(cornac_hip_mf_t h, const int64_t *order, int64_t n_total, int batch_size,
                                int optimizer, float lr, float reg, float mu, int use_bias, double *loss_sum);
int cornac_hip_mf_fit_minibatch_dropout(cornac_hip_mf_t h, const int64_t *order, int64_t n_total, int batch_size,
                                        int optimizer, float lr, float reg, float mu, int use_bias, const uint8_t *keep_u,
                                        const uint8_t *keep_i, float keep_scale, double *loss_sum);
int cornac_hip_mf_reset_optimizer(cornac_hip_mf_t h);

typedef struct cornac_hip_vbpr *cornac_hip_vbpr_t;

int cornac_hip_vbpr_create(cornac_hip_vbpr_t *out, int device, int64_t n_users, int64_t n_items, int k, int k2,
                           int n_feat, const float *features);
int cornac_hip_vbpr_destroy(cornac_hip_vbpr_t h);
int cornac_hip_vbpr_set_params(cornac_hip_vbpr_t h, const float *Bi, const float *Gu, const float *Gi, const float *Tu,
                               const float *E, const float *Bp);
int cornac_hip_vbpr_get_params(cornac_hip_vbpr_t h, float *Bi, float *Gu, float *Gi, float *Tu, float *E, float *Bp);
int cornac_hip_vbpr_fit_batches(cornac_hip_vbpr_t h, const int32_t *u, const int32_t *i, const int32_t *j,
                                int64_t n_total, int batch_size, float lr, float lambda_w, float lambda_b,
                                float lambda_e, double *sum_nll);
int cornac_hip_vbpr_item_tables(cornac_hip_vbpr_t h, float *theta_item, float *visual_bias);

typedef struct cornac_hip_wmf *cornac_hip_wmf_t;

int cornac_hip_wmf_create(cornac_hip_wmf_t *out, int device, int64_t n_users, int64_t n_items, int k,
                          const int64_t *csc_indptr, const int32_t *csc_rows, const float *csc_vals, int64_t nnz);
void cornac_hip_wmf_destroy(cornac_hip_wmf_t h);
int cornac_hip_wmf_set_factors(cornac_hip_wmf_t h, const float *U, const float *V);
int cornac_hip_wmf_get_factors(cornac_hip_wmf_t h, float *U, float *V);
int cornac_hip_wmf_fit_batches(cornac_hip_wmf_t h, const int32_t *item_ids, const int64_t *batch_ptr,
                               int64_t n_batches, float lambda_u, float lambda_v, float a, float b,
                               float learning_rate, double *loss_out);
int cornac_hip_wmf_kernel_timing(cornac_hip_wmf_t h, int enabled);
int cornac_hip_wmf_last_timing(cornac_hip_wmf_t h, double *device_ms);

typedef struct cornac_hip_scorer *cornac_hip_scorer_t;

int cornac_hip_scorer_set_exclusions(cornac_hip_scorer_t h, const int64_t *indptr, const int32_t *indices);
int cornac_hip_scorer_host_buffer(cornac_hip_scorer_t h, size_t bytes, void **out);
int cornac_hip_rank_topk_resident(cornac_hip_scorer_t h, const int32_t *users, int64_t u0, int64_t n, int topk,
                                  int32_t *items_out, float *scores_out, double *device_ms);

int cornac_hip_scorer_create(cornac_hip_scorer_t *out, int device, int64_t n_users, int64_t n_items, int k);
int cornac_hip_scorer_destroy(cornac_hip_scorer_t h);
int cornac_hip_scorer_set(cornac_hip_scorer_t h, const float *U, const float *V, const float *item_base,
                          const float *user_base);
int cornac_hip_score_user(cornac_hip_scorer_t h, int64_t user, float *out);
int cornac_hip_scorer_set_f64(cornac_hip_scorer_t h, const double *U, const double *V, const double *item_base,
                              const double *user_base);
int cornac_hip_score_user_f64(cornac_hip_scorer_t h, int64_t user, double *out);
int cornac_hip_score_block(cornac_hip_scorer_t h, const int32_t *users, int64_t n, float *out);
int cornac_hip_score_pairs(cornac_hip_scorer_t h, const int32_t *users, const int32_t *items, int64_t n, int clip,
                           float lo, float hi, float *out);
int cornac_hip_rank_topk(cornac_hip_scorer_t h, const int32_t *users, int64_t n, int topk, const int64_t *excl_indptr,
                         const int32_t *excl_indices, int32_t *items_out, float *scores_out);
int cornac_hip_rank_positions(cornac_hip_scorer_t h, const int32_t *users, int64_t n, const int64_t *excl_indptr,
                              const int32_t *excl_indices, const int64_t *tgt_indptr, const int32_t *tgt_indices,
                              int32_t *greater_out, int32_t *pos_out, int32_t *ge_out, float *tgt_scores_out);
int cornac_hip_rank_topk_device(cornac_hip_scorer_t h, int64_t u0, int64_t n, int topk, int repeats, double *ms);

#ifdef __cplusplus
}
#endif
#endif
```

Baseline: 3.431 billion.

## Add bf16 split-precision MFMA filter to fused top-k ranking with fp32 fallback

Adds a filtered variant of the fused rank kernel that scores items with bf16 hi/lo split MFMAs against a pre-split item tile layout. It keeps candidates within a per-user error band of the k-th score, and reruns in fp32 when the candidate buffer overflows. The aim is to cut the cost of fp32 MFMA and item-tile bandwidth in scoring. The change touches only the scorer's ranking path, so the BPR training throughput metric should not be affected.

New measurement: 3.351 billion. 2.3% lower.

```diff
diff --git a/cornac_amd/_lib.py b/cornac_amd/_lib.py
--- a/cornac_amd/_lib.py
+++ b/cornac_amd/_lib.py
@@ -60,6 +60,7 @@
     "cornac_hip_scorer_set_f64", "cornac_hip_score_user_f64",
     "cornac_hip_score_block", "cornac_hip_rank_topk", "cornac_hip_rank_topk_device", "cornac_hip_score_pairs",
     "cornac_hip_scorer_set_exclusions", "cornac_hip_rank_topk_resident", "cornac_hip_scorer_host_buffer",
+    "cornac_hip_scorer_rank_filter", "cornac_hip_scorer_rank_stats", "cornac_hip_scorer_rank_filter_debug",
     "cornac_hip_rank_positions",
 ]
 
@@ -270,6 +271,9 @@
         L.cornac_hip_scorer_set_exclusions.argtypes = [_vp, _vp, _vp]
         L.cornac_hip_scorer_host_buffer.argtypes = [_vp, C.c_size_t, C.POINTER(_vp)]
         L.cornac_hip_rank_topk_resident.argtypes = [_vp, _vp, C.c_int64, C.c_int64, C.c_int, _vp, _vp, _vp]
+        L.cornac_hip_scorer_rank_filter.argtypes = [_vp, C.c_int]
+        L.cornac_hip_scorer_rank_stats.argtypes = [_vp, _vp, C.c_int]
+        L.cornac_hip_scorer_rank_filter_debug.argtypes = [_vp, _i32, C.c_int64, _f32, _f32]
         _lib = L
     return _lib
 
@@ -973,6 +977,24 @@
         check(lib().cornac_hip_rank_topk_device(self.h, u0, n, topk, repeats, C.byref(ms)))
         return ms.value
 
+    RANK_STATS = ("filter", "fp32_switched_off", "fp32_unqualified", "fp32_no_band", "fp32_no_bitmap",
+                  "overflow_reruns", "max_kept", "qualified")
+
+    def rank_filter(self, enable):
+        check(lib().cornac_hip_scorer_rank_filter(self.h, 1 if enable else 0))
+
+    def rank_stats(self):
+        out = np.zeros(len(self.RANK_STATS), np.int64)
+        check(lib().cornac_hip_scorer_rank_stats(self.h, out.ctypes.data, len(out)))
+        return dict(zip(self.RANK_STATS, (int(v) for v in out)))
+
+    def rank_filter_debug(self, users):
+        users = np.ascontiguousarray(users, np.int32)
+        approx = np.empty((len(users), self.n_items), np.float32)
+        eps = np.empty(len(users), np.float32)
+        check(lib().cornac_hip_scorer_rank_filter_debug(self.h, users, len(users), approx, eps))
+        return approx, eps
+
 
 class VbprTrainer:
     NAMES = ("Bi", "Gu", "Gi", "Tu", "E", "Bp")
diff --git a/cornac_amd/csrc/rank_filter.inc b/cornac_amd/csrc/rank_filter.inc
--- /dev/null
+++ b/cornac_amd/csrc/rank_filter.inc
@@ -0,0 +1,80 @@
+typedef __bf16 bf16x8 __attribute__((ext_vector_type(8)));
+
+constexpr float kFiltMinMag = 0x1p-50f, kFiltMaxMag = 0x1p40f;
+
+__host__ __device__ __forceinline__ uint32_t bf16_rne_bits(float x) {
+    const uint32_t b = __builtin_bit_cast(uint32_t, x);
+    return (b + 0x7fffu + ((b >> 16) & 1u)) >> 16;
+}
+__host__ __device__ __forceinline__ void bf16_split(float x, uint32_t &hi, uint32_t &lo) {
+    hi = bf16_rne_bits(x);
+    lo = bf16_rne_bits(x - __builtin_bit_cast(float, hi << 16));
+}
+__device__ __forceinline__ void bf16_split8(const v4f32 x0, const v4f32 x1, uint4 &h, uint4 &l) {
+    uint32_t hh[8], ll[8];
+    const float x[8] = {x0.x, x0.y, x0.z, x0.w, x1.x, x1.y, x1.z, x1.w};
+#pragma unroll
+    for (int j = 0; j < 8; ++j) bf16_split(x[j], hh[j], ll[j]);
+    h = make_uint4(hh[0] | (hh[1] << 16), hh[2] | (hh[3] << 16), hh[4] | (hh[5] << 16), hh[6] | (hh[7] << 16));
+    l = make_uint4(ll[0] | (ll[1] << 16), ll[2] | (ll[3] << 16), ll[4] | (ll[5] << 16), ll[6] | (ll[7] << 16));
+}
+
+template <int NS>
+__device__ __forceinline__ void filt_load_a(const float *__restrict__ p, uint4 *ah, uint4 *al) {
+#pragma unroll
+    for (int s = 0; s < NS; ++s)
+        bf16_split8(*reinterpret_cast<const v4f32 *>(p + 16 * s), *reinterpret_cast<const v4f32 *>(p + 16 * s + 4), ah[s], al[s]);
+}
+
+template <int NS>
+__device__ __forceinline__ f32x16 filt_mfma(int m, const uint4 *ah, const uint4 *al, const uint4 *bh, const uint4 *bl,
+                                            f32x16 acc) {
+    const int s = m / 3, w = m % 3;
+    const uint4 a = w == 2 ? al[s] : ah[s];
+    const uint4 b = w == 1 ? bl[s] : bh[s];
+    return __builtin_amdgcn_mfma_f32_32x32x16_bf16(__builtin_bit_cast(bf16x8, a), __builtin_bit_cast(bf16x8, b), acc, 0, 0, 0);
+}
+
+__global__ __launch_bounds__(256) void filt_split_tiles_kernel(const float *__restrict__ Vr, int64_t n_tiles, int kp,
+                                                               uint4 *__restrict__ Vq) {
+    const int qr = kp / 8, nch = 64 * qr;
+    const int64_t c = (int64_t)blockIdx.x * 256 + threadIdx.x;
+    if (c >= n_tiles * nch) return;
+    const int64_t tile = c / nch;
+    const int r = (int)(c % nch), blk = r / (32 * qr), row = (r / qr) & 31, cc = r % qr;
+    const float *src = Vr + ((tile * 32 + row) * kp + cc * 8);
+    uint4 h, l;
+    bf16_split8(*reinterpret_cast<const v4f32 *>(src), *reinterpret_cast<const v4f32 *>(src + 4), h, l);
+    Vq[c] = blk ? l : h;
+}
+
+template <int NS>
+__global__ __launch_bounds__(64) void filt_debug_kernel(const float *__restrict__ U, const uint4 *__restrict__ Vq,
+                                                        const float *__restrict__ ibr, const float *__restrict__ user_base,
+                                                        const int32_t *__restrict__ users, const int32_t *__restrict__ perm,
+                                                        int64_t n_rows, int64_t n_items, float *__restrict__ out) {
+    constexpr int KP = 16 * NS, QR = KP / 8;
+    const int lane = threadIdx.x, col = lane & 31, half = lane >> 5;
+    const int64_t it = blockIdx.x, row_tile = blockIdx.y;
+    uint4 ah[NS], al[NS], bh[NS], bl[NS];
+    const int64_t r = row_tile * 32 + col;
+    filt_load_a<NS>(U + (r < n_rows ? (int64_t)users[r] : 0) * KP + 8 * half, ah, al);
+    const uint4 *tile = Vq + it * (64 * QR);
+#pragma unroll
+    for (int s = 0; s < NS; ++s) {
+        bh[s] = tile[col * QR + 2 * s + half];
+        bl[s] = tile[32 * QR + col * QR + 2 * s + half];
+    }
+    f32x16 acc = {0.f, 0.f, 0.f, 0.f, 0.f, 0.f, 0.f, 0.f, 0.f, 0.f, 0.f, 0.f, 0.f, 0.f, 0.f, 0.f};
+#pragma unroll
+    for (int m = 0; m < 3 * NS; ++m) acc = filt_mfma<NS>(m, ah, al, bh, bl, acc);
+    const int64_t p = it * 32 + col;
+    if (p >= n_items) return;
+    const float ib = ibr[p];
+    const int64_t item = perm[p];
+#pragma unroll
+    for (int q = 0; q < 16; ++q) {
+        const int64_t row = row_tile * 32 + (q & 3) + 8 * (q >> 2) + 4 * half;
+        if (row < n_rows) out[row * n_items + item] = user_base ? (ib + user_base[users[row]]) + acc[q] : ib + acc[q];
+    }
+}
diff --git a/cornac_amd/csrc/score.hip b/cornac_amd/csrc/score.hip
--- a/cornac_amd/csrc/score.hip
+++ b/cornac_amd/csrc/score.hip
@@ -121,7 +121,9 @@
     return (uint32_t)(uintptr_t)(__attribute__((address_space(3))) T *)p;
 }
 
-template <int KT, int CAP, bool UB>
+#include "rank_filter.inc"
+
+template <int KT, int CAP, bool UB, bool FILT = false>
 __global__ __launch_bounds__(kBlk, ((KT <= 32 || CAP <= 42) ? 2 : 1)) void rank_fused_kernel(const float *__restrict__ U, const float *__restrict__ V,
                                                           const float *__restrict__ item_base,
                                                           const float *__restrict__ user_base,
@@ -131,14 +133,23 @@
                                                           const int32_t *__restrict__ excl_indices, int64_t excl_row0,
                                                           const uint32_t *__restrict__ excl_bits,
                                                           const int32_t *__restrict__ perm, float *tau_pub,
-                                                          unsigned long long *__restrict__ part, int ablate) {
+                                                          unsigned long long *__restrict__ part, int ablate,
+                                                          const uint4 *__restrict__ Vq, const float *__restrict__ eps_u,
+                                                          int *ovf_flag, int *kept_max_out) {
     constexpr int KP = 2 * KT;
     __shared__ unsigned long long keys[kBlk / 64][32][CAP];
     __shared__ int32_t ipos[3][32];
     __shared__ int cnt[kBlk / 64][32];
     __shared__ float tau[kBlk / 64][32];
-    __shared__ float btile[2][32][KP + 1];
+    __shared__ float btile[FILT ? 1 : 2][FILT ? 1 : 32][KP + 1];
     __shared__ uint32_t meta_dump[1];
+    constexpr int NS = KP / 16;
+    constexpr int QR = KP / 8;
+    constexpr int RS = QR + 1;
+    constexpr int NCH = 64 * QR;
+    constexpr int SLOTS = FILT ? CAP - 32 : 0;
+    __shared__ uint4 bq[FILT ? 2 : 1][FILT ? 64 * RS : 1];
+    __shared__ float eps2s[FILT ? kBlk / 64 : 1][32];
     __shared__ uint32_t wmask[3][kBlk / 64][32];
     __shared__ float ibase[3][32];
     const int wave = threadIdx.x >> 6, lane = threadIdx.x & 63;
@@ -150,13 +161,14 @@
     const int64_t work_end = min(work_total, pos + work_per_wg);
     int64_t cur_rb = 0;
     float bcur[KT];
-    constexpr int STG = (32 * KP / 4 + kBlk - 1) / kBlk;
+    constexpr int STG = FILT ? (NCH + kBlk - 1) / kBlk : (32 * KP / 4 + kBlk - 1) / kBlk;
     v4f32 stg[STG];
     uint32_t voff[STG];
 #pragma unroll
     for (int q = 0; q < STG; ++q) {
         const int idx = threadIdx.x + q * kBlk;
-        voff[q] = idx < 32 * KP / 4 ? (uint32_t)(((idx / (KP / 4)) * KP + 4 * (idx % (KP / 4))) * 4) : 0u;
+        if constexpr (FILT) voff[q] = idx < NCH ? (uint32_t)idx * 16u : 0u;
+        else voff[q] = idx < 32 * KP / 4 ? (uint32_t)(((idx / (KP / 4)) * KP + 4 * (idx % (KP / 4))) * 4) : 0u;
     }
     uint32_t stg_a = 0;
     int32_t stg_id = 0;
@@ -179,7 +191,8 @@
         pb = perm + it * 32 + (threadIdx.x & 31);
     };
     auto stage_load = [&](int64_t it) {
-        const char *vb = reinterpret_cast<const char *>(V) + it * (int64_t)(32 * KP * 4);
+        const char *vb = FILT ? reinterpret_cast<const char *>(Vq) + it * (int64_t)(NCH * 16)
+                              : reinterpret_cast<const char *>(V) + it * (int64_t)(32 * KP * 4);
 #pragma unroll
         for (int q = 0; q < STG; ++q) stg[q] = *reinterpret_cast<const v4f32 *>(vb + voff[q]);
         stg_a = *pa;
@@ -201,7 +214,10 @@
 #pragma unroll
         for (int q = 0; q < STG; ++q) {
             const int idx = threadIdx.x + q * kBlk;
-            if ((q + 1) * kBlk <= 32 * KP / 4 || idx < 32 * KP / 4) {
+            if constexpr (FILT) {
+                if ((q + 1) * kBlk <= NCH || idx < NCH)
+                    bq[buf][(idx / (32 * QR)) * 32 * RS + ((idx / QR) & 31) * RS + (idx % QR)] = __builtin_bit_cast(uint4, stg[q]);
+            } else if ((q + 1) * kBlk <= 32 * KP / 4 || idx < 32 * KP / 4) {
                 float *dst = &btile[buf][idx / (KP / 4)][4 * (idx % (KP / 4))];
                 dst[0] = stg[q].x; dst[1] = stg[q].y; dst[2] = stg[q].z; dst[3] = stg[q].w;
             }
@@ -214,6 +230,15 @@
 #pragma unroll
         for (int t = g * FG; t < (g + 1) * FG; ++t) bcur[t] = btile[buf][col][2 * t + half];
     };
+    uint4 bh[FILT ? NS : 1], bl[FILT ? NS : 1];
+    auto load_frags_q = [&](int buf) {
+#pragma unroll
+        for (int s = 0; s < NS; ++s) {
+            bh[s] = bq[buf][col * RS + 2 * s + half];
+            bl[s] = bq[buf][32 * RS + col * RS + 2 * s + half];
+        }
+    };
+    int kept_max = 0;
     const f32x16 zero16 = {0.f, 0.f, 0.f, 0.f, 0.f, 0.f, 0.f, 0.f, 0.f, 0.f, 0.f, 0.f, 0.f, 0.f, 0.f, 0.f};
 
     int64_t pos_hi = work_end;
@@ -233,9 +258,15 @@
             if (row >= n_rows) t0 = INFINITY;
             else if (t_begin > 0) t0 = __hip_atomic_load(tau_pub + row, __ATOMIC_RELAXED, __HIP_MEMORY_SCOPE_AGENT);
             tau[wave][lane] = t0;
-        }
-        float a[KT];
-        {
+            if constexpr (FILT) eps2s[wave][lane] = row < n_rows ? 2.f * eps_u[users ? (int64_t)users[row] : u0 + row] : 0.f;
+        }
+        float a[FILT ? 1 : KT];
+        uint4 ah[FILT ? NS : 1], al[FILT ? NS : 1];
+        if constexpr (FILT) {
+            const int64_t r = row_tile * 32 + col;
+            const int64_t u = r < n_rows ? (users ? (int64_t)users[r] : u0 + r) : 0;
+            filt_load_a<NS>(U + u * KP + 8 * half, ah, al);
+        } else {
             const int64_t r = row_tile * 32 + col;
             const bool ok = r < n_rows;
             const int64_t u = ok ? (users ? (int64_t)users[r] : u0 + r) : 0;
@@ -259,7 +290,10 @@
             __builtin_amdgcn_fence(__ATOMIC_ACQ_REL, "wavefront");
             __builtin_amdgcn_wave_barrier();
 #pragma unroll
-            for (int r = 0; r < 16; ++r) thr[r] = tau[wave][(r & 3) + 8 * (r >> 2) + 4 * half];
+            for (int r = 0; r < 16; ++r) {
+                const int rl = (r & 3) + 8 * (r >> 2) + 4 * half;
+                thr[r] = FILT ? tau[wave][rl] - eps2s[wave][rl] : tau[wave][rl];
+            }
         }
         auto compact = [&](unsigned need_l) __attribute__((always_inline)) {
             unsigned need = __builtin_amdgcn_readlane(need_l, 0) | __builtin_amdgcn_readlane(need_l, 32);
@@ -304,14 +338,31 @@
                     for (int q = 0; q < 8; ++q) rank += (j0 + q < c && kj[q] > mine) ? 1 : 0;
                 }
                 const bool live = mine != 0ull;
-                const int n_keep = min(__popcll(__ballot(live)), topk);
                 const unsigned long long kth_mask = __ballot(live && rank == topk - 1);
-                if (lane < CAP) krow[lane] = 0ull;
-                if (live && rank < topk) krow[rank] = mine;
-                if (kth_mask != 0ull) {
-                    const int src = __builtin_ctzll(kth_mask);
-                    const unsigned hi = __builtin_amdgcn_readlane((unsigned)(mine >> 32), src);
-                    if (lane == 0 && row_tile * 32 + rl < n_rows) tau[wave][rl] = key_to_float(hi);
+                int n_keep;
+                if constexpr (FILT) {
+                    bool keep = live;
+                    if (kth_mask != 0ull) {
+                        const int src = __builtin_ctzll(kth_mask);
+                        const float kth = key_to_float(__builtin_amdgcn_readlane((unsigned)(mine >> 32), src));
+                        keep = live && key_to_float((uint32_t)(mine >> 32)) >= kth - eps2s[wave][rl];
+                        if (lane == 0 && row_tile * 32 + rl < n_rows) tau[wave][rl] = kth;
+                    }
+                    const int n_band = __popcll(__ballot(keep));
+                    kept_max = max(kept_max, n_band);
+                    n_keep = min(n_band, SLOTS);
+                    if (n_band > SLOTS && lane == 0) __hip_atomic_store(ovf_flag, 1, __ATOMIC_RELAXED, __HIP_MEMORY_SCOPE_SYSTEM);
+                    if (lane < CAP) krow[lane] = 0ull;
+                    if (live && rank < n_keep) krow[rank] = mine;
+                } else {
+                    n_keep = min(__popcll(__ballot(live)), topk);
+                    if (lane < CAP) krow[lane] = 0ull;
+                    if (live && rank < topk) krow[rank] = mine;
+                    if (kth_mask != 0ull) {
+                        const int src = __builtin_ctzll(kth_mask);
+                        const unsigned hi = __builtin_amdgcn_readlane((unsigned)(mine >> 32), src);
+                        if (lane == 0 && row_tile * 32 + rl < n_rows) tau[wave][rl] = key_to_float(hi);
+                    }
                 }
                 if (lane == 0) cnt[wave][rl] = n_keep;
             }
@@ -320,7 +371,7 @@
 #pragma unroll
             for (int r = 0; r < 16; ++r) {
                 const int rl = (r & 3) + 8 * (r >> 2) + 4 * half;
-                thr[r] = tau[wave][rl];
+                thr[r] = FILT ? tau[wave][rl] - eps2s[wave][rl] : tau[wave][rl];
                 cnt_r[r] = cnt[wave][rl];
             }
         };
@@ -333,7 +384,13 @@
         stage_store(0, 0);
         __syncthreads();
         if (t_begin + 1 < t_end) stage_load(t_begin + 1);
-        {
+        if constexpr (FILT) {
+            load_frags_q(0);
+            ib_a = ibase[0][col];
+            id_a = ipos[0][col];
+#pragma unroll
+            for (int m = 0; m < 3 * NS; ++m) acc_a = filt_mfma<NS>(m, ah, al, bh, bl, acc_a);
+        } else {
 #pragma unroll
             for (int t = 0; t < KT; ++t) bcur[t] = btile[0][col][2 * t + half];
             ib_a = ibase[0][col];
@@ -346,7 +403,8 @@
         auto step = [&](int64_t it, f32x16 &acc_cur, f32x16 &acc_nxt, float &ib_cur, float &ib_nxt, int32_t &id_cur,
                         int32_t &id_nxt) __attribute__((always_inline)) {
             const int buf_next = (int)((it + 1 - t_begin) & 1);
-            load_frags(buf_next, 0);
+            if constexpr (FILT) load_frags_q(buf_next);
+            else load_frags(buf_next, 0);
             __builtin_amdgcn_sched_barrier(0);
             if (it + 2 < t_end && !(ablate & 2)) stage_load(it + 2);
             const int wb1 = wb == 2 ? 0 : wb + 1, wb2 = wb1 == 2 ? 0 : wb1 + 1;
@@ -355,27 +413,40 @@
             const int32_t item = id_cur;
             unsigned long long hm[16];
             float sc[16];
-#pragma unroll
-            for (int g = 0; g < KT / FG; ++g) {
-                if (g + 1 < KT / FG) load_frags(buf_next, g + 1);
-                __builtin_amdgcn_sched_barrier(0);
-#pragma unroll
-                for (int t = g * FG; t < (g + 1) * FG; ++t) {
-                    if (t == 0) acc_nxt = __builtin_amdgcn_mfma_f32_32x32x2f32(a[t], bcur[t], zero16, 0, 0, 0);
-                    else acc_nxt = __builtin_amdgcn_mfma_f32_32x32x2f32(a[t], bcur[t], acc_nxt, 0, 0, 0);
-                    if (t < 16) {
-                        const int r = t;
+            if constexpr (FILT) {
+                constexpr int NM = 3 * NS;
+#pragma unroll
+                for (int m = 0; m < NM; ++m) {
+#pragma unroll
+                    for (int r = m * 16 / NM; r < (m + 1) * 16 / NM; ++r) {
                         sc[r] = UB ? (ib_cur + ubias[r]) + acc_cur[r] : ib_cur + acc_cur[r];
                         hm[r] = __ballot(sc[r] >= thr[r]);
                     }
+                    acc_nxt = filt_mfma<NS>(m, ah, al, bh, bl, m == 0 ? zero16 : acc_nxt);
                 }
-                __builtin_amdgcn_sched_barrier(0);
-            }
-            if (KT < 16) {
-#pragma unroll
-                for (int r = KT; r < 16; ++r) {
-                    sc[r] = UB ? (ib_cur + ubias[r]) + acc_cur[r] : ib_cur + acc_cur[r];
-                    hm[r] = __ballot(sc[r] >= thr[r]);
+            } else {
+#pragma unroll
+                for (int g = 0; g < KT / FG; ++g) {
+                    if (g + 1 < KT / FG) load_frags(buf_next, g + 1);
+                    __builtin_amdgcn_sched_barrier(0);
+#pragma unroll
+                    for (int t = g * FG; t < (g + 1) * FG; ++t) {
+                        if (t == 0) acc_nxt = __builtin_amdgcn_mfma_f32_32x32x2f32(a[t], bcur[t], zero16, 0, 0, 0);
+                        else acc_nxt = __builtin_amdgcn_mfma_f32_32x32x2f32(a[t], bcur[t], acc_nxt, 0, 0, 0);
+                        if (t < 16) {
+                            const int r = t;
+                            sc[r] = UB ? (ib_cur + ubias[r]) + acc_cur[r] : ib_cur + acc_cur[r];
+                            hm[r] = __ballot(sc[r] >= thr[r]);
+                        }
+                    }
+                    __builtin_amdgcn_sched_barrier(0);
+                }
+                if (KT < 16) {
+#pragma unroll
+                    for (int r = KT; r < 16; ++r) {
+                        sc[r] = UB ? (ib_cur + ubias[r]) + acc_cur[r] : ib_cur + acc_cur[r];
+                        hm[r] = __ballot(sc[r] >= thr[r]);
+                    }
                 }
             }
             unsigned long long any = 0ull;
@@ -440,12 +511,17 @@
         for (int rl = 0; rl < 32; ++rl) {
             const int64_t row = row_tile * 32 + rl;
             if (row >= n_rows) break;
-            if (lane < topk) part[(seg * n_rows + row) * topk + lane] = keys[wave][rl][lane];
+            if constexpr (FILT) {
+                if (lane < SLOTS) part[(seg * n_rows + row) * SLOTS + lane] = keys[wave][rl][lane];
+            } else if (lane < topk) part[(seg * n_rows + row) * topk + lane] = keys[wave][rl][lane];
         }
         if (t_begin == 0 && t_end < n_item_tiles && lane < 32 && row_tile * 32 + lane < n_rows)
             __hip_atomic_store(tau_pub + row_tile * 32 + lane, tau[wave][lane], __ATOMIC_RELAXED, __HIP_MEMORY_SCOPE_AGENT);
         __builtin_amdgcn_fence(__ATOMIC_ACQ_REL, "wavefront");
         __builtin_amdgcn_wave_barrier();
+    }
+    if constexpr (FILT) {
+        if (lane == 0 && kept_max > 0) atomicMax(kept_max_out, kept_max);
     }
 }
 
@@ -508,19 +584,40 @@
     }
 }
 
+template <bool RESCORE>
 __global__ __launch_bounds__(64) void rank_merge_kernel(const unsigned long long *__restrict__ part, int n_strips,
-                                                        int64_t n_rows, int topk, int pad,
+                                                        int64_t n_rows, int stride, int topk, int pad,
                                                         int32_t *__restrict__ items_out,
-                                                        float *__restrict__ scores_out) {
+                                                        float *__restrict__ scores_out, const float *__restrict__ U,
+                                                        const float *__restrict__ V, const float *__restrict__ item_base,
+                                                        const float *__restrict__ user_base,
+                                                        const int32_t *__restrict__ users, int64_t u0, int k, int ld) {
     extern __shared__ unsigned long long mlist[];
     const int64_t row = blockIdx.x;
     const int tid = threadIdx.x;
-    const int n = n_strips * topk;
-    for (int i = tid; i < pad; i += 64) {
+    const int n = n_strips * stride;
+    auto load_key = [&](int i) {
         unsigned long long key = 0ull;
-        if (i < n) key = part[((int64_t)(i / topk) * n_rows + row) * topk + (i % topk)];
-        mlist[i] = key;
-    }
+        if (i < n) key = part[((int64_t)(i / stride) * n_rows + row) * stride + (i % stride)];
+        if constexpr (RESCORE) {
+            if (key != 0ull) {
+                const int64_t u = users ? (int64_t)users[row] : u0 + row, item = (int64_t)(uint32_t)key;
+                const float *pu = U + u * ld, *pv = V + item * ld;
+                float acc = 0.f;
+                for (int f = 0; f < ld; f += 4) {
+                    const v4f32 a = *reinterpret_cast<const v4f32 *>(pu + f), b = *reinterpret_cast<const v4f32 *>(pv + f);
+                    acc = fmaf(a.x, b.x, acc);
+                    acc = fmaf(a.y, b.y, acc);
+                    acc = fmaf(a.z, b.z, acc);
+                    acc = fmaf(a.w, b.w, acc);
+                }
+                const float sc = user_base ? (item_base[item] + user_base[u]) + acc : item_base[item] + acc;
+                key = ((unsigned long long)order_key(sc) << 32) | (unsigned long long)(uint32_t)item;
+            }
+        }
+        return key;
+    };
+    for (int i = tid; i < pad; i += 64) mlist[i] = load_key(i);
     __syncthreads();
     for (int kk = 2; kk <= pad; kk <<= 1) {
         for (int j = kk >> 1; j > 0; j >>= 1) {
@@ -849,6 +946,14 @@
     DevBuf<int32_t> res_excl_indices;
     bool has_res_excl = false;
     DevBuf<float> tau_pub;
+    DevBuf<uint4> Vq;
+    DevBuf<float> eps_u;
+    DevBuf<int> kept_max;
+    int *ovf_host = nullptr;
+    bool filt_ok = false;
+    bool filt_enabled = true;
+    bool filt_suspended = false;
+    int64_t st_filter = 0, st_off = 0, st_unqualified = 0, st_band = 0, st_no_bitmap = 0, st_overflow = 0;
     bool has_user_base = false, is_set = false;
     DevBuf<float> scores;
     DevBuf<uint8_t> excl;
@@ -943,6 +1048,74 @@
                        h->Vr.p, h->ibr.p);
     HIP_CHECK(hipGetLastError());
     HIP_CHECK(hipStreamSynchronize(h->stream));
+}
+
+static double filt_c(int kp) {
+    return 1.01 * (3.03 * 0x1p-16 + 1.03 * 3.0 * kp * 0x1p-22 + 1.01 * kp * 0x1p-24 + 0x1p-22);
+}
+static float filt_eps(int kp, double unorm, double vmax, double ub_abs, double ib_max) {
+    const double e = filt_c(kp) * unorm * vmax + 0x1p-22 * (ub_abs + ib_max) + 0x1p-100;
+    return std::nextafter((float)e, INFINITY);
+}
+
+static void build_rank_filter(cornac_hip_scorer_t h, const float *U, const float *V, const float *item_base,
+                              const float *user_base) {
+    h->filt_ok = false;
+    if (h->k > 128) return;
+    const int64_t ni = h->n_items, nu = h->n_users;
+    const int k = h->k;
+    auto in_range = [](float x) {
+        const float a = std::fabs(x);
+        return a == 0.f || (a >= kFiltMinMag && a <= kFiltMaxMag);
+    };
+    double vmax2 = 0, ibmax = 0;
+    for (int64_t i = 0; i < ni; ++i) {
+        double n2 = 0;
+        for (int f = 0; f < k; ++f) {
+            const float x = V[i * k + f];
+            if (!in_range(x)) return;
+            n2 += (double)x * x;
+        }
+        vmax2 = std::max(vmax2, n2);
+        if (item_base) {
+            if (!(std::fabs(item_base[i]) <= kFiltMaxMag)) return;
+            ibmax = std::max(ibmax, (double)std::fabs(item_base[i]));
+        }
+    }
+    const double vmax = std::sqrt(vmax2) * (1.0 + 0x1p-40);
+    std::vector<float> eps((size_t)nu);
+    for (int64_t u = 0; u < nu; ++u) {
+        double n2 = 0;
+        for (int f = 0; f < k; ++f) {
+            const float x = U[u * k + f];
+            if (!in_range(x)) return;
+            n2 += (double)x * x;
+        }
+        double ub = 0;
+        if (user_base) {
+            if (!(std::fabs(user_base[u]) <= kFiltMaxMag)) return;
+            ub = std::fabs(user_base[u]);
+        }
+        eps[(size_t)u] = filt_eps(h->ld, std::sqrt(n2) * (1.0 + 0x1p-40), vmax, ub, ibmax);
+    }
+    const int64_t n_tiles = (ni + 31) / 32;
+    const int64_t chunks = n_tiles * 64 * (h->ld / 8);
+    h->Vq.ensure((size_t)chunks);
+    hipLaunchKernelGGL(filt_split_tiles_kernel, dim3((unsigned)((chunks + 255) / 256)), dim3(256), 0, h->stream, h->Vr.p,
+                       n_tiles, h->ld, h->Vq.p);
+    HIP_CHECK(hipGetLastError());
+    h->eps_u.ensure((size_t)nu);
+    h->eps_u.upload(eps.data(), (size_t)nu, h->stream);
+    if (!h->kept_max.p) {
+        h->kept_max.ensure(1);
+        HIP_CHECK(hipMemsetAsync(h->kept_max.p, 0, sizeof(int), h->stream));
+    }
+    if (!h->ovf_host) {
+        HIP_CHECK(hipHostMalloc(reinterpret_cast<void **>(&h->ovf_host), sizeof(int), hipHostMallocMapped));
+        *h->ovf_host = 0;
+    }
+    HIP_CHECK(hipStreamSynchronize(h->stream));
+    h->filt_ok = true;
 }
 
 static void validate_csr(const int64_t *indptr, const int32_t *indices, int64_t n, int64_t n_items, const char *what) {
@@ -1029,14 +1202,37 @@
     const int ablate = prof_env_int("CORNAC_HIP_RANK_ABLATE", 0);
     const int64_t n_item_tiles = (h->n_items + 31) / 32;
     const int64_t wg_rows = (n + 127) / 128;
-    const int wgs_per_cu = (h->ld <= 64 || topk <= 10) ? 2 : 1;
+    const bool bitmap_ok = !d_excl_indptr || (n_item_tiles <= kMaxBitmapTiles && !prof_env_set("CORNAC_HIP_RANK_NO_BITMAP"));
+    bool filt = false;
+    if (!h->filt_enabled || h->filt_suspended) ++h->st_off;
+    else if (!h->filt_ok) ++h->st_unqualified;
+    else if (topk > 24) ++h->st_band;
+    else if (!bitmap_ok) ++h->st_no_bitmap;
+    else {
+        filt = true;
+        ++h->st_filter;
+    }
+    const int filt_cap = topk <= 16 ? 56 : 64;
     const int64_t work_total = wg_rows * n_item_tiles;
-    int64_t work_per_wg = std::max<int64_t>((work_total + (int64_t)di.cus * wgs_per_cu - 1) / ((int64_t)di.cus * wgs_per_cu),
-                                            std::min<int64_t>(16, n_item_tiles));
-    const int64_t n_wgs = (work_total + work_per_wg - 1) / work_per_wg;
-    const int64_t max_segs = (n_item_tiles + work_per_wg - 1) / work_per_wg + 1;
-    h->part.ensure((size_t)(max_segs * n * topk));
-    HIP_CHECK(hipMemsetAsync(h->part.p, 0, (size_t)(max_segs * n * topk) * sizeof(unsigned long long), h->stream));
+    int stride = 0;
+    int64_t work_per_wg = 0, n_wgs = 0, max_segs = 0;
+    auto decompose = [&] {
+        stride = filt ? filt_cap - 32 : topk;
+        const int wgs_per_cu = filt ? (h->ld <= 64 ? 2 : 1) : (h->ld <= 64 || topk <= 10) ? 2 : 1;
+        work_per_wg = std::max<int64_t>((work_total + (int64_t)di.cus * wgs_per_cu - 1) / ((int64_t)di.cus * wgs_per_cu),
+                                        std::min<int64_t>(16, n_item_tiles));
+        n_wgs = (work_total + work_per_wg - 1) / work_per_wg;
+        max_segs = (n_item_tiles + work_per_wg - 1) / work_per_wg + 1;
+    };
+    decompose();
+    if (filt && max_segs * stride > 8192) {
+        filt = false;
+        --h->st_filter;
+        ++h->st_band;
+        decompose();
+    }
+    h->part.ensure((size_t)(max_segs * n * stride));
+    HIP_CHECK(hipMemsetAsync(h->part.p, 0, (size_t)(max_segs * n * stride) * sizeof(unsigned long long), h->stream));
     h->tau_pub.ensure((size_t)n);
     HIP_CHECK(hipMemsetD32Async((hipDeviceptr_t)h->tau_pub.p, 0xff800000u , (size_t)n, h->stream));
     const uint32_t *d_bits = nullptr;
@@ -1062,12 +1258,35 @@
     if (ub)                                                                                                       \
         hipLaunchKernelGGL((rank_fused_kernel<KT_, CAP_, true>), grid, block, 0, h->stream, h->U.p, h->Vr.p,       \
                            h->ibr.p, ub, d_users, u0, n, h->n_items, work_per_wg, topk, d_bits ? nullptr : d_excl_indptr, \
-                           d_excl_indices, excl_row0, d_bits, h->perm.p, h->tau_pub.p, h->part.p, ablate);       \
+                           d_excl_indices, excl_row0, d_bits, h->perm.p, h->tau_pub.p, h->part.p, ablate, nullptr, nullptr, nullptr, nullptr); \
     else                                                                                                          \
         hipLaunchKernelGGL((rank_fused_kernel<KT_, CAP_, false>), grid, block, 0, h->stream, h->U.p, h->Vr.p,      \
                            h->ibr.p, ub, d_users, u0, n, h->n_items, work_per_wg, topk, d_bits ? nullptr : d_excl_indptr, \
-                           d_excl_indices, excl_row0, d_bits, h->perm.p, h->tau_pub.p, h->part.p, ablate); } while (0)
-    if (topk <= 10 && h->ld == 128) {
+                           d_excl_indices, excl_row0, d_bits, h->perm.p, h->tau_pub.p, h->part.p, ablate, nullptr, nullptr, nullptr, nullptr); } while (0)
+#define FUSED_FILT(KT_, CAP_) do {                                                                               \
+    int *ovf_dev = nullptr;                                                                                       \
+    HIP_CHECK(hipHostGetDevicePointer(reinterpret_cast<void **>(&ovf_dev), h->ovf_host, 0));                      \
+    if (ub)                                                                                                       \
+        hipLaunchKernelGGL((rank_fused_kernel<KT_, CAP_, true, true>), grid, block, 0, h->stream, h->U.p, h->Vr.p, \
+                           h->ibr.p, ub, d_users, u0, n, h->n_items, work_per_wg, topk, nullptr,                  \
+                           d_excl_indices, excl_row0, d_bits, h->perm.p, h->tau_pub.p, h->part.p, ablate, h->Vq.p, h->eps_u.p, ovf_dev, h->kept_max.p); \
+    else                                                                                                          \
+        hipLaunchKernelGGL((rank_fused_kernel<KT_, CAP_, false, true>), grid, block, 0, h->stream, h->U.p, h->Vr.p, \
+                           h->ibr.p, ub, d_users, u0, n, h->n_items, work_per_wg, topk, nullptr,                  \
+                           d_excl_indices, excl_row0, d_bits, h->perm.p, h->tau_pub.p, h->part.p, ablate, h->Vq.p, h->eps_u.p, ovf_dev, h->kept_max.p); } while (0)
+    if (filt) {
+        if (filt_cap == 56) {
+            if (h->ld == 16) FUSED_FILT(8, 56);
+            else if (h->ld == 32) FUSED_FILT(16, 56);
+            else if (h->ld == 64) FUSED_FILT(32, 56);
+            else FUSED_FILT(64, 56);
+        } else {
+            if (h->ld == 16) FUSED_FILT(8, 64);
+            else if (h->ld == 32) FUSED_FILT(16, 64);
+            else if (h->ld == 64) FUSED_FILT(32, 64);
+            else FUSED_FILT(64, 64);
+        }
+    } else if (topk <= 10 && h->ld == 128) {
         FUSED(64, 42);
     } else if (topk <= 24) {
         if (h->ld == 16) FUSED(8, 56);
@@ -1081,10 +1300,17 @@
         else FUSED(64, 64);
     }
 #undef FUSED
+#undef FUSED_FILT
     int pad = 1;
-    while (pad < (int)max_segs * topk) pad <<= 1;
-    hipLaunchKernelGGL(rank_merge_kernel, dim3((unsigned)n), dim3(64), (size_t)pad * 8, h->stream, h->part.p,
-                       (int)max_segs, n, topk, pad, items_out, scores_out);
+    while (pad < (int)max_segs * stride) pad <<= 1;
+    if (filt)
+        hipLaunchKernelGGL(rank_merge_kernel<true>, dim3((unsigned)n), dim3(64), (size_t)pad * 8, h->stream, h->part.p,
+                           (int)max_segs, n, stride, topk, pad, items_out, scores_out, h->U.p, h->V.p, h->item_base.p, ub,
+                           d_users, u0, h->k, h->ld);
+    else
+        hipLaunchKernelGGL(rank_merge_kernel<false>, dim3((unsigned)n), dim3(64), (size_t)pad * 8, h->stream, h->part.p,
+                           (int)max_segs, n, stride, topk, pad, items_out, scores_out, nullptr, nullptr, nullptr, nullptr,
+                           nullptr, 0, h->k, h->ld);
     HIP_CHECK(hipGetLastError());
 }
 
@@ -1103,6 +1329,18 @@
                                excl_by_user);
     }
 }
+
+static bool filt_overflowed(cornac_hip_scorer_t h) {
+    if (!h->ovf_host || !*h->ovf_host) return false;
+    *h->ovf_host = 0;
+    ++h->st_overflow;
+    return true;
+}
+struct FiltSuspend {
+    cornac_hip_scorer_t h;
+    explicit FiltSuspend(cornac_hip_scorer_t h_) : h(h_) { h->filt_suspended = true; }
+    ~FiltSuspend() { h->filt_suspended = false; }
+};
 
 extern "C" {
 
@@ -1137,6 +1375,7 @@
             (void)hipStreamDestroy(h->stream);
         }
         if (h->pinned_out) (void)hipHostFree(h->pinned_out);
+        if (h->ovf_host) (void)hipHostFree(h->ovf_host);
         for (void *q : h->pinned_retired) (void)hipHostFree(q);
         delete h;
     });
@@ -1156,6 +1395,7 @@
         h->has_user_base = user_base != nullptr;
         if (user_base) h->user_base.upload(user_base, (size_t)h->n_users, h->stream);
         build_rank_order(h, U, V, item_base);
+        build_rank_filter(h, U, V, item_base, user_base);
         HIP_CHECK(hipStreamSynchronize(h->stream));
         h->is_set = true;
     });
@@ -1272,11 +1512,18 @@
             h->d_items_out.ensure((size_t)(n * topk));
             h->d_scores_out.ensure((size_t)(n * topk));
             h->d_users.upload(users, (size_t)n, h->stream);
-            launch_rank_fused(h, h->d_users.p, 0, n, topk, have_excl ? h->d_excl_indptr.p : nullptr,
-                              have_excl ? h->d_excl_indices.p : nullptr, 0, h->d_items_out.p, h->d_scores_out.p);
-            h->d_items_out.download(items_out, (size_t)(n * topk), h->stream);
-            h->d_scores_out.download(scores_out, (size_t)(n * topk), h->stream);
-            HIP_CHECK(hipStreamSynchronize(h->stream));
+            auto run = [&] {
+                launch_rank_fused(h, h->d_users.p, 0, n, topk, have_excl ? h->d_excl_indptr.p : nullptr,
+                                  have_excl ? h->d_excl_indices.p : nullptr, 0, h->d_items_out.p, h->d_scores_out.p);
+                h->d_items_out.download(items_out, (size_t)(n * topk), h->stream);
+                h->d_scores_out.download(scores_out, (size_t)(n * topk), h->stream);
+                HIP_CHECK(hipStreamSynchronize(h->stream));
+            };
+            run();
+            if (filt_overflowed(h)) {
+                FiltSuspend fp32_only(h);
+                run();
+            }
             return;
         }
         int64_t cap = rows_per_batch(h);
@@ -1426,14 +1673,21 @@
         if (device_ms) {
             HIP_CHECK(hipEventCreate(&e0));
             HIP_CHECK(hipEventCreate(&e1));
-            HIP_CHECK(hipEventRecord(e0, h->stream));
-        }
-        launch_rank_fused(h, users ? h->d_users.p : nullptr, u0, n, topk, h->res_excl_indptr.p, h->res_excl_indices.p, 0,
-                          h->d_items_out.p, h->d_scores_out.p, true);
-        if (device_ms) HIP_CHECK(hipEventRecord(e1, h->stream));
-        if (items_out) h->d_items_out.download(items_out, (size_t)(n * topk), h->stream);
-        if (scores_out) h->d_scores_out.download(scores_out, (size_t)(n * topk), h->stream);
-        HIP_CHECK(hipStreamSynchronize(h->stream));
+        }
+        auto run = [&] {
+            if (device_ms) HIP_CHECK(hipEventRecord(e0, h->stream));
+            launch_rank_fused(h, users ? h->d_users.p : nullptr, u0, n, topk, h->res_excl_indptr.p, h->res_excl_indices.p, 0,
+                              h->d_items_out.p, h->d_scores_out.p, true);
+            if (device_ms) HIP_CHECK(hipEventRecord(e1, h->stream));
+            if (items_out) h->d_items_out.download(items_out, (size_t)(n * topk), h->stream);
+            if (scores_out) h->d_scores_out.download(scores_out, (size_t)(n * topk), h->stream);
+            HIP_CHECK(hipStreamSynchronize(h->stream));
+        };
+        run();
+        if (filt_overflowed(h)) {
+            FiltSuspend fp32_only(h);
+            run();
+        }
         if (device_ms) {
             float t = 0.f;
             HIP_CHECK(hipEventElapsedTime(&t, e0, e1));
@@ -1480,6 +1734,7 @@
         hipEvent_t e0, e1;
         HIP_CHECK(hipEventCreate(&e0));
         HIP_CHECK(hipEventCreate(&e1));
+        auto run = [&] {
         HIP_CHECK(hipEventRecord(e0, h->stream));
         for (int r = 0; r < repeats; ++r) {
             for (int64_t b0 = 0; b0 < n; b0 += cap) {
@@ -1495,6 +1750,12 @@
         }
         HIP_CHECK(hipEventRecord(e1, h->stream));
         HIP_CHECK(hipEventSynchronize(e1));
+        };
+        run();
+        if (fused && filt_overflowed(h)) {
+            FiltSuspend fp32_only(h);
+            run();
+        }
         float t = 0.f;
         HIP_CHECK(hipEventElapsedTime(&t, e0, e1));
         (void)hipEventDestroy(e0);
@@ -1502,4 +1763,59 @@
         *ms = (double)t;
     });
 }
-}
+
+int cornac_hip_scorer_rank_filter(cornac_hip_scorer_t h, int enable) {
+    return guarded([&] {
+        sc_check(h, false);
+        h->filt_enabled = enable != 0;
+    });
+}
+
+int cornac_hip_scorer_rank_stats(cornac_hip_scorer_t h, int64_t *out, int n) {
+    return guarded([&] {
+        sc_check(h, false);
+        REQUIRE(out != nullptr && n >= 0, "bad arguments");
+        int kept = 0;
+        if (h->kept_max.p) {
+            HIP_CHECK(hipStreamSynchronize(h->stream));
+            HIP_CHECK(hipMemcpy(&kept, h->kept_max.p, sizeof(int), hipMemcpyDeviceToHost));
+        }
+        const int64_t v[CORNAC_HIP_RANK_STATS_N] = {h->st_filter,  h->st_off,      h->st_unqualified, h->st_band,
+                                                    h->st_no_bitmap, h->st_overflow, (int64_t)kept,     h->filt_ok ? 1 : 0};
+        for (int i = 0; i < n && i < CORNAC_HIP_RANK_STATS_N; ++i) out[i] = v[i];
+    });
+}
+
+int cornac_hip_scorer_rank_filter_debug(cornac_hip_scorer_t h, const int32_t *users, int64_t n, float *approx_out,
+                                        float *eps_out) {
+    return guarded([&] {
+        sc_check(h);
+        REQUIRE(users && approx_out && eps_out && n > 0, "bad arguments");
+        REQUIRE(h->filt_ok, "the scorer's tables do not qualify for the bf16 filter");
+        for (int64_t b = 0; b < n; ++b)
+            REQUIRE(users[b] >= 0 && users[b] < h->n_users, "user %d out of range", users[b]);
+        REQUIRE(n * h->n_items <= (int64_t(1) << 28), "debug block too large");
+        DevBuf<int32_t> du;
+        DevBuf<float> dout;
+        du.alloc((size_t)n);
+        dout.alloc((size_t)(n * h->n_items));
+        du.upload(users, (size_t)n, h->stream);
+        const float *ub = h->has_user_base ? h->user_base.p : nullptr;
+        dim3 grid((unsigned)((h->n_items + 31) / 32), (unsigned)((n + 31) / 32));
+#define DBG(NS_) hipLaunchKernelGGL(filt_debug_kernel<NS_>, grid, dim3(64), 0, h->stream, h->U.p, h->Vq.p, h->ibr.p, ub, du.p, \
+                                    h->perm.p, n, h->n_items, dout.p)
+        if (h->ld == 16) DBG(1);
+        else if (h->ld == 32) DBG(2);
+        else if (h->ld == 64) DBG(4);
+        else DBG(8);
+#undef DBG
+        HIP_CHECK(hipGetLastError());
+        dout.download(approx_out, (size_t)(n * h->n_items), h->stream);
+        HIP_CHECK(hipStreamSynchronize(h->stream));
+        std::vector<float> all((size_t)h->n_users);
+        h->eps_u.download(all.data(), (size_t)h->n_users, h->stream);
+        HIP_CHECK(hipStreamSynchronize(h->stream));
+        for (int64_t b = 0; b < n; ++b) eps_out[b] = all[(size_t)users[b]];
+    });
+}
+}
diff --git a/include/cornac_hip.h b/include/cornac_hip.h
--- a/include/cornac_hip.h
+++ b/include/cornac_hip.h
@@ -264,6 +264,11 @@
                               const int32_t *excl_indices, const int64_t *tgt_indptr, const int32_t *tgt_indices,
                               int32_t *greater_out, int32_t *pos_out, int32_t *ge_out, float *tgt_scores_out);
 int cornac_hip_rank_topk_device(cornac_hip_scorer_t h, int64_t u0, int64_t n, int topk, int repeats, double *ms);
+int cornac_hip_scorer_rank_filter(cornac_hip_scorer_t h, int enable);
+#define CORNAC_HIP_RANK_STATS_N 8
+int cornac_hip_scorer_rank_stats(cornac_hip_scorer_t h, int64_t *out, int n);
+int cornac_hip_scorer_rank_filter_debug(cornac_hip_scorer_t h, const int32_t *users, int64_t n, float *approx_out,
+                                        float *eps_out);
 
 #ifdef __cplusplus
 }
```
